# Lanv1/gsplat.js

Measured on AMD Instinct MI355X. Metric: frames_per_sec, higher is better.
Workload: dtype f32

## Files before the change

### gsplat.js_amd/csrc/gsr_api.cpp

```cpp
#include "gsr_ctx.h"

#include <cstdarg>
#include <cstdio>
#include <cstdlib>
#include <cstring>
#include <mutex>

using namespace gsr;

namespace {

thread_local std::string g_create_error;

Knobs read_knobs(std::string& bad)
{
    Knobs k;
    if (const char* e = getenv("GSR_NO_GRAPH")) k.graphs = atoi(e) == 0;
    if (const char* e = getenv("GSR_FUSE_COMBINE")) k.fuse_combine = atoi(e) != 0;
    if (const char* e = getenv("GSR_SATURATE")) k.saturate = atoi(e) != 0;
    if (const char* e = getenv("GSR_ITEMS_BY_SIZE")) k.items_by_size = atoi(e) != 0 ? 1 : 0;
    if (const char* e = getenv("GSR_LONG_ITEMS")) k.long_items = atoi(e) != 0 ? 1 : 0;
    if (const char* e = getenv("GSR_LONG_TAU")) k.long_tau = (uint32_t)std::max(0L, atol(e));
    if (const char* e = getenv("GSR_BIN_ROUNDS")) k.bin_rounds = std::min(64L, std::max(0L, atol(e)));
    if (const char* e = getenv("GSR_BIN_BIG")) k.bin_big = (uint32_t)std::min(2, std::max(0, atoi(e)));
    if (const char* e = getenv("GSR_BIN_TWO_LEVEL")) k.bin_two_level = atoi(e) ? 1 : 0;
    if (const char* e = getenv("GSR_RECT_CARRY")) { k.rect_carry = atoi(e) != 0; k.rect_carry_bucket = atoi(e) == 2; }
    if (const char* e = getenv("GSR_BLEND_SUB")) k.blend_sub = atoi(e) == 2 ? 2 : atoi(e) == 1 ? 1 : 0;
    if (const char* e = getenv("GSR_SORT_ORDER")) k.sort_order = !strcmp(e, "lsd") ? 0 : !strcmp(e, "bucket") ? 1 : -1;
    if (const char* e = getenv("GSR_TIMING_EVERY")) k.timing_every = (uint32_t)std::max(1L, atol(e));
    if (const char* e = getenv("GSR_CELL_GRID")) { const long v = atol(e); if (v >= 1) k.cell_grid = (uint32_t)std::min(v, 65535L); }
    if (const char* e = getenv("GSR_SEG_TARGET")) { const long v = atol(e); if (v >= 1) k.seg_target = (uint32_t)v; }
    if (const char* e = getenv("GSR_BLEND_GRID")) { const long v = atol(e); if (v >= 1) k.blend_grid = (uint32_t)v; }
    if (const char* e = getenv("GSR_SEG_LEN")) { const long v = atol(e); if (v >= 256) k.seg_len = (uint32_t)(v / 256 * 256); }
    if (const char* e = getenv("GSR_SORT_KPB")) { const long v = atol(e); if (v == 2048 || v == 4096 || v == 8192) k.sort_kpb = (uint32_t)v; }
    if (const char* e = getenv("GSR_FRONT_WAVES")) {
        char* end = nullptr;
        const long v = strtol(e, &end, 10);
        if (end != e && *end == 0 && (v == (long)FRONT_WAVES_NARROW || v == (long)FRONT_WAVES_WIDE)) k.front_waves = (uint32_t)v;
        else bad = std::string("GSR_FRONT_WAVES must be ") + std::to_string(FRONT_WAVES_NARROW) + " or " + std::to_string(FRONT_WAVES_WIDE) + ", not \"" + e + "\"";
    }
    if (const char* e = getenv("GSR_DEPTH_SKIP")) k.depth_skip = atoi(e) != 0;
    return k;
}

int alloc_fb(gsr_ctx* c)
{
    const size_t np = (size_t)c->W * c->H;
    if (np > c->out.pixels) {
        if (int r = c->out.fb.alloc(c, np)) return r;
        if (int r = c->out.fb8.alloc(c, np)) return r;
        c->out.pixels = np;
    }
    launch_clear_fb(c->out.fb, c->W, c->H, c->stream);
    return GSR_OK;
}

}

int gsr::fail(gsr_ctx* c, int code, const char* fmt, ...)
{
    char buf[512];
    va_list ap;
    va_start(ap, fmt);
    vsnprintf(buf, sizeof buf, fmt, ap);
    va_end(ap);
    if (c) {
        c->error = buf;
        if (code == GSR_ERR_HIP) c->words.slots_need_init = true;
    }
    else g_create_error = buf;
    return code;
}

extern "C" {

const char* gsr_last_error(gsr_ctx* ctx) { return ctx ? ctx->error.c_str() : g_create_error.c_str(); }

int gsr_create(gsr_ctx** out, const gsr_options* opt)
{
    if (!out) return fail(nullptr, GSR_ERR_ARG, "out is NULL");
    *out = nullptr;
    std::string bad_knob;
    const Knobs knobs = read_knobs(bad_knob);
    if (!bad_knob.empty()) return fail(nullptr, GSR_ERR_ARG, "%s", bad_knob.c_str());
    int count = 0;
    if (hipGetDeviceCount(&count) != hipSuccess || count <= 0)
        return fail(nullptr, GSR_ERR_NO_DEVICE, "no HIP device is visible (this library has no CPU path)");
    gsr_options o{};
    if (opt) o = *opt;
    if (o.device < 0 || o.device >= count) return fail(nullptr, GSR_ERR_ARG, "device %d out of range (%d visible)", o.device, count);
    if (o.width < 0 || o.height < 0 || o.width > 8192 || o.height > 8192) return fail(nullptr, GSR_ERR_ARG, "bad framebuffer size %dx%d (up to 8192)", o.width, o.height);
    if (!(o.early_out_eps >= 0.0f && o.early_out_eps < 1.0f)) return fail(nullptr, GSR_ERR_ARG, "early_out_eps must be in [0,1)");
    gsr_ctx* c = new gsr_ctx();
    c->device = o.device;
    c->scene = new SharedScene();
    c->scene->members.push_back(c);
    c->scene_gen = c->scene->generation;
    c->opt = o;
    c->knobs = knobs;
    c->graph.enabled = c->knobs.graphs;
    c->timing.every = c->knobs.timing_every;
    auto bail = [&](int code) {
        g_create_error = c->error;
        gsr_destroy(c);
        return code;
    };
    gsr_ctx::Words& w = c->words;
    const int r = [&]() -> int {
        HIP_TRY(c, hipSetDevice(c->device));
        HIP_TRY(c, hipStreamCreateWithFlags(&c->stream, hipStreamNonBlocking));
        int cus = 0;
        if (hipDeviceGetAttribute(&cus, hipDeviceAttributeMultiprocessorCount, c->device) == hipSuccess && cus > 0) c->cu_count = cus;
        const size_t slot_words = (size_t)3 * FRAME_SLOTS * FRAME_SLOT_WORDS;
        if (int r = w.fstate.alloc(c, 1)) return r;
        if (int r = w.cam_dev.alloc(c, 1)) return r;
        if (int r = w.slots.alloc(c, slot_words)) return r;
        HIP_TRY(c, hipMemset(w.slots, 0, sizeof(int32_t) * slot_words));
        w.slots_need_init = true;
        if (int r = w.accum.alloc(c, 8)) return r;
        HIP_TRY(c, hipMemset(w.accum, 0, 8 * sizeof(uint64_t)));
        HIP_TRY(c, hipHostMalloc((void**)&w.mailbox, 64, hipHostMallocMapped));
        memset(w.mailbox, 0, 64);
        reinterpret_cast<uint32_t*>(w.mailbox)[2] = 0xffffffffu;
        HIP_TRY(c, hipHostGetDevicePointer((void**)&w.mailbox_dev, w.mailbox, 0));
        HIP_TRY(c, hipHostMalloc((void**)&w.fstate_host, sizeof(FrameState), hipHostMallocDefault));
        memset(w.fstate_host, 0, sizeof(FrameState));
        w.fstate_host->minmax[0] = 0x7fffffff;
        w.fstate_host->minmax[1] = (int32_t)0x80000000;
        HIP_TRY(c, hipMemcpy(w.fstate, w.fstate_host, sizeof(FrameState), hipMemcpyHostToDevice));
        if (o.flags & GSR_FLAG_TIMING) {
            for (auto& set : c->timing.evring)
                for (auto& e : set) HIP_TRY(c, hipEventCreate(&e));
            c->timing.valid = true;
        }
        if (o.width && o.height) {
            if (int r = gsr_resize(c, o.width, o.height)) return r;
            if (o.band_x1 > o.band_x0) {
                if (int r = gsr_set_band(c, o.band_x0, o.band_x1)) return r;
            }
        }
        return GSR_OK;
    }();
    if (r) return bail(r);
    *out = c;
    return GSR_OK;
}

int gsr_destroy(gsr_ctx* c)
{
    if (!c) return GSR_OK;
    (void)hipSetDevice(c->device);
    if (c->stream) (void)hipStreamSynchronize(c->stream);
    comm_release(c);
    delivery_free(c);
    drop_graph(c);
    scene_release(c);
    if (c->share_ev) (void)hipEventDestroy(c->share_ev);
    for (auto& set : c->timing.evring)
        for (auto& e : set) if (e) (void)hipEventDestroy(e);
    for (auto& e : c->link_ev) if (e) (void)hipEventDestroy(e);
    if (c->words.fstate_host) (void)hipHostFree(c->words.fstate_host);
    if (c->words.mailbox) (void)hipHostFree(c->words.mailbox);
    if (c->stream) (void)hipStreamDestroy(c->stream);
    delete c;
    return GSR_OK;
}

int gsr_resize(gsr_ctx* c, int32_t w, int32_t h)
{
    if (!c) return GSR_ERR_ARG;
    if (w <= 0 || h <= 0 || w > 8192 || h > 8192) return fail(c, GSR_ERR_ARG, "bad framebuffer size %dx%d (1..8192)", w, h);
    const gsr_ctx::Delivery& dl = c->delivery;
    const bool new_ring = !dl.ring.empty() && (w != dl.W || h != dl.H);
    if (new_ring && delivery_frame_held(c))
        return fail(c, GSR_ERR_ARG, "gsr_resize: a delivered frame is held (gsr_release_frame first): its pixels would be freed");
    HIP_TRY(c, hipSetDevice(c->device));
    HIP_TRY(c, hipStreamSynchronize(c->stream));
    if (c->comm.nccl && (w != c->W || h != c->H)) comm_release(c);
    c->W = w; c->H = h;
    c->band_x0 = c->band_x1 = 0;
    c->have_frame = false;
    if (int r = alloc_fb(c)) return r;
    if (new_ring) { if (int r = delivery_alloc(c, (int)dl.ring.size())) return r; }
    return alloc_bins(c);
}

int gsr_set_band(gsr_ctx* c, int32_t x0, int32_t x1)
{
    if (!c) return GSR_ERR_ARG;
    if (x0 == 0 && x1 == 0) { c->band_x0 = c->band_x1 = 0; return alloc_bins(c); }
    if (x0 < 0 || x1 <= x0 || x0 % BIN_PX) return fail(c, GSR_ERR_ARG, "band [%d,%d) must start on a multiple of %d", x0, x1, BIN_PX);
    if (x1 > c->W) x1 = c->W;
    if (x0 >= c->W) return fail(c, GSR_ERR_ARG, "band starts outside the image");
    HIP_TRY(c, hipSetDevice(c->device));
    HIP_TRY(c, hipStreamSynchronize(c->stream));
    c->band_x0 = x0; c->band_x1 = x1;
    launch_clear_fb(c->out.fb, c->W, c->H, c->stream);
    return alloc_bins(c);
}

int gsr_set_list_capacity(gsr_ctx* c, uint32_t entries)
{
    if (!c) return GSR_ERR_ARG;
    HIP_TRY(c, hipSetDevice(c->device));
    HIP_TRY(c, hipStreamSynchronize(c->stream));
    c->bin.capacity = std::max<uint32_t>(entries, 1024u);
    if (int r = c->bin.list.alloc(c, c->bin.capacity)) return r;
    return alloc_bins(c, true);
}

int gsr_set_camera(gsr_ctx* c, const float* view, const float* proj, const float* vp, float fx, float fy)
{
    if (!c) return GSR_ERR_ARG;
    if (!view || !proj || !vp) return fail(c, GSR_ERR_ARG, "matrix pointer is NULL");
    memcpy(c->cam.view, view, 64);
    memcpy(c->cam.proj, proj, 64);
    c->cam.vp2 = vp[2]; c->cam.vp6 = vp[6]; c->cam.vp10 = vp[10];
    c->cam.fx = fx; c->cam.fy = fy;
    c->have_cam = true;
    return GSR_OK;
}

int gsr_set_depth_fade(gsr_ctx* c, int32_t use_depth_fade, float depth_fade)
{
    if (!c) return GSR_ERR_ARG;
    c->cam.use_fade = use_depth_fade ? 1 : 0;
    c->cam.fade = depth_fade;
    return GSR_OK;
}

int gsr_render_async(gsr_ctx* c)
{
    if (!c) return GSR_ERR_ARG;
    HIP_TRY(c, hipSetDevice(c->device));
    return enqueue_frame(c, true);
}

int gsr_sync(gsr_ctx* c)
{
    if (!c) return GSR_ERR_ARG;
    HIP_TRY(c, hipSetDevice(c->device));
    if (int r = sync_and_repair(c)) return r;
    if (c->comm.stream) HIP_TRY(c, hipStreamSynchronize(c->comm.stream));
    if (c->delivery.copy_stream) HIP_TRY(c, hipStreamSynchronize(c->delivery.copy_stream));
    if (c->words.dropped_unreported) {
        const unsigned long long k = c->words.dropped_unreported;
        c->words.dropped_unreported = 0;
        return fail(c, GSR_ERR_OVERFLOW,
                    "%llu asynchronous frame(s) were not composited: their bin lists did not fit and later frames had already been "
                    "enqueued (the framebuffer kept the preceding image for them); the lists have been regrown, the context stays usable",
                    k);
    }
    return GSR_OK;
}

int gsr_overflow_pending(gsr_ctx* c) { return c && overflow_pending(c) ? 1 : 0; }

int gsr_render(gsr_ctx* c)
{
    if (int r = gsr_render_async(c)) return r;
    c->timing.render = true;
    return gsr_sync(c);
}

int gsr_sort(gsr_ctx* c)
{
    if (!c) return GSR_ERR_ARG;
    HIP_TRY(c, hipSetDevice(c->device));
    if (int r = enqueue_frame(c, false)) return r;
    return finish_frame(c);
}

int gsr_get_timings(gsr_ctx* c, gsr_timings* out)
{
    if (!c || !out) return GSR_ERR_ARG;
    if (c->timing.recorded) { if (int r = finish_frame(c)) return r; }
    *out = c->timing.tm;
    out->overflow_frames = c->words.overflow_frames;
    out->dropped_frames = c->words.dropped_frames;
    return GSR_OK;
}

int gsr_set_timing_interval(gsr_ctx* c, uint32_t every)
{
    if (!c || !every) return c ? fail(c, GSR_ERR_ARG, "timing interval must be >= 1") : GSR_ERR_ARG;
    c->timing.every = every;
    c->timing.frame_no = 0;
    return GSR_OK;
}

int gsr_reset_timings(gsr_ctx* c)
{
    if (!c) return GSR_ERR_ARG;
    if (c->timing.recorded) { if (int r = finish_frame(c)) return r; }
    gsr_timings& tm = c->timing.tm;
    const uint64_t v = tm.visible, b = tm.bin_entries, d = tm.tile_entries;
    tm = gsr_timings{};
    HIP_TRY(c, hipMemsetAsync(c->words.accum, 0, 4 * sizeof(uint64_t), c->stream));
    tm.visible = v; tm.bin_entries = b; tm.tile_entries = d; tm.n = c->scene->n;
    c->timing.frame_no = 0;
    return GSR_OK;
}

int gsr_device_info(gsr_ctx* c, char* name, int32_t name_len, int32_t* cus, int32_t* clock_khz)
{
    if (!c) return GSR_ERR_ARG;
    hipDeviceProp_t p;
    HIP_TRY(c, hipGetDeviceProperties(&p, c->device));
    if (name && name_len > 0) snprintf(name, (size_t)name_len, "%s (%s)", p.name[0] ? p.name : "AMD GPU", p.gcnArchName);
    if (cus) *cus = p.multiProcessorCount;
    if (clock_khz) *clock_khz = p.clockRate;
    return GSR_OK;
}

void gsplat_sort_host(const float* viewProj, uint32_t vertexCount, const float* fBuffer, uint32_t* depthBuffer,
                      uint32_t* depthIndex, uint32_t* starts, uint32_t* counts)
{
    (void)starts; (void)counts;
    static std::mutex mu;
    static gsr_ctx* ctx = nullptr;
    std::lock_guard<std::mutex> lock(mu);
    auto failed = [&](const char* what) {
        fprintf(stderr, "gsplat_sort_host: %s\n", what);
        if (depthIndex && vertexCount) memset(depthIndex, 0, (size_t)vertexCount * sizeof(uint32_t));
    };
    if (!viewProj || !depthIndex || (vertexCount && !fBuffer)) return failed("NULL argument");
    if (!ctx) {
        gsr_options o{};
        if (gsr_create(&ctx, &o) != GSR_OK) { ctx = nullptr; return failed(gsr_last_error(nullptr)); }
    }
    gsr_ctx* c = ctx;
    if (hipSetDevice(c->device) != hipSuccess || hipStreamSynchronize(c->stream) != hipSuccess) return failed("device unavailable");
    if (vertexCount != c->scene->n || !c->scene->arr.px) {
        if (vertexCount > 0x7fffffffu / 8) return failed("too many splats");
        if (alloc_scene(c, vertexCount, false) != GSR_OK) return failed(gsr_last_error(c));
        c->scene->n = vertexCount;
    }
    c->have_sort = false; c->have_frame = false;
    static DevBuf<float>& stage_pos = *new DevBuf<float>();
    static size_t stage_cap = 0;
    if (vertexCount) {
        if ((size_t)vertexCount * 3 > stage_cap) {
            if (stage_pos.alloc(c, (size_t)vertexCount * 3) != GSR_OK) { stage_cap = 0; return failed(gsr_last_error(c)); }
            stage_cap = (size_t)vertexCount * 3;
        }
        const gsr::SceneArrays& sa = c->scene->arr;
        hipError_t e1 = hipMemcpyAsync(stage_pos, fBuffer, (size_t)vertexCount * 12, hipMemcpyHostToDevice, c->stream);
        launch_repack_positions(stage_pos, vertexCount, sa.px, sa.py, sa.pz, c->stream);
        for (hipError_t e : {e1, hipGetLastError()})
            if (e != hipSuccess) return failed(hipGetErrorString(e));
    }
    float ident[16] = {1, 0, 0, 0, 0, 1, 0, 0, 0, 0, 1, 0, 0, 0, 0, 1};
    if (gsr_set_camera(c, ident, ident, viewProj, 1.f, 1.f) != GSR_OK) return failed(gsr_last_error(c));
    if (hipSetDevice(c->device) != hipSuccess || enqueue_frame(c, false) != GSR_OK) return failed(gsr_last_error(c));
    if (vertexCount) {
        hipError_t e1 = hipMemcpyAsync(depthIndex, c->sort.depth_index, (size_t)vertexCount * 4, hipMemcpyDeviceToHost, c->stream);
        hipError_t e2 = depthBuffer ? hipMemcpyAsync(depthBuffer, c->sort.keys, (size_t)vertexCount * 4, hipMemcpyDeviceToHost, c->stream) : hipSuccess;
        for (hipError_t e : {e1, e2})
            if (e != hipSuccess) return failed(hipGetErrorString(e));
    }
    if (finish_frame(c) != GSR_OK) return failed(gsr_last_error(c));
}

const char* gsr_build_id(void)
{
#ifdef GSR_BUILD_ID
    return GSR_BUILD_ID;
#else
    return "unknown";
#endif
}

}
```

### gsplat.js_amd/csrc/gsr_ctx.h

```cpp
#pragma once
#include "../../include/gsplat_hip.h"
#include "gsr_internal.h"

#include <algorithm>
#include <cstddef>
#include <string>
#include <type_traits>
#include <utility>
#include <vector>

struct ncclComm;

#pragma GCC visibility push(hidden)

namespace gsr {

int fail(gsr_ctx* c, int code, const char* fmt, ...);

#define HIP_TRY(c, expr)                                                                         \
    do {                                                                                         \
        hipError_t e_ = (expr);                                                                  \
        if (e_ != hipSuccess) return gsr::fail((c), GSR_ERR_HIP, "%s failed: %s", #expr, hipGetErrorString(e_)); \
    } while (0)

template <class T>
struct DevBuf {
    T* p = nullptr;
    DevBuf() = default;
    DevBuf(const DevBuf&) = delete;
    DevBuf& operator=(const DevBuf&) = delete;
    DevBuf(DevBuf&& o) noexcept : p(o.p) { o.p = nullptr; }
    DevBuf& operator=(DevBuf&& o) noexcept { std::swap(p, o.p); return *this; }
    ~DevBuf() { reset(); }
    void reset() { if (p) { (void)hipFree(p); p = nullptr; } }
    int alloc(gsr_ctx* c, size_t count)
    {
        reset();
        if (!count) count = 1;
        HIP_TRY(c, hipMalloc((void**)&p, count * sizeof(T)));
        return GSR_OK;
    }
    operator T*() const { return p; }
    T* operator->() const { return p; }
};

enum Stage { EV_BEGIN = 0, EV_PROJECT, EV_SORT, EV_BIN, EV_BLEND , EV_COMBINE , EV_COUNT };

struct FrameState {
    int32_t minmax[2];
    uint32_t overflow;
    uint32_t queue;
    uint64_t visible;
    uint64_t tile_entries;
    uint64_t report[6];
    uint32_t digit_total[RADIX_LO_BINS + RADIX_HI_BINS];
    uint32_t sorted_count;
    uint32_t seg_len;
    uint32_t n_items;
    uint32_t spec;
};

struct Knobs {
    bool graphs = true;
    bool fuse_combine = true;
    bool saturate = true;
    int items_by_size = -1;
    int long_items = -1;
    uint32_t long_tau = 0;
    long bin_rounds = 0;
    uint32_t bin_big = 2;
    int bin_two_level = -1;
    bool rect_carry = true;
    bool rect_carry_bucket = false;
    int blend_sub = 0;
    int sort_order = -1;
    uint32_t timing_every = 1;
    uint32_t cell_grid = 0;
    uint32_t seg_target = 0;
    uint32_t blend_grid = 0;
    uint32_t seg_len = 0;
    uint32_t sort_kpb = 0;
    uint32_t front_waves = 0;
    bool depth_skip = true;
};

struct SceneArrays {
    DevBuf<float> px, py, pz;
    DevBuf<uint32_t> cov0, cov1, cov2, rgba;
    DevBuf<float4> rot, scl;
    int alloc(gsr_ctx* c, size_t n, bool with_rows)
    {
        int r;
        if ((r = px.alloc(c, n)) || (r = py.alloc(c, n)) || (r = pz.alloc(c, n)) || (r = cov0.alloc(c, n)) || (r = cov1.alloc(c, n)) ||
            (r = cov2.alloc(c, n)) || (r = rgba.alloc(c, n)))
            return r;
        rot.reset(); scl.reset();
        if (with_rows && ((r = rot.alloc(c, n)) || (r = scl.alloc(c, n)))) return r;
        return GSR_OK;
    }
    SceneDev view() const { return SceneDev{px, py, pz, cov0, cov1, cov2, rgba, rot, scl}; }
};

struct SharedScene {
    SceneArrays arr;
    uint32_t n = 0;
    uint32_t arr_rows = 0;
    bool have_rows = false;
    bool given = false;
    std::vector<gsr_ctx*> members;
    uint64_t generation = 1;
    DevBuf<uint32_t> sh_r, sh_g, sh_b;
    uint32_t sh_count = 0;
    int32_t band[3] = {-1, -1, -1};
    SceneSoA soa(float4* shcol) const { return SceneSoA{arr.px, arr.py, arr.pz, arr.cov0, arr.cov1, arr.cov2, arr.rgba, sh_r, sh_g, sh_b, shcol}; }
    bool sh_follow = false;
    DevBuf<uint32_t> sh_spare[3];
    uint32_t sh_rows = 0, sh_spare_rows = 0;
    double sh_frame[9] = {1, 0, 0, 0, 1, 0, 0, 0, 1};
    void reset_sh_frame() { for (int k = 0; k < 9; k++) sh_frame[k] = (k % 4 == 0) ? 1.0 : 0.0; }
    bool sh_frame_is_identity() const
    {
        for (int k = 0; k < 9; k++) if (sh_frame[k] != ((k % 4 == 0) ? 1.0 : 0.0)) return false;
        return true;
    }
    void drop_sh() { sh_count = 0; band[0] = band[1] = band[2] = -1; sh_r.reset(); sh_g.reset(); sh_b.reset(); reset_sh_frame();
                     for (auto& b : sh_spare) b.reset();
                     sh_rows = sh_spare_rows = 0; }
    struct Selection {
        DevBuf<uint32_t> mask, scratch;
        DevBuf<uint32_t> counters;
        DevBuf<uint8_t> region;
        uint32_t words = 0;
        uint32_t counter_words = 0;
        size_t region_bytes = 0;
        uint32_t count = 0;
        void reset() { mask.reset(); scratch.reset(); counters.reset(); region.reset(); words = counter_words = 0; region_bytes = 0; count = 0; }
        uint64_t bytes() const { return (uint64_t)words * 8 + (uint64_t)counter_words * 4 + region_bytes; }
    } sel;
    struct Contrib {
        DevBuf<unsigned long long> weight;
        DevBuf<uint32_t> peak, pixels;
        DevBuf<uint32_t> counters;
        uint32_t rows = 0;
        static constexpr uint32_t COUNTER_WORDS = 2;
        bool live() const { return (bool)counters.p; }
        void reset() { weight.reset(); peak.reset(); pixels.reset(); counters.reset(); rows = 0; }
        uint64_t bytes() const { return live() ? (uint64_t)rows * 16 + COUNTER_WORDS * 4 : 0; }
    } contrib;
    uint64_t bytes() const
    {
        return (uint64_t)arr_rows * (7 * 4 + (arr.rot ? 32 : 0)) + ((uint64_t)sh_rows + sh_spare_rows) * 3 * 32 + sel.bytes() + contrib.bytes();
    }
};

struct ProjectArgs {
    SceneSoA sc;
    int32_t* depth; int32_t* slots; Record* rec; uint32_t* rect; uint32_t* overflow; uint32_t* kept; uint8_t* kept_lane;
};

struct FrameArgs {
    ProjectArgs proj;
    int32_t* slots_next;
    SortBuffers sort;
    BinBuffers bin;
    BinGrid grid;
    BlendBuffers blend;
    float early_out_eps;
    uint32_t n;
    bool render;
};
static_assert(std::is_trivially_copyable<FrameArgs>::value, "FrameArgs is compared and copied as bytes");

struct DepthSpec {
    int format = GSR_DEPTH_NONE;
    int step = 1;
    float near = 0.0f;
    static DepthSpec from(const gsr_depth_delivery_options* o)
    {
        if (!o || o->format == GSR_DEPTH_NONE) return {};
        return {o->format, o->step, o->format == GSR_DEPTH_U16 ? o->near : 0.0f};
    }
    bool on() const { return format != GSR_DEPTH_NONE; }
    size_t sample_bytes() const { return format == GSR_DEPTH_U16 ? 2 : 4; }
    bool operator==(const DepthSpec& o) const { return format == o.format && step == o.step && near == o.near; }
    size_t plane_bytes(int Wd, int Hd) const { return (size_t)Wd * Hd * sample_bytes(); }
    gsr_depth_layout layout(int Wd, int Hd, uint64_t offset) const
    {
        gsr_depth_layout l{};
        l.format = format; l.step = step; l.width = Wd; l.height = Hd;
        l.stride = (int32_t)plane_bytes(Wd, 1);
        l.offset = offset;
        l.bytes = plane_bytes(Wd, Hd);
        l.near = near;
        return l;
    }
};

struct DepthPlanes {
    DevBuf<float> hit;
    DevBuf<float> mean;
    DevBuf<uint32_t> index;
    DevBuf<uint32_t> invalid;
    int Wd = 0, Hd = 0;
    int fill_key[4] = {0, 0, 0, 0};
    int alloc(gsr_ctx* c, int W, int H, int step)
    {
        reset();
        Wd = (W + step - 1) / step; Hd = (H + step - 1) / step;
        const size_t np = (size_t)Wd * Hd;
        int r = hit.alloc(c, np);
        if (!r && step == 1) { r = mean.alloc(c, np); if (!r) r = index.alloc(c, np); }
        if (!r) r = invalid.alloc(c, 1);
        if (r) reset();
        return r;
    }
    void reset() { hit.reset(); mean.reset(); index.reset(); invalid.reset(); Wd = Hd = 0; std::fill(fill_key, fill_key + 4, 0); }
};
enum DepthFill { DEPTH_FILL_NOTHING, DEPTH_FILL_HIT , DEPTH_FILL_PLANES  };

}

struct gsr_ctx {
    int device = 0;
    int cu_count = 256;
    hipStream_t stream = nullptr;
    std::string error;
    gsr_options opt{};
    gsr::Knobs knobs;
    int W = 0, H = 0;
    int band_x0 = 0, band_x1 = 0;
    gsr::CamParams cam{};
    gsr::CamParams cam_frame{};
    bool have_cam = false, have_frame = false, have_sort = false;
    uint64_t frame_serial = 0;
    bool frame_lists = false;
    hipEvent_t link_ev[2] = {nullptr, nullptr};

    gsr::SharedScene* scene = nullptr;
    uint64_t scene_gen = 0;
    gsr::DevBuf<float4> shcol;
    hipEvent_t share_ev = nullptr;
    gsr::SceneSoA scene_soa() const { return scene->soa(shcol); }

    struct Sort {
        gsr::DevBuf<int32_t> depth;
        gsr::DevBuf<uint32_t> kept;
        gsr::DevBuf<uint8_t> kept_lane;
        gsr::DevBuf<uint32_t> koff;
        gsr::DevBuf<uint32_t> keys, keys_tmp, idx_tmp, depth_index, block_hist;
        gsr::DevBuf<gsr::Record> rec;
        gsr::DevBuf<uint32_t> rect_idx;
        gsr::DevBuf<uint32_t> rects;
        gsr::DevBuf<uint32_t> rect_tmp;
        gsr::DevBuf<uint32_t> chunk_tab;
        uint32_t rows = 0;
        int parity = 0;
        gsr::SortPlan plan{};
    } sort;

    struct Bin {
        gsr::DevBuf<uint32_t> table, total, start, start_pre, list;
        gsr::DevBuf<uint32_t> cell_list, cell_total, cell_start, chunk_start, chunk_info, cell_table2, cell_wcnt;
        gsr::DevBuf<uint32_t> seg_start, items;
        gsr::DevBuf<unsigned long long> mask;
        gsr::DevBuf<float4> partial;
        gsr::BinPlan plan{};
        gsr::BlendPlan blend{};
        uint32_t cell_capacity_alloc = 0, cell_ncells_alloc = 0;
        uint32_t capacity = 0, table_elems = 0, nbins_alloc = 0;
    } bin;

    struct Words {
        gsr::DevBuf<gsr::FrameState> fstate;
        gsr::FrameState* fstate_host = nullptr;
        gsr::DevBuf<int32_t> slots;
        bool slots_need_init = true;
        gsr::DevBuf<gsr::CamParams> cam_dev;
        gsr::DevBuf<uint64_t> accum;
        uint64_t* mailbox = nullptr;
        uint64_t* mailbox_dev = nullptr;
        uint64_t overflow_seen = 0;
        uint64_t overflow_frames = 0;
        uint64_t dropped_frames = 0;
        uint64_t dropped_unreported = 0;
    } words;

    struct Out {
        gsr::DevBuf<float4> fb;
        gsr::DevBuf<uint32_t> fb8;
        size_t pixels = 0;
    } out;

    struct Graph {
        bool enabled = true;
        hipGraph_t graph = nullptr;
        hipGraphExec_t exec = nullptr;
        hipGraphNode_t project = nullptr;
        gsr::FrameArgs key;
    } graph;
    gsr::ProjectLaunch proj{};

    struct Timing {
        static constexpr int EV_RING = 128;
        hipEvent_t evring[EV_RING][gsr::EV_COUNT]{};
        bool is_render[EV_RING]{};
        int head = 0, pending = 0;
        hipEvent_t* ev = nullptr;
        bool valid = false, recorded = false, render = false;
        uint32_t every = 1, frame_no = 0;
        gsr_timings tm{};
    } timing;

    struct Comm {
        ncclComm* nccl = nullptr;
        gsr_allgather_fn fn = nullptr;
        void* fn_user = nullptr;
        bool owned = true;
        gsr_ctx* leader = nullptr;
        std::vector<gsr_ctx*> followers;
        int rank = 0, world = 0, slab_w = 0;
        hipStream_t stream = nullptr;
        hipEvent_t ev_packed = nullptr, ev_slab_free = nullptr;
        gsr::DevBuf<uint32_t> slab, gathered, frame8;
        gsr::SlabEdges edges{};
        bool frame8_valid = false;
        bool joined() const { return nccl || fn; }
        struct DepthExchange {
            gsr::DepthSpec spec;
            gsr::DepthPlanes planes;
            int W = 0, H = 0;
            int stride = 0;
            size_t offset = 0;
            size_t slab_bytes = 0;
            gsr::SlabEdges edges{};
            gsr::DevBuf<uint32_t> plane;
            bool on() const { return spec.on(); }
            size_t plane_bytes() const { return spec.plane_bytes(planes.Wd, planes.Hd); }
            void reset() { spec = {}; planes.reset(); plane.reset(); W = H = stride = 0; offset = slab_bytes = 0; }
        } depth;
        size_t slab_bytes(int H) const { return depth.on() ? depth.slab_bytes : ((size_t)slab_w * H + gsr::SLAB_FLAG_WORDS) * 4; }
    } comm;

    struct Depth {
        gsr::DepthPlanes planes;
        size_t pixels = 0;
        gsr::DevBuf<int32_t> query;
        gsr::DevBuf<gsr::PickResult> result;
        gsr::DevBuf<uint32_t> pick_invalid;
        float hit_alpha = 0.5f;
        uint64_t planes_serial = 0;
    } depth;

    struct Delivery {
        struct Slot {
            uint8_t* host = nullptr;
            gsr::DevBuf<uint32_t> staging;
            hipEvent_t done = nullptr;
            uint64_t serial = 0;
            enum State { FREE, IN_FLIGHT, HELD } state = FREE;
        };
        std::vector<Slot> ring;
        hipStream_t copy_stream = nullptr;
        hipEvent_t ev_staged = nullptr;
        int W = 0, H = 0;
        int format = GSR_FORMAT_RGBA8;
        gsr::YuvParams yuv{};
        int next = 0;
        uint64_t serial = 0;
        struct DepthPlane {
            gsr::DepthSpec spec;
            gsr::DepthPlanes planes;
        } depth;
        size_t pixel_bytes() const { return format == GSR_FORMAT_RGBA8 ? (size_t)W * H * 4 : gsr::yuv420_bytes(W, H); }
        size_t depth_offset() const { return (pixel_bytes() + 15) & ~(size_t)15; }
        size_t depth_bytes() const { return depth.spec.plane_bytes(depth.planes.Wd, depth.planes.Hd); }
        size_t trailer_offset() const { return depth.spec.on() ? (depth_offset() + depth_bytes() + 15) & ~(size_t)15 : (pixel_bytes() + 3) & ~(size_t)3; }
        size_t slot_bytes() const { return trailer_offset() + gsr::DELIVER_TRAILER_WORDS * 4; }
    } delivery;
};

namespace gsr {

inline BinGrid make_grid(const gsr_ctx* c)
{
    BinGrid g;
    g.W = c->W; g.H = c->H;
    g.nbx = (c->W + BIN_PX - 1) / BIN_PX;
    g.nby = (c->H + BIN_PX - 1) / BIN_PX;
    if (c->band_x1 > c->band_x0) {
        g.bx_lo = c->band_x0 / BIN_PX;
        g.bx_hi = std::min((c->band_x1 + BIN_PX - 1) / BIN_PX, g.nbx);
    } else {
        g.bx_lo = 0; g.bx_hi = g.nbx;
    }
    return g;
}

inline uint32_t front_waves_of(const gsr_ctx* c)
{
    return c->knobs.front_waves ? c->knobs.front_waves : (c->opt.flags & GSR_FLAG_THROUGHPUT) ? FRONT_WAVES_NARROW : FRONT_WAVES_WIDE;
}

inline SortKnobs sort_knobs_of(const gsr_ctx* c)
{
    return SortKnobs{c->knobs.sort_order, c->knobs.sort_kpb, c->knobs.rect_carry ? 1u : 0u, c->knobs.rect_carry_bucket ? 1u : 0u};
}

int alloc_bins(gsr_ctx* c, bool fresh_items = false);
int enqueue_frame(gsr_ctx* c, bool render);
int finish_frame(gsr_ctx* c);
int sync_and_repair(gsr_ctx* c);
void drop_graph(gsr_ctx* c);
int alloc_scene(gsr_ctx* c, uint32_t n, bool with_rows);
int adopt_scene(gsr_ctx* c);
void scene_release(gsr_ctx* c);
int scene_compact(gsr_ctx* c, const ScenePred& p, const char* what, uint32_t* kept_out);
int select_ensure(gsr_ctx* c);
int select_fold_and_count(gsr_ctx* c, int op, uint32_t* selected);
void comm_release(gsr_ctx* c);
int depth_frame_check(gsr_ctx* c, const char* who);
int depth_enqueue(gsr_ctx* c, DepthPlanes& p, int step, DepthFill fill);
int depth_settle_frame(gsr_ctx* c, const char* who);
int depth_planes_current(gsr_ctx* c, const char* who);
int delivery_alloc(gsr_ctx* c, int slots);
int depth_options_check(gsr_ctx* c, const char* who, const gsr_depth_delivery_options* depth);
void delivery_free(gsr_ctx* c);
bool delivery_frame_held(const gsr_ctx* c);

inline bool overflow_pending(const gsr_ctx* c)
{
    return c->words.mailbox && *reinterpret_cast<volatile const uint64_t*>(c->words.mailbox) != c->words.overflow_seen;
}

}

#pragma GCC visibility pop
```

### gsplat.js_amd/csrc/gsr_frame.cpp

```cpp
#include "gsr_ctx.h"

#include <algorithm>
#include <cstring>

using namespace gsr;

namespace {

inline uint32_t largest_bucket_reported(const gsr_ctx* c) { return reinterpret_cast<volatile const uint32_t*>(c->words.mailbox)[2]; }

bool band_is_partial(const BinGrid& g) { return g.bx_lo > 0 || g.bx_hi < g.nbx; }

void build_frame_args(const gsr_ctx* c, bool render, FrameArgs& a)
{
    memset(&a, 0, sizeof a);
    const BinGrid g = make_grid(c);
    const SortPlan sp = plan_sort(c->scene->n, c->sort.rows, front_waves_of(c), render, band_is_partial(g), largest_bucket_reported(c), sort_knobs_of(c));
    FrameState* fs = c->words.fstate;
    a.render = render;
    a.n = c->scene->n;
    a.grid = g;
    a.early_out_eps = c->opt.early_out_eps;

    const size_t slot_set = (size_t)FRAME_SLOTS * FRAME_SLOT_WORDS;
    int32_t* slots_now = render ? c->words.slots.p : c->words.slots + (size_t)(1 + c->sort.parity) * slot_set;
    a.slots_next = render ? nullptr : c->words.slots + (size_t)(2 - c->sort.parity) * slot_set;

    a.proj.sc = c->scene_soa();
    a.proj.depth = c->sort.depth;
    a.proj.slots = slots_now;
    if (render) {
        a.proj.rec = c->sort.rec;
        a.proj.rect = c->sort.rect_idx;
        a.proj.overflow = &fs->overflow;
        a.proj.kept = sp.band ? c->sort.kept.p : nullptr;
        a.proj.kept_lane = sp.band ? c->sort.kept_lane.p : nullptr;
    }

    SortBuffers& sb = a.sort;
    sb.depth = c->sort.depth;
    sb.slots = slots_now;
    sb.minmax = fs->minmax;
    sb.keys = c->sort.keys;
    sb.keys_tmp = c->sort.keys_tmp;
    sb.idx_tmp = c->sort.idx_tmp;
    sb.depth_index = c->sort.depth_index;
    sb.block_hist = c->sort.block_hist;
    sb.digit_total = fs->digit_total;
    sb.rect = c->sort.rect_idx;
    sb.kept = c->sort.kept;
    sb.kept_lane = c->sort.kept_lane;
    sb.koff = sp.band ? c->sort.koff.p : nullptr;
    sb.count = &fs->sorted_count;
    sb.plan = sp;
    sb.max_bucket = reinterpret_cast<uint32_t*>(c->words.mailbox_dev + 1);
    sb.chunk_tab = c->sort.chunk_tab;
    sb.rect_tmp = c->sort.rect_tmp;
    sb.rects_out = sp.carry ? c->sort.rects.p : nullptr;
    if (!render) return;

    BinBuffers& bb = a.bin;
    bb.depth_index = c->sort.depth_index;
    bb.count = &fs->sorted_count;
    bb.table = c->bin.table;
    bb.slots = c->words.slots;
    bb.rect_idx = c->sort.rect_idx;
    bb.rects = c->sort.rects;
    bb.rects_sorted = sp.carry;
    bb.bin_total = c->bin.total;
    bb.bin_start = c->bin.start;
    bb.bin_start_pre = c->bin.start_pre;
    bb.plan = c->bin.plan;
    bb.seg_start = c->bin.seg_start;
    bb.items = c->bin.items;
    bb.list = c->bin.list;
    bb.overflow = &fs->overflow;
    bb.visible = &fs->visible;
    bb.tile_entries = &fs->tile_entries;
    bb.accum = c->words.accum;
    bb.mailbox = c->words.mailbox_dev;
    bb.report = fs->report;
    bb.capacity = c->bin.capacity;
    bb.seg_len_dev = &fs->seg_len;
    bb.queue = &fs->queue;
    bb.bin_mask = c->bin.mask;
    bb.cell_list = c->bin.cell_list;
    bb.cell_total = c->bin.cell_total;
    bb.cell_start = c->bin.cell_start;
    bb.chunk_start = c->bin.chunk_start;
    bb.chunk_info = c->bin.chunk_info;
    bb.cell_wcnt = c->bin.cell_wcnt;
    bb.cell_table2 = c->bin.cell_table2;
    bb.band = band_is_partial(g) ? 1u : 0u;
    bb.n_max = c->scene->n;

    BlendBuffers& bl = a.blend;
    bl.items = bb.items;
    bl.seg_start = bb.seg_start;
    bl.bin_start = bb.bin_start;
    bl.list = bb.list;
    bl.rec = c->sort.rec;
    bl.shcol = c->shcol;
    bl.fb = c->out.fb;
    bl.partial = c->bin.partial;
    bl.queue = bb.queue;
    bl.seg_len_dev = bb.seg_len_dev;
    bl.capacity = bb.capacity;
    bl.nsplats = std::max(c->scene->n, 1u);
    bl.bin_mask = bb.bin_mask;
    bl.plan = c->bin.blend;
}

void set_projection(gsr_ctx* c, const FrameArgs& a)
{
    ProjectLaunch& p = c->proj;
    p.sc = a.proj.sc;
    p.n = a.n;
    p.cam = c->cam;
    p.do_project = 1;
    p.depth = a.proj.depth;
    p.slots = a.proj.slots;
    p.rec = a.proj.rec;
    p.bbox = nullptr;
    p.rect = a.proj.rect;
    p.overflow = a.proj.overflow;
    p.kept = a.proj.kept;
    p.kept_lane = a.proj.kept_lane;
    p.bind();
}

int enqueue_chain(gsr_ctx* c, const FrameArgs& a, bool timing)
{
    hipStream_t s = c->stream;
    hipEvent_t* ev = c->timing.ev;
    if (timing) HIP_TRY(c, hipEventRecord(ev[EV_BEGIN], s));
    if (a.n) {
        if (a.render) launch_project_key(c->proj, s);
        else launch_depth_key(a.proj.sc, a.n, c->cam, a.proj.depth, a.proj.slots, a.slots_next, s);
    } else {
        HIP_TRY(c, hipMemsetD32Async((hipDeviceptr_t)&a.sort.minmax[0], 0x7fffffff, 1, s));
        HIP_TRY(c, hipMemsetD32Async((hipDeviceptr_t)&a.sort.minmax[1], (int)0x80000000u, 1, s));
    }
    if (timing) HIP_TRY(c, hipEventRecord(ev[EV_PROJECT], s));
    launch_sort(a.sort, a.n, s);
    if (timing) HIP_TRY(c, hipEventRecord(ev[EV_SORT], s));
    if (a.render) {
        if (!a.n) {
            HIP_TRY(c, hipMemsetAsync(a.bin.bin_total, 0, sizeof(uint32_t) * a.bin.plan.nbins, s));
            HIP_TRY(c, hipMemsetAsync(a.bin.overflow, 0, sizeof(uint32_t), s));
        }
        launch_bin(a.bin, a.blend.plan, a.grid, s);
        if (timing) HIP_TRY(c, hipEventRecord(ev[EV_BIN], s));
        launch_blend(a.blend, a.grid, a.early_out_eps, s, (timing && !a.blend.plan.fused) ? ev[EV_BLEND] : nullptr);
        if (timing) HIP_TRY(c, hipEventRecord(ev[EV_COMBINE], s));
    }
    HIP_TRY(c, hipGetLastError());
    return GSR_OK;
}

bool capture_graph(gsr_ctx* c, const FrameArgs& a)
{
    hipStream_t s = c->stream;
    if (hipStreamBeginCapture(s, hipStreamCaptureModeRelaxed) != hipSuccess) return false;
    const int r = enqueue_chain(c, a, false);
    hipGraph_t gph = nullptr;
    bool ok = (hipStreamEndCapture(s, &gph) == hipSuccess) && r == GSR_OK && gph;
    hipGraphNode_t project = nullptr;
    if (ok && a.n) {
        size_t nn = 0;
        ok = hipGraphGetNodes(gph, nullptr, &nn) == hipSuccess && nn > 0;
        std::vector<hipGraphNode_t> nodes(nn);
        if (ok) ok = hipGraphGetNodes(gph, nodes.data(), &nn) == hipSuccess;
        for (size_t k = 0; ok && k < nn && !project; k++) {
            hipGraphNodeType ty;
            hipKernelNodeParams kp{};
            if (hipGraphNodeGetType(nodes[k], &ty) == hipSuccess && ty == hipGraphNodeTypeKernel &&
                hipGraphKernelNodeGetParams(nodes[k], &kp) == hipSuccess && kp.func == project_key_kernel())
                project = nodes[k];
        }
        ok = ok && project != nullptr;
    }
    if (ok) ok = hipGraphInstantiate(&c->graph.exec, gph, nullptr, nullptr, 0) == hipSuccess;
    if (ok) { c->graph.graph = gph; c->graph.project = project; memcpy(&c->graph.key, &a, sizeof a); }
    else if (gph) (void)hipGraphDestroy(gph);
    return ok;
}

bool set_graph_camera(gsr_ctx* c)
{
    hipKernelNodeParams kp{};
    kp.func = const_cast<void*>(project_key_kernel());
    kp.gridDim = project_key_grid(c->proj.n);
    kp.blockDim = dim3(PROJ_THREADS);
    kp.sharedMemBytes = 0;
    kp.kernelParams = c->proj.ptrs;
    kp.extra = nullptr;
    return hipGraphExecKernelNodeSetParams(c->graph.exec, c->graph.project, &kp) == hipSuccess;
}

int check_frame_words(gsr_ctx* c, bool* overflowed)
{
    FrameState* host = c->words.fstate_host;
    HIP_TRY(c, hipMemcpyAsync(host, c->words.fstate, offsetof(FrameState, digit_total), hipMemcpyDeviceToHost, c->stream));
    HIP_TRY(c, hipStreamSynchronize(c->stream));
    const uint64_t* acc = host->report;
    gsr_timings& tm = c->timing.tm;
    tm.sum_visible = acc[0]; tm.sum_bin_entries = acc[1]; tm.sum_tile_entries = acc[2]; tm.sum_frames = acc[3];
    tm.visible = host->visible;
    tm.tile_entries = host->tile_entries;
    tm.bin_entries = (uint32_t)host->report[5];
    tm.n = c->scene->n;
    *overflowed = host->overflow != 0;
    return GSR_OK;
}

int handle_overflow(gsr_ctx* c, uint64_t* newly)
{
    *newly = 0;
    HIP_TRY(c, hipStreamSynchronize(c->stream));
    uint64_t acc[8];
    HIP_TRY(c, hipMemcpyAsync(acc, c->words.accum, sizeof acc, hipMemcpyDeviceToHost, c->stream));
    HIP_TRY(c, hipStreamSynchronize(c->stream));
    if (acc[5] == c->words.overflow_seen) return GSR_OK;
    *newly = acc[5] - c->words.overflow_seen;
    c->words.overflow_seen = acc[5];
    c->words.overflow_frames += *newly;
    const uint64_t need = acc[6];
    const uint64_t want = need + (need >> 2) + (1u << 20);
    if (want > 0xfffffff0ull) return fail(c, GSR_ERR_OVERFLOW, "bin list would need %llu entries", (unsigned long long)want);
    if (want > c->bin.capacity) {
        c->bin.capacity = (uint32_t)want;
        if (int r = c->bin.list.alloc(c, c->bin.capacity)) return r;
    }
    return alloc_bins(c, true);
}

}

namespace gsr {

int alloc_bins(gsr_ctx* c, bool fresh_items)
{
    if (!c->W) return GSR_OK;
    c->frame_lists = false;
    gsr_ctx::Bin& b = c->bin;
    const Knobs& k = c->knobs;
    const BinGrid g = make_grid(c);
    const uint64_t capacity = b.capacity ? b.capacity : std::max<uint64_t>(6ull * c->scene->n + (1u << 20), 1u << 22);
    b.plan = plan_bins(g, c->scene->n, capacity, c->cu_count, front_waves_of(c), BinKnobs{k.bin_two_level, k.bin_big, k.bin_rounds, k.cell_grid});
    const BinPlan& p = b.plan;
    const uint32_t nbins = (uint32_t)p.nbins;
    const bool items_afresh = fresh_items || nbins > b.nbins_alloc || !b.capacity;
    const uint32_t items_alloc = items_afresh ? 0u : b.blend.max_items;
    b.blend = plan_blend(nbins, (uint32_t)((g.bx_hi - g.bx_lo) * BIN_PX) * (uint32_t)c->H, (uint32_t)capacity, c->cu_count,
                         (c->opt.flags & GSR_FLAG_THROUGHPUT) != 0, c->opt.early_out_eps > 0.0f, items_alloc,
                         BlendKnobs{k.fuse_combine ? 1u : 0u, k.saturate ? 1u : 0u, k.items_by_size, k.long_items, k.long_tau, k.blend_sub, k.seg_target,
                                    k.blend_grid, k.seg_len});
    const size_t table = (size_t)p.table_rows * p.table_cols;
    if (table > b.table_elems) {
        if (int r = b.table.alloc(c, table)) return r;
        b.table_elems = (uint32_t)table;
    }
    if (nbins > b.nbins_alloc) {
        if (int r = b.total.alloc(c, nbins)) return r;
        if (int r = b.start.alloc(c, nbins + 1)) return r;
        if (int r = b.start_pre.alloc(c, nbins + 1)) return r;
        if (int r = b.seg_start.alloc(c, nbins + 1)) return r;
        if (b.blend.fused) {
            if (int r = b.mask.alloc(c, nbins)) return r;
        }
        b.nbins_alloc = nbins;
    }
    if (!b.capacity) {
        b.capacity = (uint32_t)capacity;
        if (int r = b.list.alloc(c, b.capacity)) return r;
    }
    if (p.form == BIN_TWO_LEVEL) {
        const uint32_t ncells = (uint32_t)p.ncells;
        if (ncells > b.cell_ncells_alloc) {
            if (int r = b.cell_total.alloc(c, ncells + 1)) return r;
            if (int r = b.cell_start.alloc(c, ncells + 1)) return r;
            if (int r = b.chunk_start.alloc(c, ncells + 2)) return r;
            b.cell_ncells_alloc = ncells;
            b.cell_capacity_alloc = 0;
        }
        if (b.capacity > b.cell_capacity_alloc) {
            if (int r = b.cell_list.alloc(c, (size_t)b.capacity * 2)) return r;
            if (int r = b.cell_table2.alloc(c, (size_t)p.chunks * 16u)) return r;
            if (int r = b.chunk_info.alloc(c, (size_t)p.chunks * 4u)) return r;
            if (int r = b.cell_wcnt.alloc(c, (size_t)p.chunks * 64u)) return r;
            b.cell_capacity_alloc = b.capacity;
        }
    }
    if (b.blend.max_items > items_alloc) {
        if (int r = b.items.alloc(c, (size_t)b.blend.max_items * 4)) return r;
        if (b.blend.partial_slots) {
            if (int r = b.partial.alloc(c, (size_t)b.blend.partial_slots * BIN_PX * BIN_PX)) return r;
        }
    }
    return GSR_OK;
}

void drop_graph(gsr_ctx* c)
{
    if (c->graph.exec) (void)hipGraphExecDestroy(c->graph.exec);
    if (c->graph.graph) (void)hipGraphDestroy(c->graph.graph);
    c->graph.exec = nullptr; c->graph.graph = nullptr; c->graph.project = nullptr;
}

int enqueue_frame(gsr_ctx* c, bool render)
{
    if (!c->have_cam) return fail(c, GSR_ERR_ARG, "gsr_set_camera has not been called");
    if (render && (!c->W || !c->H)) return fail(c, GSR_ERR_ARG, "framebuffer size is 0");
    hipStream_t s = c->stream;
    if (int r = adopt_scene(c)) return r;
    if (render && overflow_pending(c)) {
        uint64_t newly = 0;
        if (int r = handle_overflow(c, &newly)) return r;
        c->words.dropped_frames += newly;
        c->words.dropped_unreported += newly;
    }
    gsr_ctx::Timing& t = c->timing;
    const bool timing = t.valid && t.every != 0xffffffffu && (t.frame_no++ % t.every) == 0;
    if (timing) {
        if (t.pending == gsr_ctx::Timing::EV_RING) { if (int r = finish_frame(c)) return r; }
        const int slot = (t.head + t.pending) % gsr_ctx::Timing::EV_RING;
        t.ev = t.evring[slot];
        t.is_render[slot] = render;
    }
    FrameArgs a;
    build_frame_args(c, render, a);
    c->cam.W = c->W; c->cam.H = c->H;
    c->cam.band_px0 = a.grid.bx_lo * BIN_PX;
    c->cam.band_px1 = a.grid.bx_hi * BIN_PX;
    c->cam.sh_on = c->scene->sh_count ? 1 : 0;
    c->cam.band[0] = c->scene->band[0]; c->cam.band[1] = c->scene->band[1]; c->cam.band[2] = c->scene->band[2];
    c->cam.sh_frame = (c->scene->sh_count && !c->scene->sh_frame_is_identity()) ? 1 : 0;
    for (int k = 0; k < 9; k++) c->cam.shm[k] = c->cam.sh_frame ? (float)c->scene->sh_frame[k] : 0.0f;
    if (render) c->cam_frame = c->cam;
    static_assert(offsetof(FrameState, minmax) == 0 && sizeof(FrameState) % 4 == 0, "k_begin_frame initialises the frame words");
    if (c->words.slots_need_init) {
        for (int k = 0; k < 3; k++)
            launch_begin_frame(c->cam, c->words.cam_dev, reinterpret_cast<uint32_t*>(c->words.fstate.p), (uint32_t)(sizeof(FrameState) / 4),
                               c->words.slots + (size_t)k * FRAME_SLOTS * FRAME_SLOT_WORDS, s);
        c->words.slots_need_init = false;
    }
    if (render) set_projection(c, a);

    bool replayed = false;
    if (c->graph.enabled && render && !timing) {
        bool ok = true;
        if (!c->graph.exec || memcmp(&a, &c->graph.key, sizeof a) != 0) {
            drop_graph(c);
            ok = capture_graph(c, a);
        }
        else if (c->graph.project) ok = set_graph_camera(c);
        if (!ok) {
            (void)hipGetLastError();
            drop_graph(c);
            c->graph.enabled = false;
        }
        if (c->graph.exec) {
            HIP_TRY(c, hipGraphLaunch(c->graph.exec, s));
            replayed = true;
        }
    }
    if (!replayed) { if (int r = enqueue_chain(c, a, timing)) return r; }
    if (!render && a.n) c->sort.parity ^= 1;
    c->sort.plan = a.sort.plan;
    if (timing) t.pending++;
    t.recorded = timing;
    t.render = render;
    c->have_sort = true;
    c->have_frame = c->have_frame || render;
    if (render) { c->frame_serial++; c->frame_lists = true; }
    return GSR_OK;
}

int finish_frame(gsr_ctx* c)
{
    HIP_TRY(c, hipStreamSynchronize(c->stream));
    gsr_ctx::Timing& t = c->timing;
    while (t.pending > 0) {
        hipEvent_t* ev = t.evring[t.head];
        const bool render = t.is_render[t.head];
        float a = 0, b = 0, d = 0, e = 0, f = 0, tot = 0;
        HIP_TRY(c, hipEventElapsedTime(&a, ev[EV_BEGIN], ev[EV_PROJECT]));
        HIP_TRY(c, hipEventElapsedTime(&b, ev[EV_PROJECT], ev[EV_SORT]));
        tot = a + b;
        if (render) {
            HIP_TRY(c, hipEventElapsedTime(&d, ev[EV_SORT], ev[EV_BIN]));
            if (c->bin.blend.fused) {
                HIP_TRY(c, hipEventElapsedTime(&e, ev[EV_BIN], ev[EV_COMBINE]));
            } else {
                HIP_TRY(c, hipEventElapsedTime(&e, ev[EV_BIN], ev[EV_BLEND]));
                HIP_TRY(c, hipEventElapsedTime(&f, ev[EV_BLEND], ev[EV_COMBINE]));
            }
            HIP_TRY(c, hipEventElapsedTime(&tot, ev[EV_BEGIN], ev[EV_COMBINE]));
        }
        t.tm.ms_project_key = a; t.tm.ms_sort = b; t.tm.ms_bin = d; t.tm.ms_blend = e; t.tm.ms_combine = f; t.tm.ms_total = tot;
        t.tm.sum_ms_project_key += a; t.tm.sum_ms_sort += b; t.tm.sum_ms_bin += d; t.tm.sum_ms_blend += e; t.tm.sum_ms_combine += f;
        t.tm.sum_ms_total += tot;
        t.tm.frames++;
        t.head = (t.head + 1) % gsr_ctx::Timing::EV_RING;
        t.pending--;
    }
    t.recorded = false;
    return GSR_OK;
}

int sync_and_repair(gsr_ctx* c)
{
    if (int r = finish_frame(c)) return r;
    bool last_ov = false;
    if (c->have_frame && c->timing.render) {
        if (int r = check_frame_words(c, &last_ov)) return r;
    }
    if (overflow_pending(c)) {
        uint64_t newly = 0;
        if (int r = handle_overflow(c, &newly)) return r;
        if (last_ov && newly) {
            if (int r = enqueue_frame(c, true)) return r;
            if (int r = finish_frame(c)) return r;
            bool again = false;
            if (int r = check_frame_words(c, &again)) return r;
            if (again) return fail(c, GSR_ERR_OVERFLOW, "bin list overflow after regrowth");
            newly -= 1;
        }
        c->words.dropped_frames += newly;
        c->words.dropped_unreported += newly;
    }
    return GSR_OK;
}

}

extern "C" int gsr_debug_last_sort_plan(gsr_ctx* c, SortPlan* out)
{
    if (!c || !out) return GSR_ERR_ARG;
    if (!c->have_sort) return fail(c, GSR_ERR_ARG, "no sort has run yet");
    *out = c->sort.plan;
    return GSR_OK;
}

extern "C" int gsr_debug_last_blend_plan(gsr_ctx* c, BlendPlan* out)
{
    if (!c || !out) return GSR_ERR_ARG;
    *out = c->bin.blend;
    return GSR_OK;
}
```

### gsplat.js_amd/csrc/gsr_internal.h

```cpp
#pragma once
#include <hip/hip_runtime.h>
#include <stdint.h>

namespace gsr {

constexpr int WAVE = 64;
constexpr uint32_t DEPTH_RANGE = 65536u;
constexpr int KEY_BITS = 17;
constexpr int RADIX_LO_BITS = 8;
constexpr int RADIX_HI_BITS = 9;
constexpr int RADIX_LO_BINS = 1 << RADIX_LO_BITS;
constexpr int RADIX_HI_BINS = 1 << RADIX_HI_BITS;

constexpr int TILE = 16;
constexpr int BIN_TILES = 2;
constexpr int BIN_PX = TILE * BIN_TILES;

struct CamParams {
    float view[16];
    float proj[16];
    float vp2, vp6, vp10;
    float fx, fy;
    int32_t W, H;
    int32_t sh_on;
    int32_t band[3];
    int32_t band_px0, band_px1;
    int32_t use_fade;
    float fade;
    int32_t sh_frame;
    float shm[9];
};

struct __attribute__((aligned(16))) Record {
    float cx, cy, ux, uy;
    float wx, wy, la;
    uint32_t rgb8;
};
constexpr uint32_t RGB8_IN_SHCOL = 0x01000000u;
static_assert(sizeof(Record) == 32, "record must be 32 bytes");

constexpr uint32_t BBOX_INVISIBLE_X = 1u;
constexpr uint32_t BBOX_INVISIBLE_Y = 1u;

constexpr uint32_t RECT_NONE = 1u;
__host__ __device__ inline uint32_t pack_bin_rect(uint32_t bbx, uint32_t bby, int bx_lo, int bx_hi)
{
    const int px0 = (int)(bbx & 0xffffu), px1 = (int)(bbx >> 16), py0 = (int)(bby & 0xffffu), py1 = (int)(bby >> 16);
    if (px0 > px1) return RECT_NONE;
    const int x0 = (px0 / BIN_PX > bx_lo ? px0 / BIN_PX : bx_lo) - bx_lo;
    const int x1 = (px1 / BIN_PX < bx_hi - 1 ? px1 / BIN_PX : bx_hi - 1) - bx_lo;
    if (x0 > x1) return RECT_NONE;
    return (uint32_t)x0 | ((uint32_t)x1 << 8) | ((uint32_t)(py0 / BIN_PX) << 16) | ((uint32_t)(py1 / BIN_PX) << 24);
}

struct SceneSoA {
    const float *px, *py, *pz;
    const uint32_t *cov0, *cov1, *cov2, *rgba;
    const uint32_t *sh_r, *sh_g, *sh_b;
    float4* shcol;
};

struct SceneDev {
    float *px, *py, *pz;
    uint32_t *cov0, *cov1, *cov2, *rgba;
    float4* rot;
    float4* scl;
};
void launch_build_scene(const uint8_t* rows, uint32_t n, const SceneDev& sc, hipStream_t s);
void launch_scene_translate(uint32_t n, const SceneDev& sc, const double* t, hipStream_t s);
void launch_scene_rotate(uint32_t n, const SceneDev& sc, const double* q_xyzw, hipStream_t s);
void launch_scene_scale(uint32_t n, const SceneDev& sc, const double* sv, hipStream_t s);
struct ScenePred { const double* box; const uint32_t* mask; uint32_t keep; };
void launch_scene_compact(uint32_t n, const SceneDev& src, const SceneDev& dst, const ScenePred& p, uint32_t* block_count,
                          uint32_t* total, hipStream_t s);
void launch_scene_compact_sh(uint32_t n, const SceneDev& src, const ScenePred& p, const uint32_t* block_off, uint32_t* count,
                             const int32_t* band, uint32_t sh_count, const uint32_t* const* sh_in, uint32_t* const* sh_out, hipStream_t s);
void launch_scene_import(const float* scales, uint32_t n, float4* scl, hipStream_t s);
void launch_scene_export(uint32_t n, const SceneDev& sc, uint32_t* data, float* positions, float* scales, hipStream_t s);

void launch_repack_scene(const uint32_t* data, const float* positions, uint32_t n, float* px, float* py, float* pz,
                         uint32_t* cov0, uint32_t* cov1, uint32_t* cov2, uint32_t* rgba, uint32_t* mismatch, hipStream_t s);

void launch_repack_positions(const float* positions, uint32_t n, float* px, float* py, float* pz, hipStream_t s);

void launch_begin_frame(const CamParams& cam, CamParams* dst, uint32_t* frame_words, uint32_t nwords, int32_t* slots, hipStream_t s);
#ifdef __HIPCC__
__device__ __forceinline__ uint32_t xcd_group_remap(uint32_t bid, uint32_t nwg)
{
    constexpr uint32_t RUN = 8u, G = 8u * RUN;
    const uint32_t full = nwg - nwg % G;
    if (bid >= full) return bid;
    const uint32_t in = bid % G;
    return (bid - in) + (in % 8u) * RUN + in / 8u;
}
#endif
#ifdef GSR_BOUNDS
#define GSR_BOUNDS_DECL(name) __device__ unsigned int g_bounds_##name[8];                                             \
    extern "C" int gsr_debug_bounds_##name(unsigned int* out) { return hipMemcpyFromSymbol(out, HIP_SYMBOL(g_bounds_##name), sizeof g_bounds_##name) == hipSuccess ? 0 : -1; }
#define GSR_BOUND(name, site, idx, limit) do { if (!((unsigned long long)(idx) < (unsigned long long)(limit))) atomicAdd(&g_bounds_##name[site], 1u); } while (0)
#else
#define GSR_BOUNDS_DECL(name)
#define GSR_BOUND(name, site, idx, limit) do { } while (0)
#endif

constexpr uint32_t PROJ_THREADS = 256;
constexpr int FRAME_SLOTS = 64;
constexpr int FRAME_SLOT_WORDS = 32;
void launch_depth_key(const SceneSoA& sc, uint32_t n, const CamParams& cam, int32_t* depth, int32_t* slots, int32_t* slots_next, hipStream_t s);
struct ProjectLaunch {
    SceneSoA sc; uint32_t n; CamParams cam; int do_project;
    int32_t* depth;
    int32_t* slots;
    Record* rec; uint2* bbox;
    uint32_t* rect;
    uint32_t* overflow;
    uint32_t* kept;
    uint8_t* kept_lane;
    void* ptrs[12];
    void bind();
};
const void* project_key_kernel();
dim3 project_key_grid(uint32_t n);
void launch_project_key(ProjectLaunch& a, hipStream_t s);

constexpr uint32_t FRONT_WAVES_WIDE = 16, FRONT_WAVES_NARROW = 8;

enum SortForm : uint32_t {
    SORT_NONE = 0,
    SORT_LSD,
    SORT_BUCKET_WIDE,
    SORT_BUCKET_NARROW,
};
struct SortPlan {
    uint32_t form;
    uint32_t carry;
    uint32_t band;
    uint32_t keys_per_block;
    uint32_t blocks;
    uint32_t waves;
    uint32_t lds_first, lds_last;
    uint32_t local_grid;
    uint32_t proj_blocks;
};
struct SortSizes {
    uint32_t keys_per_block;
    size_t block_hist, chunk_tab, kept, koff;
};
struct SortKnobs { int32_t sort_order; uint32_t sort_kpb, rect_carry, rect_carry_bucket; };
SortPlan plan_sort(uint32_t n, uint32_t rows, uint32_t front_waves, bool render, bool cull, uint32_t largest_bucket, const SortKnobs& k);
SortSizes sort_sizes(uint32_t rows, const SortKnobs& k);

struct SortBuffers {
    const int32_t* depth;
    const int32_t* slots;
    int32_t* minmax;
    uint32_t* keys;
    uint32_t* keys_tmp;
    uint32_t* idx_tmp;
    uint32_t* depth_index;
    uint32_t* block_hist;
    uint32_t* digit_total;
    const uint32_t* rect;
    const uint32_t* kept;
    const uint8_t* kept_lane;
    uint32_t* koff;
    uint32_t* count;
    SortPlan plan;
    uint32_t* max_bucket;
    uint32_t* chunk_tab;
    uint32_t* rect_tmp;
    uint32_t* rects_out;
};
void launch_sort(const SortBuffers& b, uint32_t n, hipStream_t s);
void launch_column_scan(uint32_t* table, uint32_t* total, int ncols, uint32_t nrows, hipStream_t s, const uint32_t* live = nullptr, uint32_t live_unit = 1);

struct BinGrid {
    int32_t nbx, nby;
    int32_t bx_lo, bx_hi;
    int32_t W, H;
};
enum BinForm : uint32_t {
    BIN_FINALIZE_ONLY = 0,
    BIN_FUSED_WIDE,
    BIN_FUSED_NARROW,
    BIN_SEPARATE_FINALIZE,
    BIN_LARGE_GRID,
    BIN_TWO_LEVEL,
};
struct BinSlices { int32_t sx, sy, w, h; };
struct BinPlan {
    uint32_t form;
    int32_t nbins;
    uint32_t groups;
    uint32_t steps_per_wave;
    uint32_t rounds;
    uint32_t blocks;
    BinSlices slices;
    uint32_t count_slices, count_rows;
    uint32_t count_lds, scatter_lds;
    uint32_t extra_wg;
    uint32_t table_rows, table_cols;
    int32_t ncx, ncy, ncells;
    uint32_t cell_grid;
    uint32_t chunks;
};
struct BinKnobs { int32_t two_level; uint32_t big; int64_t rounds; uint32_t cell_grid; };
BinPlan plan_bins(const BinGrid& g, uint32_t n, uint64_t capacity, int cu_count, uint32_t front_waves, const BinKnobs& k);

constexpr uint32_t SEG_LEN_WHOLE_BIN = 0x7fffff00u;
__host__ __device__ inline bool is_whole_bin(uint32_t seg_len) { return seg_len >= 0x40000000u; }

struct BlendPlan {
    uint32_t waves_per_tile;
    uint32_t fused;
    uint32_t separate_fold;
    uint32_t whole_bin;
    uint32_t threads;
    uint32_t grid;
    uint32_t queue_start;
    uint32_t seg_len;
    uint32_t seg_target_items;
    uint32_t max_items;
    uint32_t partial_slots;
    int32_t items_by_size;
    int32_t long_policy;
    uint32_t seg_len_long, long_tau;
    uint32_t long_tiles_x2;
    uint32_t long_tau_bin;
    uint32_t long_mass_min;
    uint32_t npix;
    uint32_t saturate;
};
struct BlendKnobs { uint32_t fuse_combine, saturate; int32_t items_by_size, long_items; uint32_t long_tau; int32_t blend_sub; uint32_t seg_target, blend_grid, seg_len; };
BlendPlan plan_blend(uint32_t nbins, uint32_t npix, uint32_t capacity, int cu_count, bool throughput, bool early_out, uint32_t allocated_items,
                     const BlendKnobs& k);

struct BinBuffers {
    const uint32_t* depth_index;
    const uint32_t* count;
    uint32_t* table;
    int32_t* slots;
    const uint32_t* rect_idx;
    uint32_t* rects;
    uint32_t rects_sorted;
    uint32_t* bin_total;
    uint32_t* bin_start;
    uint32_t* bin_start_pre;
    BinPlan plan;
    uint32_t* seg_start;
    uint32_t* items;
    uint32_t* list;
    uint32_t* overflow;
    uint64_t* visible;
    uint64_t* tile_entries;
    uint64_t* accum;
    uint64_t* mailbox;
    uint64_t* report;
    uint32_t capacity;
    uint32_t* seg_len_dev;
    uint32_t* queue;
    unsigned long long* bin_mask;
    uint32_t* cell_list;
    uint32_t* cell_total;
    uint32_t* cell_start;
    uint32_t* chunk_start;
    uint32_t* chunk_info;
    uint32_t* cell_wcnt;
    uint32_t* cell_table2;
    uint32_t band;
    uint32_t n_max;
};
void launch_bin(const BinBuffers& b, const BlendPlan& bp, const BinGrid& g, hipStream_t s);

struct BlendBuffers {
    const uint32_t* items;
    const uint32_t* seg_start;
    const uint32_t* bin_start;
    const uint32_t* list;
    const Record* rec;
    const float4* shcol;
    float4* fb;
    float4* partial;
    uint32_t* queue;
    const uint32_t* seg_len_dev;
    uint32_t capacity;
    uint32_t nsplats;
    unsigned long long* bin_mask;
    BlendPlan plan;
};
void launch_blend(const BlendBuffers& b, const BinGrid& g, float early_out_eps, hipStream_t s, hipEvent_t between);
void launch_clear_fb(float4* fb, int32_t W, int32_t H, hipStream_t s);
void launch_to_rgba8(const float4* fb, uint32_t* out, uint32_t npix, hipStream_t s);
#ifdef __HIPCC__
__device__ __forceinline__ uint32_t to_rgba8(float4 v)
{
    auto q = [](float x) -> uint32_t {
        x = fminf(fmaxf(x, 0.0f), 1.0f);
        return (uint32_t)(x * 255.0f + 0.5f);
    };
    return q(v.x) | (q(v.y) << 8) | (q(v.z) << 16) | (q(v.w) << 24);
}
#endif
constexpr int DELIVER_TRAILER_WORDS = 4;
void launch_deliver_rgba8(const float4* fb, uint32_t* staging, int32_t W, int32_t H, uint64_t serial, const uint32_t* overflow, hipStream_t s);
struct YuvParams {
    int32_t y0, y[3], cb[3], cr[3], c_lo, c_hi;
    uint32_t bg;
};
constexpr int DELIVER_NV12 = 1, DELIVER_I420 = 2;
inline size_t yuv420_bytes(int32_t W, int32_t H) { return (size_t)W * H + 2 * (size_t)((W + 1) / 2) * ((H + 1) / 2); }
void launch_deliver_yuv(int format, const float4* fb, const uint32_t* frame8, uint8_t* staging, size_t staging_bytes, int32_t W, int32_t H,
                        const YuvParams& k, uint64_t serial, const uint32_t* overflow, hipStream_t s);
constexpr int DELIVER_DEPTH_F32 = 1, DELIVER_DEPTH_U16 = 2;
void launch_deliver_depth(int format, const float* plane, uint8_t* staging, size_t depth_offset, size_t trailer_offset, int32_t Wd, int32_t Hd, float near,
                          int32_t W, int32_t H, uint64_t serial, const uint32_t* overflow, hipStream_t s);

struct DepthBuffers {
    const uint32_t* bin_start;
    const uint32_t* list;
    const Record* rec;
    const float *px, *py, *pz;
    const uint32_t* overflow;
    uint32_t* invalid;
    float* mean; float* hit; uint32_t* index;
    uint32_t capacity;
    uint32_t nsplats;
    float hit_alpha;
};
struct PickResult { uint32_t index; float depth, mean, alpha; };
void launch_depth_planes(const DepthBuffers& b, const BinGrid& g, const CamParams& cam, bool skip, int step, hipStream_t s);
void launch_pick(const DepthBuffers& b, const BinGrid& g, const CamParams& cam, const int32_t* xy, uint32_t count, PickResult* out, hipStream_t s);
void launch_depth_fill(float* mean, float* hit, uint32_t* index, uint32_t npix, hipStream_t s);

constexpr int SELECT_CENTRE = 0, SELECT_HIT = 1;
constexpr int SELOP_REPLACE = 0, SELOP_ADD = 1, SELOP_SUBTRACT = 2, SELOP_INTERSECT = 3,
              SELOP_INVERT = 4;
constexpr uint32_t SELECT_APPLY_THREADS = 256;
struct SelectRegion {
    int32_t x0, y0, x1, y1;
    const uint8_t* bytes;
    int32_t stride;
    uint32_t nbytes;
};
struct SelectBuffers {
    const uint32_t* bin_start;
    const uint32_t* list;
    const Record* rec;
    const uint32_t* overflow;
    const uint32_t* index;
    uint32_t* invalid;
    uint32_t* scratch;
    uint32_t capacity;
    uint32_t nsplats, nwords;
};
void launch_select_region(int mode, const SelectBuffers& b, const BinGrid& g, const SelectRegion& r, hipStream_t s);
void launch_select_box(uint32_t n, const float* px, const float* py, const float* pz, const double* box, uint32_t* scratch, uint32_t nwords, hipStream_t s);
void launch_select_apply(int op, uint32_t* sel, const uint32_t* scratch, uint32_t n, uint32_t nwords, uint32_t* block_sums, uint32_t* count, hipStream_t s);

struct ContribBuffers {
    const uint32_t* bin_start;
    const uint32_t* list;
    const Record* rec;
    const float *px, *py, *pz;
    const uint32_t* overflow;
    unsigned long long* weight;
    uint32_t* peak;
    uint32_t* pixels;
    uint32_t* frames;
    uint32_t capacity;
    uint32_t nsplats;
    uint32_t rows;
};
constexpr int CONTRIB_WEIGHT = 0, CONTRIB_PEAK = 1, CONTRIB_PIXELS = 2;
void launch_contrib(const ContribBuffers& b, const BinGrid& g, const CamParams& cam, bool skip, hipStream_t s);
void launch_contrib_select(int stat, double below, uint32_t n, const unsigned long long* weight, const uint32_t* peak, const uint32_t* pixels,
                           uint32_t* scratch, uint32_t nwords, hipStream_t s);

constexpr int MAX_SLABS = 16;
struct SlabEdges { int32_t x0[MAX_SLABS], x1[MAX_SLABS]; };
constexpr int SLAB_FLAG_WORDS = 4;
void launch_pack_band_rgba8(const float4* fb, uint32_t* slab, int W, int H, int x0, int x1, int slab_w, hipStream_t s, const uint32_t* overflow = nullptr);
void launch_unpack_slabs_rgba8(const uint32_t* gathered, uint32_t* image, int W, int H, int slab_w, int world,
                               const SlabEdges& e, hipStream_t s, uint32_t* stale = nullptr, size_t slab_stride = 0);
void launch_pack_band_depth(int format, const float* plane, uint8_t* section, int Wd, int Hd, int xd0, int xd1, int stride, float near, hipStream_t s);
void launch_unpack_slabs_depth(int format, const uint8_t* gathered, uint32_t* plane, int Wd, int Hd, size_t slab_bytes, size_t offset, int stride,
                               int world, const SlabEdges& e, hipStream_t s);
void launch_deliver_gathered_depth(const uint32_t* plane, uint32_t words, uint8_t* staging, size_t depth_offset, size_t trailer_offset, int32_t W, int32_t H,
                                   uint64_t serial, const uint32_t* stale, hipStream_t s);

}
```

### gsplat.js_amd/csrc/k_project.hip

```cpp
#include "gsr_internal.h"

namespace gsr {

__global__ __launch_bounds__(256) void k_repack_scene(const uint4* __restrict__ data, const float* __restrict__ positions,
                                                      uint32_t n, float* __restrict__ px, float* __restrict__ py,
                                                      float* __restrict__ pz, uint32_t* __restrict__ cov0,
                                                      uint32_t* __restrict__ cov1, uint32_t* __restrict__ cov2,
                                                      uint32_t* __restrict__ rgba, uint32_t* __restrict__ mismatch)
{
    uint32_t i = blockIdx.x * blockDim.x + threadIdx.x;
    if (i >= n) return;
    uint4 a = data[2 * (size_t)i], b = data[2 * (size_t)i + 1];
    float x = positions[3 * (size_t)i], y = positions[3 * (size_t)i + 1], z = positions[3 * (size_t)i + 2];
    if (__float_as_uint(x) != a.x || __float_as_uint(y) != a.y || __float_as_uint(z) != a.z) atomicOr(mismatch, 1u);
    px[i] = x; py[i] = y; pz[i] = z;
    cov0[i] = b.x; cov1[i] = b.y; cov2[i] = b.z; rgba[i] = b.w;
}

void launch_repack_scene(const uint32_t* data, const float* positions, uint32_t n, float* px, float* py, float* pz,
                         uint32_t* cov0, uint32_t* cov1, uint32_t* cov2, uint32_t* rgba, uint32_t* mismatch, hipStream_t s)
{
    if (!n) return;
    hipLaunchKernelGGL(k_repack_scene, dim3((n + 255) / 256), dim3(256), 0, s, (const uint4*)data, positions, n, px, py,
                       pz, cov0, cov1, cov2, rgba, mismatch);
}

__global__ __launch_bounds__(256) void k_repack_positions(const float* __restrict__ positions, uint32_t n, float* __restrict__ px,
                                                          float* __restrict__ py, float* __restrict__ pz)
{
    const uint32_t i = blockIdx.x * blockDim.x + threadIdx.x;
    if (i >= n) return;
    px[i] = positions[3 * (size_t)i]; py[i] = positions[3 * (size_t)i + 1]; pz[i] = positions[3 * (size_t)i + 2];
}

void launch_repack_positions(const float* positions, uint32_t n, float* px, float* py, float* pz, hipStream_t s)
{
    if (!n) return;
    hipLaunchKernelGGL(k_repack_positions, dim3((n + 255) / 256), dim3(256), 0, s, positions, n, px, py, pz);
}

__device__ __forceinline__ void mat3_mul(const float* a, const float* b, float* r)
{
#pragma unroll
    for (int c = 0; c < 3; c++)
#pragma unroll
        for (int ro = 0; ro < 3; ro++) {
            float s = a[0 * 3 + ro] * b[c * 3 + 0];
            s = s + a[1 * 3 + ro] * b[c * 3 + 1];
            s = s + a[2 * 3 + ro] * b[c * 3 + 2];
            r[c * 3 + ro] = s;
        }
}

__device__ __forceinline__ float half_bits_to_float(uint32_t h)
{
    return (float)__builtin_bit_cast(_Float16, (unsigned short)(h & 0xffffu));
}

__device__ __forceinline__ bool finite4(float a, float b, float c, float d)
{
    return isfinite(a) && isfinite(b) && isfinite(c) && isfinite(d);
}

__device__ __forceinline__ float eval_sh_channel(const float* k, uint32_t deg, float x, float y, float z)
{
    constexpr float C0 = 0.28209479177387814f, C1 = 0.4886025119029199f;
    constexpr float C2_0 = 1.0925484305920792f, C2_1 = -1.0925484305920792f, C2_2 = 0.31539156525252005f,
                    C2_3 = -1.0925484305920792f, C2_4 = 0.5462742152960396f;
    constexpr float C3_0 = -0.5900435899266435f, C3_1 = 2.890611442640554f, C3_2 = -0.4570457994644658f,
                    C3_3 = 0.3731763325901154f, C3_4 = -0.4570457994644658f, C3_5 = 1.445305721320277f,
                    C3_6 = -0.5900435899266435f;
    float r = C0 * k[0];
    if (deg > 0) {
        r = r - ((((C1 * y) * k[1]) + ((C1 * z) * k[2])) - ((C1 * x) * k[3]));
        if (deg > 1) {
            const float xx = x * x, yy = y * y, zz = z * z, xy = x * y, yz = y * z, xz = x * z;
            float s2 = (C2_0 * xy) * k[4];
            s2 = s2 + (C2_1 * yz) * k[5];
            s2 = s2 + (C2_2 * ((2.0f * zz - xx) - yy)) * k[6];
            s2 = s2 + (C2_3 * xz) * k[7];
            s2 = s2 + (C2_4 * (xx - yy)) * k[8];
            r = r + s2;
            if (deg > 2) {
                float s3 = ((C3_0 * y) * (3.0f * xx - yy)) * k[9];
                s3 = s3 + ((C3_1 * xy) * z) * k[10];
                s3 = s3 + ((C3_2 * y) * ((4.0f * zz - xx) - yy)) * k[11];
                s3 = s3 + ((C3_3 * z) * ((2.0f * zz - 3.0f * xx) - 3.0f * yy)) * k[12];
                s3 = s3 + ((C3_4 * x) * ((4.0f * zz - xx) - yy)) * k[13];
                s3 = s3 + ((C3_5 * z) * (xx - yy)) * k[14];
                s3 = s3 + ((C3_6 * x) * (xx - 3.0f * yy)) * k[15];
                r = r + s3;
            }
        }
    }
    r = r + 0.5f;
    r = (r > 0.0f) ? r : 0.0f;
    return (r < 1.0f) ? r : 1.0f;
}

__device__ __forceinline__ float eval_sh_texture(const uint32_t* __restrict__ tex, uint32_t t, uint32_t deg, float x, float y, float z)
{
    const uint4 a = reinterpret_cast<const uint4*>(tex)[2 * (size_t)t], b = reinterpret_cast<const uint4*>(tex)[2 * (size_t)t + 1];
    const uint32_t w[8] = {a.x, a.y, a.z, a.w, b.x, b.y, b.z, b.w};
    float k[16];
#pragma unroll
    for (int j = 0; j < 8; j++) { k[2 * j] = half_bits_to_float(w[j]); k[2 * j + 1] = half_bits_to_float(w[j] >> 16); }
    return eval_sh_channel(k, deg, x, y, z);
}

__global__ __launch_bounds__(PROJ_THREADS) void k_project_key(SceneSoA sc, uint32_t n, CamParams cam,
                                                              int do_project, int32_t* __restrict__ depth,
                                                              int32_t* __restrict__ slots,
                                                              Record* __restrict__ rec, uint2* __restrict__ bbox,
                                                              uint32_t* __restrict__ rect, uint32_t* __restrict__ overflow,
                                                              uint32_t* __restrict__ kept, uint8_t* __restrict__ kept_lane)
{
    const bool frame = do_project != 2;
    const bool pack = frame && kept != nullptr;
    if (frame && blockIdx.x == 0 && threadIdx.x == 0) *overflow = 0u;
    __shared__ int32_t s_min[4], s_max[4];
    __shared__ uint32_t s_vis[4], s_til[4], s_oti[4], s_oma[4], s_keep[4];
    int32_t mydepth = 0;
    bool keep = false;
    int32_t dmin = 0x7fffffff, dmax = (int32_t)0x80000000;
    uint32_t vis = 0, tiles = 0;
    uint32_t otiles = 0;
    uint32_t omass = 0;
    const int bx_lo = cam.band_px0 / BIN_PX, bx_hi = (cam.band_px1 + BIN_PX - 1) / BIN_PX;

    const uint32_t i = blockIdx.x * PROJ_THREADS + threadIdx.x;
    if (i < n) {
        const float x = sc.px[i], y = sc.py[i], z = sc.pz[i];
        const float f0 = cam.vp2 * x;
        const float f1 = cam.vp6 * y;
        const float f2 = cam.vp10 * z;
        const int32_t d = (int32_t)(((f0 + f1) + f2) * 4096.0f);
        if (frame && !pack) depth[i] = d;
        mydepth = d;
        dmin = d; dmax = d;

        if (do_project) {
            uint2 bb = make_uint2(BBOX_INVISIBLE_X, BBOX_INVISIBLE_Y);
            uint32_t op8 = 0;
            float area = 0.0f;
            do {
                float camv[4], pos2d[4];
#pragma unroll
                for (int r = 0; r < 4; r++) {
                    float s = cam.view[0 * 4 + r] * x;
                    s = s + cam.view[1 * 4 + r] * y;
                    s = s + cam.view[2 * 4 + r] * z;
                    s = s + cam.view[3 * 4 + r];
                    camv[r] = s;
                }
#pragma unroll
                for (int r = 0; r < 4; r++) {
                    float s = cam.proj[0 * 4 + r] * camv[0];
                    s = s + cam.proj[1 * 4 + r] * camv[1];
                    s = s + cam.proj[2 * 4 + r] * camv[2];
                    s = s + cam.proj[3 * 4 + r] * camv[3];
                    pos2d[r] = s;
                }
                const float clip = 1.2f * pos2d[3];
                if (pos2d[2] < -pos2d[3] || pos2d[0] < -clip || pos2d[0] > clip || pos2d[1] < -clip || pos2d[1] > clip) break;

                const uint32_t c0 = sc.cov0[i], c1 = sc.cov1[i], c2 = sc.cov2[i], cw = sc.rgba[i];
                const float u1x = half_bits_to_float(c0), u1y = half_bits_to_float(c0 >> 16);
                const float u2x = half_bits_to_float(c1), u2y = half_bits_to_float(c1 >> 16);
                const float u3x = half_bits_to_float(c2), u3y = half_bits_to_float(c2 >> 16);
                const float Vrk[9] = {u1x, u1y, u2x, u1y, u2y, u3x, u2x, u3x, u3y};
                const float zz = camv[2] * camv[2];
                const float J[9] = {cam.fx / camv[2], 0.f, -(cam.fx * camv[0]) / zz,
                                    0.f, -cam.fy / camv[2], (cam.fy * camv[1]) / zz,
                                    0.f, 0.f, 0.f};
                const float V3t[9] = {cam.view[0], cam.view[4], cam.view[8], cam.view[1], cam.view[5],
                                      cam.view[9], cam.view[2], cam.view[6], cam.view[10]};
                float T[9], Tt[9], TtV[9], cov2d[9];
                mat3_mul(V3t, J, T);
#pragma unroll
                for (int c = 0; c < 3; c++)
#pragma unroll
                    for (int r = 0; r < 3; r++) Tt[c * 3 + r] = T[r * 3 + c];
                mat3_mul(Tt, Vrk, TtV);
                mat3_mul(TtV, T, cov2d);
                const float a = cov2d[0] + 0.3f;
                const float b = cov2d[1];
                const float c = cov2d[4] + 0.3f;
                const float det = a * c - b * b;
                if (det == 0.0f) break;
                const float mid = (a + c) / 2.0f;
                const float rad = mid * mid - det;
                const float sq = sqrtf((0.1f < rad) ? rad : 0.1f);
                const float lambda1 = mid + sq;
                const float lambda2 = mid - sq;
                if (lambda2 < 0.0f) break;
                const float dvx = b, dvy = lambda1 - a;
                const float len = sqrtf(dvx * dvx + dvy * dvy);
                const float dgx = dvx / len, dgy = dvy / len;
                float smaj = sqrtf(2.0f * lambda1), smin = sqrtf(2.0f * lambda2);
                smaj = (1024.0f < smaj) ? 1024.0f : smaj;
                smin = (1024.0f < smin) ? 1024.0f : smin;
                float majx = smaj * dgx, majy = smaj * dgy;
                float minx = smin * dgy, miny = smin * -dgx;
                if (cam.use_fade) {
                    const float depthNorm = (pos2d[2] / pos2d[3] + 1.0f) / 2.0f;
                    const float nearv = 0.1f, farv = 100.0f;
                    const float normalizedDepth = (2.0f * nearv) / (farv + nearv - depthNorm * (farv - nearv));
                    float st = normalizedDepth - 0.1f; st = (st > 0.0f) ? st : 0.0f;
                    float en = normalizedDepth + 0.1f; en = (en < 1.0f) ? en : 1.0f;
                    float sf = (cam.fade - st) / (en - st);
                    sf = (sf < 0.0f) ? 0.0f : ((sf > 1.0f) ? 1.0f : sf);
                    if (!(sf > 0.0f)) break;
                    majx = majx * sf; majy = majy * sf; minx = minx * sf; miny = miny * sf;
                }
                if (!finite4(majx, majy, minx, miny)) break;
                const float opacity = (float)((cw >> 24) & 0xffu) / 255.0f;
                op8 = (cw >> 24) & 0xffu;
                const float vcx = pos2d[0] / pos2d[3], vcy = pos2d[1] / pos2d[3];
                const float cx = ((vcx + 1.0f) * 0.5f) * (float)cam.W;
                const float cy = ((1.0f - vcy) * 0.5f) * (float)cam.H;
                const float m2 = majx * majx + majy * majy;
                const float n2 = minx * minx + miny * miny;
                const float im = 2.0f / m2, in = 2.0f / n2;
                area = fminf(0.77f * __builtin_amdgcn_sqrtf(m2 * n2), 65535.0f);
                Record r;
                r.cx = cx; r.cy = cy;
                r.ux = majx * im; r.uy = -majy * im;
                r.wx = minx * in; r.wy = -miny * in;
                if (!(finite4(r.ux, r.uy, r.wx, r.wy) && isfinite(cx) && isfinite(cy))) break;
                r.la = __log2f(opacity);
                r.rgb8 = cw & 0x00ffffffu;
                if (cam.sh_on && (int32_t)i > cam.band[0]) {
                    const uint32_t deg = (int32_t)i > cam.band[1] ? ((int32_t)i > cam.band[2] ? 3u : 2u) : 1u;
                    float cp[3];
#pragma unroll
                    for (int q = 0; q < 3; q++) {
                        float t = cam.view[q * 4 + 0] * cam.view[12];
                        t = t + cam.view[q * 4 + 1] * cam.view[13];
                        t = t + cam.view[q * 4 + 2] * cam.view[14];
                        cp[q] = -t;
                    }
                    float dvx = x - cp[0], dvy = y - cp[1], dvz = z - cp[2];
                    if (cam.sh_frame) {
                        const float e0 = (cam.shm[0] * dvx + cam.shm[1] * dvy) + cam.shm[2] * dvz;
                        const float e1 = (cam.shm[3] * dvx + cam.shm[4] * dvy) + cam.shm[5] * dvz;
                        const float e2 = (cam.shm[6] * dvx + cam.shm[7] * dvy) + cam.shm[8] * dvz;
                        dvx = e0; dvy = e1; dvz = e2;
                    }
                    const float dl = sqrtf((dvx * dvx + dvy * dvy) + dvz * dvz);
                    const float dxn = dvx / dl, dyn = dvy / dl, dzn = dvz / dl;
                    const uint32_t t = i - (uint32_t)(cam.band[0] + 1);
                    sc.shcol[i] = make_float4(eval_sh_texture(sc.sh_r, t, deg, dxn, dyn, dzn), eval_sh_texture(sc.sh_g, t, deg, dxn, dyn, dzn),
                                              eval_sh_texture(sc.sh_b, t, deg, dxn, dyn, dzn), 0.0f);
                    r.rgb8 = RGB8_IN_SHCOL;
                }
                const float ex = sqrtf(majx * majx + minx * minx);
                const float ey = sqrtf(majy * majy + miny * miny);
                float fx0 = floorf(cx - ex - 0.5f), fx1 = ceilf(cx + ex - 0.5f);
                float fy0 = floorf(cy - ey - 0.5f), fy1 = ceilf(cy + ey - 0.5f);
                fx0 = fmaxf(fx0, 0.0f); fy0 = fmaxf(fy0, 0.0f);
                fx1 = fminf(fx1, (float)(cam.W - 1)); fy1 = fminf(fy1, (float)(cam.H - 1));
                if (fx0 <= fx1 && (fx1 < (float)cam.band_px0 || fx0 >= (float)cam.band_px1)) break;
                float4* rp = reinterpret_cast<float4*>(rec + i);
                rp[0] = make_float4(r.cx, r.cy, r.ux, r.uy);
                rp[1] = make_float4(r.wx, r.wy, r.la, __uint_as_float(r.rgb8));
                if (fx0 > fx1 || fy0 > fy1) break;
                bb.x = (uint32_t)(int32_t)fx0 | ((uint32_t)(int32_t)fx1 << 16);
                bb.y = (uint32_t)(int32_t)fy0 | ((uint32_t)(int32_t)fy1 << 16);
            } while (0);
            if (bbox) bbox[i] = bb;
            if (frame) {
                const uint32_t rv = pack_bin_rect(bb.x, bb.y, bx_lo, bx_hi);
                keep = rv != RECT_NONE;
                if (!pack || keep) rect[i] = rv;
            }
            if ((bb.x & 0xffffu) <= (bb.x >> 16)) {
                vis++;
                const int tx0 = max((int)(bb.x & 0xffffu) / TILE, bx_lo * BIN_TILES), tx1 = min((int)(bb.x >> 16) / TILE, bx_hi * BIN_TILES - 1);
                const uint32_t nt = (uint32_t)((tx1 - tx0 + 1) * ((int)(bb.y >> 16) / TILE - (int)(bb.y & 0xffffu) / TILE + 1));
                tiles += nt;
                otiles += (op8 * min(nt, 4096u)) >> 4;
                omass += (op8 * (uint32_t)area) >> 8;
            }
        }
    }

#pragma unroll
    for (int off = 32; off > 0; off >>= 1) {
        dmin = min(dmin, __shfl_xor(dmin, off));
        dmax = max(dmax, __shfl_xor(dmax, off));
        vis += __shfl_xor(vis, off);
        tiles += __shfl_xor(tiles, off);
        otiles += __shfl_xor(otiles, off);
        omass += __shfl_xor(omass, off);
    }
    const int wave = threadIdx.x >> 6;
    uint32_t keep_rank = 0;
    if (pack) {
        const unsigned long long kb = __ballot(keep);
        keep_rank = __builtin_amdgcn_mbcnt_hi((uint32_t)(kb >> 32), __builtin_amdgcn_mbcnt_lo((uint32_t)kb, 0u));
        if ((threadIdx.x & 63) == 0) s_keep[wave] = (uint32_t)__popcll(kb);
    }
    if ((threadIdx.x & 63) == 0) { s_min[wave] = dmin; s_max[wave] = dmax; s_vis[wave] = vis; s_til[wave] = tiles; s_oti[wave] = otiles; s_oma[wave] = omass; }
    __syncthreads();
    if (pack) {
        uint32_t before = 0;
        for (int w = 0; w < wave; w++) before += s_keep[w];
        if (keep) {
            const uint32_t slot = blockIdx.x * PROJ_THREADS + before + keep_rank;
            depth[slot] = mydepth;
            kept_lane[slot] = (uint8_t)threadIdx.x;
        }
        if (threadIdx.x == 0) kept[blockIdx.x] = s_keep[0] + s_keep[1] + s_keep[2] + s_keep[3];
    }
    if (threadIdx.x == 0 && frame) {
        int32_t* slot = slots + (size_t)(blockIdx.x & (FRAME_SLOTS - 1)) * FRAME_SLOT_WORDS;
        atomicMin(&slot[0], min(min(s_min[0], s_min[1]), min(s_min[2], s_min[3])));
        atomicMax(&slot[1], max(max(s_max[0], s_max[1]), max(s_max[2], s_max[3])));
        if (do_project) {
            atomicAdd(reinterpret_cast<uint32_t*>(&slot[2]), s_vis[0] + s_vis[1] + s_vis[2] + s_vis[3]);
            atomicAdd(reinterpret_cast<uint32_t*>(&slot[3]), s_til[0] + s_til[1] + s_til[2] + s_til[3]);
            atomicAdd(reinterpret_cast<uint32_t*>(&slot[4]), s_oti[0] + s_oti[1] + s_oti[2] + s_oti[3]);
            atomicAdd(reinterpret_cast<uint32_t*>(&slot[5]), s_oma[0] + s_oma[1] + s_oma[2] + s_oma[3]);
        }
    }
}

constexpr int KEY_PER_THREAD = 4;
__global__ __launch_bounds__(PROJ_THREADS) void k_depth_key(SceneSoA sc, uint32_t n, float vp2, float vp6, float vp10,
                                                            int32_t* __restrict__ depth, int32_t* __restrict__ slots,
                                                            int32_t* __restrict__ slots_next)
{
    struct { float vp2, vp6, vp10; } cam = {vp2, vp6, vp10};
    if (blockIdx.x == 0 && threadIdx.x < FRAME_SLOTS) {
        slots_next[(size_t)threadIdx.x * FRAME_SLOT_WORDS + 0] = 0x7fffffff;
        slots_next[(size_t)threadIdx.x * FRAME_SLOT_WORDS + 1] = (int32_t)0x80000000;
    }
    __shared__ int32_t s_min[PROJ_THREADS / WAVE], s_max[PROJ_THREADS / WAVE];
    int32_t dmin = 0x7fffffff, dmax = (int32_t)0x80000000;
    float x[KEY_PER_THREAD], y[KEY_PER_THREAD], z[KEY_PER_THREAD];
#pragma unroll
    for (int k = 0; k < KEY_PER_THREAD; k++) {
        const uint32_t i = (blockIdx.x * KEY_PER_THREAD + k) * PROJ_THREADS + threadIdx.x;
        const bool in = i < n;
        x[k] = in ? sc.px[i] : 0.0f; y[k] = in ? sc.py[i] : 0.0f; z[k] = in ? sc.pz[i] : 0.0f;
    }
#pragma unroll
    for (int k = 0; k < KEY_PER_THREAD; k++) {
        const uint32_t i = (blockIdx.x * KEY_PER_THREAD + k) * PROJ_THREADS + threadIdx.x;
        if (i < n) {
            const float f0 = cam.vp2 * x[k];
            const float f1 = cam.vp6 * y[k];
            const float f2 = cam.vp10 * z[k];
            const int32_t d = (int32_t)(((f0 + f1) + f2) * 4096.0f);
            depth[i] = d;
            dmin = min(dmin, d); dmax = max(dmax, d);
        }
    }
#pragma unroll
    for (int off = 32; off > 0; off >>= 1) {
        dmin = min(dmin, __shfl_xor(dmin, off));
        dmax = max(dmax, __shfl_xor(dmax, off));
    }
    const int wave = threadIdx.x >> 6;
    if ((threadIdx.x & 63) == 0) { s_min[wave] = dmin; s_max[wave] = dmax; }
    __syncthreads();
    if (threadIdx.x == 0) {
        int32_t* slot = slots + (size_t)(blockIdx.x & (FRAME_SLOTS - 1)) * FRAME_SLOT_WORDS;
        int32_t mn = s_min[0], mx = s_max[0];
        for (int w = 1; w < PROJ_THREADS / WAVE; w++) { mn = min(mn, s_min[w]); mx = max(mx, s_max[w]); }
        atomicMin(&slot[0], mn);
        atomicMax(&slot[1], mx);
    }
}

void launch_depth_key(const SceneSoA& sc, uint32_t n, const CamParams& cam, int32_t* depth, int32_t* slots, int32_t* slots_next, hipStream_t s)
{
    if (!n) return;
    const uint32_t per = PROJ_THREADS * KEY_PER_THREAD;
    hipLaunchKernelGGL(k_depth_key, dim3((n + per - 1) / per), dim3(PROJ_THREADS), 0, s, sc, n, cam.vp2, cam.vp6, cam.vp10, depth, slots, slots_next);
}

void ProjectLaunch::bind()
{
    void* p[] = {&sc, &n, &cam, &do_project, &depth, &slots, &rec, &bbox, &rect, &overflow, &kept, &kept_lane};
    static_assert(sizeof p == sizeof ptrs, "one pointer per kernel argument");
    for (size_t k = 0; k < sizeof p / sizeof p[0]; k++) ptrs[k] = p[k];
}
const void* project_key_kernel() { return (const void*)k_project_key; }
dim3 project_key_grid(uint32_t n) { return dim3((n + PROJ_THREADS - 1) / PROJ_THREADS); }

void launch_project_key(ProjectLaunch& a, hipStream_t s)
{
    if (!a.n) return;
    a.bind();
    (void)hipLaunchKernel(project_key_kernel(), project_key_grid(a.n), dim3(PROJ_THREADS), a.ptrs, 0, s);
}

__global__ void k_begin_frame(CamParams cam, CamParams* __restrict__ dst, uint32_t* __restrict__ frame_words, uint32_t nwords,
                              int32_t* __restrict__ slots)
{
    for (uint32_t t = threadIdx.x; t < (uint32_t)FRAME_SLOTS * 8; t += blockDim.x) {
        const uint32_t k = t & 7u;
        slots[(size_t)(t >> 3) * FRAME_SLOT_WORDS + k] = k == 0 ? 0x7fffffff : k == 1 ? (int32_t)0x80000000 : 0;
    }
    constexpr uint32_t WORDS = sizeof(CamParams) / 4;
    const uint32_t* src = reinterpret_cast<const uint32_t*>(&cam);
    for (uint32_t w = threadIdx.x; w < WORDS; w += blockDim.x) reinterpret_cast<uint32_t*>(dst)[w] = src[w];
    for (uint32_t w = threadIdx.x; w < nwords; w += blockDim.x) frame_words[w] = w == 0 ? 0x7fffffffu : w == 1 ? 0x80000000u : 0u;
}

void launch_begin_frame(const CamParams& cam, CamParams* dst, uint32_t* frame_words, uint32_t nwords, int32_t* slots, hipStream_t s)
{
    static_assert(sizeof(CamParams) % 4 == 0, "camera is copied word by word");
    hipLaunchKernelGGL(k_begin_frame, dim3(1), dim3(256), 0, s, cam, dst, frame_words, nwords, slots);
}

}
```

### gsplat.js_amd/csrc/k_sort.hip

```cpp
#include "gsr_internal.h"

#include <algorithm>
#include <cstring>
#include <mutex>

namespace gsr {

GSR_BOUNDS_DECL(sort)
constexpr int SORT_THREADS = 256;

#ifdef GSR_KSTAMPS
__device__ unsigned int g_sort_stamps[2 * 4096 * 8];
#define KSTAMP(slot) do { if (threadIdx.x == 0 && blockIdx.x < 4096) g_sort_stamps[((FIRST ? 0 : 1) * 4096 + blockIdx.x) * 8 + (slot)] = (unsigned int)__builtin_amdgcn_s_memrealtime(); } while (0)
extern "C" int gsr_debug_sort_stamps(unsigned int* out) { return hipMemcpyFromSymbol(out, HIP_SYMBOL(g_sort_stamps), sizeof g_sort_stamps) == hipSuccess ? 0 : -1; }
#else
#define KSTAMP(slot)
#endif

__device__ __forceinline__ uint32_t lanes_below(uint64_t mask)
{
    return __builtin_amdgcn_mbcnt_hi((uint32_t)(mask >> 32), __builtin_amdgcn_mbcnt_lo((uint32_t)mask, 0u));
}

template <int BITS>
__device__ __forceinline__ uint64_t match_digit(uint32_t digit, bool valid)
{
    uint64_t m = __ballot(valid);
#pragma unroll
    for (int b = 0; b < BITS; b++) {
        const bool bit = (digit >> b) & 1u;
        const uint64_t bal = __ballot(bit);
        m &= bit ? bal : ~bal;
    }
    return valid ? m : 0ull;
}

constexpr int KS_THREADS = 1024;
constexpr int KS_WAVES = KS_THREADS / WAVE;
constexpr int KS_BATCH = 4;
__global__ __launch_bounds__(KS_THREADS) void k_kept_scan(const uint32_t* __restrict__ kept, uint32_t nb, uint32_t* __restrict__ koff,
                                                          uint32_t* __restrict__ count)
{
    extern __shared__ uint32_t s_sup[];
    const uint32_t nsup = (nb + WAVE - 1u) / WAVE;
    const uint32_t wave = threadIdx.x >> 6, lane = threadIdx.x & 63u;
    for (uint32_t sb = wave; sb < nsup; sb += KS_WAVES * KS_BATCH) {
        uint32_t v[KS_BATCH];
#pragma unroll
        for (int k = 0; k < KS_BATCH; k++) {
            const uint32_t b = (sb + k * KS_WAVES) * WAVE + lane;
            v[k] = b < nb ? kept[b] : 0u;
        }
#pragma unroll
        for (int k = 0; k < KS_BATCH; k++) {
            uint32_t t = v[k];
#pragma unroll
            for (int off = 32; off > 0; off >>= 1) t += __shfl_xor(t, off);
            if (lane == 0 && sb + k * KS_WAVES < nsup) s_sup[sb + k * KS_WAVES] = t;
        }
    }
    __syncthreads();
    if (wave == 0) {
        uint32_t carry = 0;
        for (uint32_t base = 0; base < nsup; base += WAVE) {
            const uint32_t v = base + lane < nsup ? s_sup[base + lane] : 0u;
            uint32_t inc = v;
#pragma unroll
            for (int off = 1; off < WAVE; off <<= 1) {
                const uint32_t u = __shfl_up(inc, off);
                if ((int)lane >= off) inc += u;
            }
            if (base + lane < nsup) s_sup[base + lane] = carry + inc - v;
            carry += __shfl(inc, WAVE - 1);
        }
        if (lane == 0) { koff[nb] = carry; *count = carry; }
    }
    __syncthreads();
    for (uint32_t sb = wave; sb < nsup; sb += KS_WAVES * KS_BATCH) {
        uint32_t v[KS_BATCH];
#pragma unroll
        for (int k = 0; k < KS_BATCH; k++) {
            const uint32_t b = (sb + k * KS_WAVES) * WAVE + lane;
            v[k] = b < nb ? kept[b] : 0u;
        }
#pragma unroll
        for (int k = 0; k < KS_BATCH; k++) {
            const uint32_t b = (sb + k * KS_WAVES) * WAVE + lane;
            uint32_t inc = v[k];
#pragma unroll
            for (int off = 1; off < WAVE; off <<= 1) {
                const uint32_t u = __shfl_up(inc, off);
                if ((int)lane >= off) inc += u;
            }
            if (b < nb) koff[b] = s_sup[sb + k * KS_WAVES] + inc - v[k];
        }
    }
}

constexpr int BG_BLOCKS = 4;
__global__ __launch_bounds__(BG_BLOCKS * WAVE) void k_band_gather(const int32_t* __restrict__ depth, const uint8_t* __restrict__ kept_lane,
                                                                 const uint32_t* __restrict__ kept, const uint32_t* __restrict__ koff,
                                                                 uint32_t n, uint32_t nb, int32_t* __restrict__ depth_out,
                                                                 uint32_t* __restrict__ idx_out)
{
    const uint32_t b = blockIdx.x * BG_BLOCKS + (threadIdx.x >> 6);
    if (b >= nb) return;
    const uint32_t c = kept[b], o = koff[b];
    const uint32_t lane = threadIdx.x & 63u;
#pragma unroll
    for (uint32_t k = 0; k < PROJ_THREADS / WAVE; k++) {
        const uint32_t t = k * WAVE + lane;
        if (t < c) {
            const uint32_t slot = b * PROJ_THREADS + t;
            GSR_BOUND(sort, 4, slot, n);
            depth_out[o + t] = depth[slot];
            idx_out[o + t] = b * PROJ_THREADS + kept_lane[slot];
        }
    }
}

__global__ __launch_bounds__(SORT_THREADS) void k_quantise_hist(const int32_t* __restrict__ depth,
                                                                const int32_t* __restrict__ slots,
                                                                int32_t* __restrict__ minmax_out, uint32_t n,
                                                                uint32_t keys_per_block, const uint32_t* __restrict__ live,
                                                                uint32_t* __restrict__ keys,
                                                                uint32_t* __restrict__ block_hist, int hist_shift, int hist_bins)
{
    __shared__ uint32_t h_lo[RADIX_HI_BINS];
    __shared__ int32_t s_mm[2][SORT_THREADS / WAVE];
    for (int d = threadIdx.x; d < hist_bins; d += SORT_THREADS) h_lo[d] = 0;
    const uint32_t begin = blockIdx.x * keys_per_block;
    if (live) n = *live;
    const uint32_t end = min(begin + keys_per_block, n);
    constexpr int QH_PRE = 8;
    int32_t pre[QH_PRE];
#pragma unroll
    for (int k = 0; k < QH_PRE; k++) {
        const uint32_t i = begin + threadIdx.x + (uint32_t)k * SORT_THREADS;
        pre[k] = i < end ? depth[i] : 0;
    }
    int32_t mn = 0x7fffffff, mx = (int32_t)0x80000000;
    if (threadIdx.x < FRAME_SLOTS) {
        mn = slots[(size_t)threadIdx.x * FRAME_SLOT_WORDS];
        mx = slots[(size_t)threadIdx.x * FRAME_SLOT_WORDS + 1];
    }
#pragma unroll
    for (int off = 32; off > 0; off >>= 1) {
        mn = min(mn, __shfl_xor(mn, off));
        mx = max(mx, __shfl_xor(mx, off));
    }
    if ((threadIdx.x & 63) == 0) { s_mm[0][threadIdx.x >> 6] = mn; s_mm[1][threadIdx.x >> 6] = mx; }
    __syncthreads();
    int32_t minDepth = s_mm[0][0], maxDepth = s_mm[1][0];
#pragma unroll
    for (int w = 1; w < SORT_THREADS / WAVE; w++) { minDepth = min(minDepth, s_mm[0][w]); maxDepth = max(maxDepth, s_mm[1][w]); }
    if (blockIdx.x == 0 && threadIdx.x == 0) { minmax_out[0] = minDepth; minmax_out[1] = maxDepth; }

    const bool degenerate = (maxDepth == minDepth);
    const float depthInv = degenerate ? 0.0f : (float)DEPTH_RANGE / (float)(maxDepth - minDepth);

    auto quantise = [&](uint32_t i, int32_t d) {
        const uint32_t rel = (uint32_t)d - (uint32_t)minDepth;
        uint32_t q = degenerate ? 0u : (uint32_t)((float)rel * depthInv);
        q = min(q, DEPTH_RANGE);
        keys[i] = q;
        atomicAdd(&h_lo[(q >> hist_shift) & (uint32_t)(hist_bins - 1)], 1u);
    };
#pragma unroll
    for (int k = 0; k < QH_PRE; k++) {
        const uint32_t i = begin + threadIdx.x + (uint32_t)k * SORT_THREADS;
        if (i < end) quantise(i, pre[k]);
    }
    for (uint32_t i = begin + threadIdx.x + QH_PRE * SORT_THREADS; i < end; i += SORT_THREADS) quantise(i, depth[i]);
    __syncthreads();
    for (int d = threadIdx.x; d < hist_bins; d += SORT_THREADS) block_hist[(size_t)blockIdx.x * hist_bins + d] = h_lo[d];
}

__global__ __launch_bounds__(SORT_THREADS) void k_hist_hi(const uint32_t* __restrict__ keys, const uint32_t* __restrict__ count,
                                                          uint32_t keys_per_block, uint32_t* __restrict__ block_hist)
{
    const uint32_t n = *count;
    __shared__ uint32_t h[RADIX_HI_BINS];
    for (int d = threadIdx.x; d < RADIX_HI_BINS; d += SORT_THREADS) h[d] = 0;
    __syncthreads();
    const uint32_t begin = blockIdx.x * keys_per_block;
    const uint32_t end = min(begin + keys_per_block, n);
    for (uint32_t i = begin + threadIdx.x; i < end; i += SORT_THREADS) atomicAdd(&h[keys[i] >> RADIX_LO_BITS], 1u);
    __syncthreads();
    for (int d = threadIdx.x; d < RADIX_HI_BINS; d += SORT_THREADS) block_hist[(size_t)blockIdx.x * RADIX_HI_BINS + d] = h[d];
}

constexpr int CS_THREADS = 512;
constexpr int CS_COLS = 16;
constexpr int CS_SLOTS = CS_THREADS / CS_COLS;
constexpr int CS_BATCH = 8;

constexpr int CS_KEEP = 16;
constexpr int CS_KEEP_LONG = 40;

template <int KEEP>
__global__ __launch_bounds__(CS_THREADS) void k_column_scan(uint32_t* __restrict__ table, uint32_t* __restrict__ total,
                                                            int ncols, uint32_t nrows, const uint32_t* __restrict__ live, uint32_t live_unit)
{
    if (live) nrows = min(nrows, (*live + live_unit - 1u) / live_unit);
    __shared__ uint32_t s_sum[CS_SLOTS][CS_COLS];
    const int c = threadIdx.x & (CS_COLS - 1);
    const int slot = threadIdx.x / CS_COLS;
    const int col = blockIdx.x * CS_COLS + c;
    const bool ok = col < ncols;
    const uint32_t per = (nrows + CS_SLOTS - 1) / CS_SLOTS;
    const uint32_t r0 = min((uint32_t)slot * per, nrows), r1 = min(r0 + per, nrows);
    uint32_t* p = table + (size_t)r0 * ncols + (ok ? col : 0);

    uint32_t sum = 0;
    uint32_t kept[KEEP ? KEEP : 1];
    if (KEEP) {
#pragma unroll
        for (int k = 0; k < KEEP; k++) kept[k] = (ok && r0 + k < r1) ? p[(size_t)k * ncols] : 0u;
#pragma unroll
        for (int k = 0; k < KEEP; k++) sum += kept[k];
    } else if (ok) {
        for (uint32_t r = r0; r < r1; r += CS_BATCH) {
            uint32_t v[CS_BATCH];
#pragma unroll
            for (int k = 0; k < CS_BATCH; k++) v[k] = (r + k < r1) ? p[(size_t)(r - r0 + k) * ncols] : 0u;
#pragma unroll
            for (int k = 0; k < CS_BATCH; k++) sum += v[k];
        }
    }
    s_sum[slot][c] = sum;
    __syncthreads();
    uint32_t base = 0, tot = 0;
#pragma unroll 8
    for (int k = 0; k < CS_SLOTS; k++) {
        const uint32_t v = s_sum[k][c];
        base += (k < slot) ? v : 0u;
        tot += v;
    }
    if (ok) {
        uint32_t run = base;
        if (KEEP) {
#pragma unroll
            for (int k = 0; k < KEEP; k++) {
                if (r0 + k < r1) p[(size_t)k * ncols] = run;
                run += kept[k];
            }
        } else {
            for (uint32_t r = r0; r < r1; r += CS_BATCH) {
                uint32_t v[CS_BATCH];
#pragma unroll
                for (int k = 0; k < CS_BATCH; k++) v[k] = (r + k < r1) ? p[(size_t)(r - r0 + k) * ncols] : 0u;
#pragma unroll
                for (int k = 0; k < CS_BATCH; k++) {
                    if (r + k < r1) p[(size_t)(r - r0 + k) * ncols] = run;
                    run += v[k];
                }
            }
        }
        if (slot == 0) total[col] = tot;
    }
}

void launch_column_scan(uint32_t* table, uint32_t* total, int ncols, uint32_t nrows, hipStream_t s, const uint32_t* live, uint32_t live_unit)
{
    const dim3 grid((ncols + CS_COLS - 1) / CS_COLS), block(CS_THREADS);
    if (nrows <= (uint32_t)CS_SLOTS * CS_KEEP) hipLaunchKernelGGL(k_column_scan<CS_KEEP>, grid, block, 0, s, table, total, ncols, nrows, live, live_unit);
    else if (nrows <= (uint32_t)CS_SLOTS * CS_KEEP_LONG) hipLaunchKernelGGL(k_column_scan<CS_KEEP_LONG>, grid, block, 0, s, table, total, ncols, nrows, live, live_unit);
    else hipLaunchKernelGGL(k_column_scan<0>, grid, block, 0, s, table, total, ncols, nrows, live, live_unit);
}

constexpr int SCAT_THREADS = 1024;
constexpr int SCAT_WAVES = SCAT_THREADS / WAVE;
constexpr int SCAT_MAX_STEPS = 8;
constexpr uint32_t NARROW_KEYS_PER_BLOCK = 2048;
constexpr int scat_max_steps(int waves) { return waves == SCAT_WAVES ? SCAT_MAX_STEPS : (int)NARROW_KEYS_PER_BLOCK / (waves * WAVE); }
constexpr uint32_t LOCAL_CHUNK = 4096;

constexpr size_t scatter_lds_bytes(int bits, uint32_t keys_per_block, int waves = SCAT_WAVES)
{
    return (size_t)(waves * (1 << bits) + 2 * (1 << bits) + 3 * ((1 << bits) / WAVE) + 2 * keys_per_block) * sizeof(uint32_t);
}

template <int BITS, int SHIFT, bool FIRST, bool PAY = false, int WAVES = SCAT_WAVES>
__global__ __launch_bounds__(WAVES * WAVE) void k_scatter(const uint32_t* __restrict__ keys_in,
                                                          const uint32_t* __restrict__ idx_in, uint32_t n_in,
                                                          uint32_t* __restrict__ count,
                                                          uint32_t keys_per_block, const uint32_t* __restrict__ base,
                                                          const uint32_t* __restrict__ total,
                                                          uint32_t* __restrict__ keys_out, uint32_t* __restrict__ idx_out,
                                                          uint32_t* __restrict__ max_bucket,
                                                          const uint32_t* __restrict__ pay_in = nullptr, uint32_t* __restrict__ pay_out = nullptr,
                                                          uint4* __restrict__ chunk_tab = nullptr)
{
    constexpr int BINS = 1 << BITS;
    constexpr int THREADS = WAVES * WAVE, MAX_STEPS = scat_max_steps(WAVES);
    static_assert(BINS <= THREADS, "one digit per thread");
    const bool band = FIRST && idx_in != nullptr;
    const uint32_t n = (FIRST && !band) ? n_in : *count;
    extern __shared__ uint32_t s_scat[];
    uint32_t (*cnt)[BINS] = reinterpret_cast<uint32_t (*)[BINS]>(s_scat);
    uint32_t* gdelta = s_scat + WAVES * BINS;
    uint32_t* lstart = gdelta + BINS;
    uint32_t* wsum = lstart + BINS;
    uint32_t* lkey = wsum + 3 * (BINS / WAVE);
    uint32_t* lidx = lkey + keys_per_block;
    const int lane = threadIdx.x & 63, wave = threadIdx.x >> 6;
    const uint32_t blk = xcd_group_remap(blockIdx.x, gridDim.x);
    if ((unsigned long long)blk * keys_per_block >= n && blockIdx.x != 0) return;
    KSTAMP(0);
    uint32_t tot = 0, wg_base = 0;
    if (threadIdx.x < BINS) {
        tot = total[threadIdx.x];
        wg_base = base[(size_t)blk * BINS + threadIdx.x];
    }
    for (int d = threadIdx.x; d < WAVES * BINS; d += THREADS) (&cnt[0][0])[d] = 0;
    __syncthreads();
    KSTAMP(1);

    const uint32_t per_wave = keys_per_block / WAVES;
    const uint32_t steps = per_wave / WAVE;
    const uint32_t wbegin = blk * keys_per_block + wave * per_wave;
    const uint32_t wend = min(wbegin + per_wave, n);

    uint32_t key[MAX_STEPS], src[MAX_STEPS];
    uint32_t pay[PAY ? MAX_STEPS : 1], pos[PAY ? MAX_STEPS : 1];
#pragma unroll
    for (int k = 0; k < MAX_STEPS; k++) {
        const uint32_t i = wbegin + k * WAVE + lane;
        const bool in = (uint32_t)k < steps && i < wend;
        key[k] = in ? keys_in[i] : 0xffffffffu;
        src[k] = (FIRST && !band) ? i : (in ? idx_in[i] : 0u);
        if (band) GSR_BOUND(sort, 4, src[k], n_in);
        if (PAY) pay[k] = in ? pay_in[band ? src[k] : i] : 0u;
    }
#pragma unroll
    for (int k = 0; k < MAX_STEPS; k++)
        if (key[k] != 0xffffffffu) atomicAdd(&cnt[wave][(key[k] >> SHIFT) & (BINS - 1)], 1u);
    __syncthreads();
    KSTAMP(2);
    uint32_t H = 0, incl_t = 0, incl_h = 0;
    if (threadIdx.x < BINS) {
        const int d = threadIdx.x;
#pragma unroll
        for (int w = 0; w < WAVES; w++) {
            const uint32_t c = cnt[w][d];
            cnt[w][d] = H;
            H += c;
        }
        incl_t = tot; incl_h = H;
#pragma unroll
        for (int off = 1; off < WAVE; off <<= 1) {
            const uint32_t u = __shfl_up(incl_t, off), v = __shfl_up(incl_h, off);
            if (lane >= off) { incl_t += u; incl_h += v; }
        }
        if (lane == WAVE - 1) { wsum[wave] = incl_t; wsum[BINS / WAVE + wave] = incl_h; }
        if (max_bucket && blockIdx.x == 0) {
            uint32_t mx = tot;
#pragma unroll
            for (int off = 32; off > 0; off >>= 1) mx = max(mx, __shfl_xor(mx, off));
            if (lane == 0) wsum[2 * (BINS / WAVE) + wave] = mx;
        }
    }
    __syncthreads();
    if (max_bucket && blockIdx.x == 0 && threadIdx.x == 0) {
        uint32_t mx = 0;
        for (int w = 0; w < BINS / WAVE; w++) mx = max(mx, wsum[2 * (BINS / WAVE) + w]);
        *max_bucket = mx;
    }
    KSTAMP(3);
    if (threadIdx.x < BINS) {
        const int d = threadIdx.x;
        uint32_t run_t = incl_t - tot, run_h = incl_h - H;
        for (int w = 0; w < wave; w++) { run_t += wsum[w]; run_h += wsum[BINS / WAVE + w]; }
        if (FIRST && blockIdx.x == 0 && d == BINS - 1) *count = run_t + tot;
        lstart[d] = run_h;
        gdelta[d] = run_t + wg_base - run_h;
    }
    if (chunk_tab && blockIdx.x == 0) {
        __shared__ uint32_t s_cw[BINS / WAVE];
        const uint32_t nch = threadIdx.x < BINS ? (tot + LOCAL_CHUNK - 1) / LOCAL_CHUNK : 0u;
        uint32_t inc = nch;
#pragma unroll
        for (int off = 1; off < WAVE; off <<= 1) {
            const uint32_t u = __shfl_up(inc, off);
            if (lane >= off) inc += u;
        }
        if (threadIdx.x < BINS && lane == WAVE - 1) s_cw[wave] = inc;
        __syncthreads();
        if (threadIdx.x < BINS) {
            uint32_t first = inc - nch, run_t = incl_t - tot, all = 0;
            for (int w = 0; w < BINS / WAVE; w++) {
                if (w < wave) { first += s_cw[w]; run_t += wsum[w]; }
                all += s_cw[w];
            }
            for (uint32_t ch = 0; ch < nch; ch++) chunk_tab[1 + first + ch] = make_uint4((uint32_t)threadIdx.x, ch, run_t, tot);
            if (threadIdx.x == 0) chunk_tab[0] = make_uint4(all, 0u, 0u, 0u);
        }
    }
    __syncthreads();
    KSTAMP(4);
    uint32_t* wc = cnt[wave];
#pragma unroll
    for (int k = 0; k < MAX_STEPS; k++) {
        if ((uint32_t)k >= steps) break;
        const bool valid = key[k] != 0xffffffffu;
        const uint32_t digit = (key[k] >> SHIFT) & (BINS - 1);
        const uint64_t m = match_digit<BITS>(digit, valid);
        const uint32_t rank = lanes_below(m);
        const uint32_t before = wc[valid ? digit : 0];
        __builtin_amdgcn_fence(__ATOMIC_SEQ_CST, "wavefront", "local");
        __builtin_amdgcn_wave_barrier();
        if (valid && rank == 0) wc[digit] = before + (uint32_t)__popcll(m);
        __builtin_amdgcn_fence(__ATOMIC_SEQ_CST, "wavefront", "local");
        __builtin_amdgcn_wave_barrier();
        if (valid) {
            const uint32_t p = lstart[digit] + before + rank;
            GSR_BOUND(sort, 1, p, keys_per_block);
            lkey[p] = key[k];
            lidx[p] = src[k];
            if (PAY) pos[k] = p;
        }
    }
    __syncthreads();
    const uint32_t nlocal = lstart[BINS - 1] + cnt[WAVES - 1][BINS - 1];
    for (uint32_t p = threadIdx.x; p < nlocal; p += THREADS) {
        const uint32_t kv = lkey[p];
        const uint32_t dst = gdelta[(kv >> SHIFT) & (BINS - 1)] + p;
        GSR_BOUND(sort, 0, dst, n);
        GSR_BOUND(sort, 3, kv, DEPTH_RANGE + 1u);
        if (keys_out) keys_out[dst] = kv;
        idx_out[dst] = lidx[p];
    }
    if (PAY) {
        __syncthreads();
#pragma unroll
        for (int k = 0; k < MAX_STEPS; k++) {
            if ((uint32_t)k >= steps) break;
            if (key[k] != 0xffffffffu) lidx[pos[k]] = pay[k];
        }
        __syncthreads();
        for (uint32_t p = threadIdx.x; p < nlocal; p += THREADS) pay_out[gdelta[(lkey[p] >> SHIFT) & (BINS - 1)] + p] = lidx[p];
    }
#ifdef GSR_KSTAMPS
    __syncthreads();
    KSTAMP(5);
#endif
}

inline uint32_t local_sort_grid(uint32_t n) { return (n + LOCAL_CHUNK - 1) / LOCAL_CHUNK + RADIX_HI_BINS / 2 + 1; }

template <int WAVES>
__global__ __launch_bounds__(WAVES * WAVE) void k_local_sort(const uint32_t* __restrict__ keys, const uint32_t* __restrict__ idx,
                                                              const uint4* __restrict__ chunk_tab,
                                                              uint32_t* __restrict__ depth_index,
                                                              const uint32_t* __restrict__ pay_in, uint32_t* __restrict__ pay_out)
{
    constexpr int BINS = RADIX_LO_BINS;
    constexpr int LOCAL_THREADS = WAVES * WAVE, LOCAL_WAVES = WAVES, LOCAL_STEPS = (int)LOCAL_CHUNK / LOCAL_THREADS;
    static_assert(BINS <= LOCAL_THREADS && LOCAL_STEPS * LOCAL_THREADS == (int)LOCAL_CHUNK, "one digit per thread, whole steps");
    __shared__ uint32_t cnt[LOCAL_WAVES][BINS];
    __shared__ uint32_t tot[BINS];
    __shared__ uint32_t bef[BINS];
    __shared__ uint32_t wsum[BINS / WAVE];
    const int lane = threadIdx.x & 63, wave = threadIdx.x >> 6;
    if (blockIdx.x >= chunk_tab[0].x) return;
    const uint4 me = chunk_tab[1 + blockIdx.x];
    for (int d = threadIdx.x; d < LOCAL_WAVES * BINS; d += LOCAL_THREADS) (&cnt[0][0])[d] = 0;
    if (threadIdx.x < BINS) { tot[threadIdx.x] = 0; bef[threadIdx.x] = 0; }
    __syncthreads();
    const uint32_t chunk = me.y, s0 = me.z, sz = me.w;
    const uint32_t cbeg = chunk * LOCAL_CHUNK, cend = min(cbeg + LOCAL_CHUNK, sz);

    const uint32_t wbegin = cbeg + wave * (LOCAL_STEPS * WAVE), wend = min(wbegin + LOCAL_STEPS * WAVE, cend);
    uint32_t key[LOCAL_STEPS], src[LOCAL_STEPS], pay[LOCAL_STEPS];
#pragma unroll
    for (int k = 0; k < LOCAL_STEPS; k++) {
        const uint32_t i = wbegin + k * WAVE + lane;
        const bool in = i < wend;
        key[k] = in ? (keys[s0 + i] & (BINS - 1)) : 0xffffffffu;
        src[k] = in ? idx[s0 + i] : 0u;
        pay[k] = (in && pay_out) ? pay_in[s0 + i] : 0u;
    }
#pragma unroll
    for (int k = 0; k < LOCAL_STEPS; k++)
        if (key[k] != 0xffffffffu) atomicAdd(&cnt[wave][key[k]], 1u);
    constexpr int CB = 8;
    for (uint32_t i0 = threadIdx.x; i0 < sz; i0 += CB * LOCAL_THREADS) {
        uint32_t v[CB];
#pragma unroll
        for (int j = 0; j < CB; j++) {
            const uint32_t i = i0 + j * LOCAL_THREADS;
            v[j] = (i < sz && (i < cbeg || i >= cend)) ? keys[s0 + i] : 0xffffffffu;
        }
#pragma unroll
        for (int j = 0; j < CB; j++) {
            const uint32_t i = i0 + j * LOCAL_THREADS;
            if (v[j] != 0xffffffffu) atomicAdd(i < cbeg ? &bef[v[j] & (BINS - 1)] : &tot[v[j] & (BINS - 1)], 1u);
        }
    }
    __syncthreads();
    uint32_t H = 0, incl = 0, td = 0;
    if (threadIdx.x < BINS) {
        const int d = threadIdx.x;
#pragma unroll
        for (int w = 0; w < LOCAL_WAVES; w++) {
            const uint32_t cv = cnt[w][d];
            cnt[w][d] = H;
            H += cv;
        }
        td = tot[d] + bef[d] + H;
        incl = td;
#pragma unroll
        for (int off = 1; off < WAVE; off <<= 1) {
            const uint32_t u = __shfl_up(incl, off);
            if (lane >= off) incl += u;
        }
        if (lane == WAVE - 1) wsum[wave] = incl;
    }
    __syncthreads();
    if (threadIdx.x < BINS) {
        uint32_t run = incl - td;
        for (int w = 0; w < wave; w++) run += wsum[w];
        tot[threadIdx.x] = run + bef[threadIdx.x];
    }
    __syncthreads();
    uint32_t* wc = cnt[wave];
#pragma unroll
    for (int k = 0; k < LOCAL_STEPS; k++) {
        const bool valid = key[k] != 0xffffffffu;
        const uint32_t digit = valid ? key[k] : 0u;
        const uint64_t m = match_digit<RADIX_LO_BITS>(digit, valid);
        const uint32_t rank = lanes_below(m);
        const uint32_t earlier = wc[digit];
        __builtin_amdgcn_fence(__ATOMIC_SEQ_CST, "wavefront", "local");
        __builtin_amdgcn_wave_barrier();
        if (valid && rank == 0) wc[digit] = earlier + (uint32_t)__popcll(m);
        __builtin_amdgcn_fence(__ATOMIC_SEQ_CST, "wavefront", "local");
        __builtin_amdgcn_wave_barrier();
        if (valid) {
            GSR_BOUND(sort, 2, tot[digit] + earlier + rank, sz);
            depth_index[s0 + tot[digit] + earlier + rank] = src[k];
            if (pay_out) pay_out[s0 + tot[digit] + earlier + rank] = pay[k];
        }
    }
}

constexpr uint32_t KPB_SMALL = 2048, KPB_LARGE = 4096, KPB_SMALL_MAX_ROWS = 3u << 20;
constexpr uint32_t BUCKET_ORDER_MAX_N = 3u << 20;
constexpr uint32_t LOCAL_BUCKET_LIMIT = 48u << 10;
constexpr uint32_t CHUNK_TAB_SPARE = 2;

inline uint32_t keys_per_block_of(uint32_t rows, const SortKnobs& k) { return k.sort_kpb ? k.sort_kpb : rows <= KPB_SMALL_MAX_ROWS ? KPB_SMALL : KPB_LARGE; }
inline uint32_t ceil_div(uint32_t a, uint32_t b) { return (uint32_t)(((uint64_t)a + b - 1u) / b); }

SortSizes sort_sizes(uint32_t rows, const SortKnobs& k)
{
    SortSizes z;
    z.keys_per_block = keys_per_block_of(rows, k);
    z.block_hist = (size_t)std::max(ceil_div(rows, z.keys_per_block), 1u) * RADIX_HI_BINS;
    z.chunk_tab = 4 * ((size_t)1 + local_sort_grid(rows) + CHUNK_TAB_SPARE);
    z.kept = (size_t)ceil_div(rows, PROJ_THREADS) + 1;
    z.koff = (size_t)ceil_div(rows, PROJ_THREADS) + 2;
    return z;
}

SortPlan plan_sort(uint32_t n, uint32_t rows, uint32_t front_waves, bool render, bool cull, uint32_t largest_bucket, const SortKnobs& k)
{
    SortPlan p;
    memset(&p, 0, sizeof p);
    p.keys_per_block = keys_per_block_of(rows, k);
    if (!n) return p;
    const bool bucket = k.sort_order >= 0 ? k.sort_order == 1 : (n <= BUCKET_ORDER_MAX_N && largest_bucket <= LOCAL_BUCKET_LIMIT);
    const bool narrow = bucket && front_waves == FRONT_WAVES_NARROW && p.keys_per_block == NARROW_KEYS_PER_BLOCK;
    p.form = !bucket ? SORT_LSD : narrow ? SORT_BUCKET_NARROW : SORT_BUCKET_WIDE;
    p.waves = narrow ? FRONT_WAVES_NARROW : FRONT_WAVES_WIDE;
    p.carry = (render && k.rect_carry && (k.rect_carry_bucket || !bucket)) ? 1u : 0u;
    p.band = (render && cull) ? 1u : 0u;
    p.blocks = ceil_div(n, p.keys_per_block);
    p.proj_blocks = ceil_div(n, PROJ_THREADS);
    if (bucket) {
        p.lds_first = (uint32_t)scatter_lds_bytes(RADIX_HI_BITS, p.keys_per_block, (int)p.waves);
        p.local_grid = local_sort_grid(n);
    } else {
        p.lds_first = (uint32_t)scatter_lds_bytes(RADIX_LO_BITS, p.keys_per_block, (int)p.waves);
        p.lds_last = (uint32_t)scatter_lds_bytes(RADIX_HI_BITS, p.keys_per_block, (int)p.waves);
    }
    return p;
}

extern "C" int gsr_debug_sort_plan(unsigned int n, unsigned int rows, unsigned int front_waves, int render, int cull, unsigned int largest_bucket,
                                    int sort_order, unsigned int sort_kpb, int rect_carry, int rect_carry_bucket, SortPlan* out)
{
    *out = plan_sort(n, rows, front_waves, render != 0, cull != 0, largest_bucket,
                     SortKnobs{sort_order, sort_kpb, rect_carry ? 1u : 0u, rect_carry_bucket ? 1u : 0u});
    return (int)sizeof(SortPlan);
}
extern "C" int gsr_debug_sort_sizes(unsigned int rows, unsigned int sort_kpb, unsigned long long* out)
{
    const SortSizes z = sort_sizes(rows, SortKnobs{-1, sort_kpb, 1u, 0u});
    out[0] = z.keys_per_block; out[1] = z.block_hist; out[2] = z.chunk_tab; out[3] = z.kept; out[4] = z.koff;
    return 5;
}

using ScatterFn = void (*)(const uint32_t*, const uint32_t*, uint32_t, uint32_t*, uint32_t, const uint32_t*, const uint32_t*, uint32_t*, uint32_t*,
                           uint32_t*, const uint32_t*, uint32_t*, uint4*);
using LocalSortFn = void (*)(const uint32_t*, const uint32_t*, const uint4*, uint32_t*, const uint32_t*, uint32_t*);
struct ScatterKernel { ScatterFn fn; uint32_t waves; int bits; bool first, pay; };
static const ScatterKernel SCATTER_KERNELS[] = {
    {k_scatter<RADIX_LO_BITS, 0, true>, FRONT_WAVES_WIDE, RADIX_LO_BITS, true, false},
    {k_scatter<RADIX_LO_BITS, 0, true, true>, FRONT_WAVES_WIDE, RADIX_LO_BITS, true, true},
    {k_scatter<RADIX_HI_BITS, RADIX_LO_BITS, false>, FRONT_WAVES_WIDE, RADIX_HI_BITS, false, false},
    {k_scatter<RADIX_HI_BITS, RADIX_LO_BITS, false, true>, FRONT_WAVES_WIDE, RADIX_HI_BITS, false, true},
    {k_scatter<RADIX_HI_BITS, RADIX_LO_BITS, true>, FRONT_WAVES_WIDE, RADIX_HI_BITS, true, false},
    {k_scatter<RADIX_HI_BITS, RADIX_LO_BITS, true, true>, FRONT_WAVES_WIDE, RADIX_HI_BITS, true, true},
    {k_scatter<RADIX_HI_BITS, RADIX_LO_BITS, true, false, FRONT_WAVES_NARROW>, FRONT_WAVES_NARROW, RADIX_HI_BITS, true, false},
    {k_scatter<RADIX_HI_BITS, RADIX_LO_BITS, true, true, FRONT_WAVES_NARROW>, FRONT_WAVES_NARROW, RADIX_HI_BITS, true, true},
};
struct LocalSortKernel { LocalSortFn fn; uint32_t waves; };
static const LocalSortKernel LOCAL_SORT_KERNELS[] = {{k_local_sort<SCAT_WAVES>, FRONT_WAVES_WIDE}, {k_local_sort<FRONT_WAVES_NARROW>, FRONT_WAVES_NARROW}};

static const ScatterKernel& scatter_kernel(int bits, bool first, bool pay, uint32_t waves)
{
    for (const ScatterKernel& k : SCATTER_KERNELS)
        if (k.bits == bits && k.first == first && k.pay == pay && k.waves == waves) return k;
    return SCATTER_KERNELS[0];
}
static LocalSortFn local_sort_kernel(uint32_t waves) { return LOCAL_SORT_KERNELS[waves == LOCAL_SORT_KERNELS[0].waves ? 0 : 1].fn; }

static void raise_scatter_lds()
{
    static std::once_flag once[64];
    int dev = 0;
    (void)hipGetDevice(&dev);
    std::call_once(once[dev >= 0 && dev < 64 ? dev : 0], [] {
        for (const ScatterKernel& k : SCATTER_KERNELS)
            (void)hipFuncSetAttribute((const void*)k.fn, hipFuncAttributeMaxDynamicSharedMemorySize,
                                      (int)scatter_lds_bytes(k.bits, k.waves * WAVE * scat_max_steps((int)k.waves), (int)k.waves));
        (void)hipGetLastError();
    });
}

void launch_sort(const SortBuffers& b, uint32_t n, hipStream_t s)
{
    const SortPlan& p = b.plan;
    if (p.form == SORT_NONE) return;
    raise_scatter_lds();
    const dim3 grid(p.blocks), block(SORT_THREADS);
    uint32_t* total_lo = b.digit_total;
    uint32_t* total_hi = b.digit_total + RADIX_LO_BINS;
    uint32_t* band_idx = p.band ? b.depth_index : nullptr;
    const uint32_t* live = p.band ? b.count : nullptr;
    const int32_t* depth_in = p.band ? reinterpret_cast<const int32_t*>(b.keys_tmp) : b.depth;
    if (p.band) {
        const uint32_t nb = p.proj_blocks;
        hipLaunchKernelGGL(k_kept_scan, dim3(1), dim3(KS_THREADS), (size_t)((nb + WAVE - 1u) / WAVE) * sizeof(uint32_t), s, b.kept, nb, b.koff, b.count);
        hipLaunchKernelGGL(k_band_gather, dim3((nb + BG_BLOCKS - 1) / BG_BLOCKS), dim3(BG_BLOCKS * WAVE), 0, s, b.depth, b.kept_lane, b.kept,
                           (const uint32_t*)b.koff, n, nb, reinterpret_cast<int32_t*>(b.keys_tmp), band_idx);
    }
    const bool bucket = p.form != SORT_LSD;
    const int bits = bucket ? RADIX_HI_BITS : RADIX_LO_BITS;
    uint32_t* total = bucket ? total_hi : total_lo;
    uint4* tab = bucket ? reinterpret_cast<uint4*>(b.chunk_tab) : nullptr;
    hipLaunchKernelGGL(k_quantise_hist, grid, block, 0, s, depth_in, b.slots, b.minmax, n, p.keys_per_block, live, b.keys, b.block_hist,
                       bucket ? RADIX_LO_BITS : 0, 1 << bits);
    launch_column_scan(b.block_hist, total, 1 << bits, p.blocks, s, live, p.keys_per_block);
    const ScatterFn first = scatter_kernel(bits, true, p.carry, p.waves).fn;
    hipLaunchKernelGGL(first, grid, dim3(p.waves * WAVE), p.lds_first, s, (const uint32_t*)b.keys,
                       (const uint32_t*)band_idx, n, b.count, p.keys_per_block, (const uint32_t*)b.block_hist, (const uint32_t*)total, b.keys_tmp,
                       b.idx_tmp, bucket ? b.max_bucket : nullptr, p.carry ? b.rect : nullptr, p.carry ? b.rect_tmp : nullptr, tab);
    if (bucket) {
        const LocalSortFn local = local_sort_kernel(p.waves);
        hipLaunchKernelGGL(local, dim3(p.local_grid), dim3(p.waves * WAVE), 0, s, (const uint32_t*)b.keys_tmp, (const uint32_t*)b.idx_tmp,
                           (const uint4*)tab, b.depth_index, (const uint32_t*)b.rect_tmp, b.rects_out);
        return;
    }
    hipLaunchKernelGGL(k_hist_hi, grid, block, 0, s, (const uint32_t*)b.keys_tmp, (const uint32_t*)b.count, p.keys_per_block, b.block_hist);
    launch_column_scan(b.block_hist, total_hi, RADIX_HI_BINS, p.blocks, s, live, p.keys_per_block);
    const ScatterFn last = scatter_kernel(RADIX_HI_BITS, false, p.carry, p.waves).fn;
    hipLaunchKernelGGL(last, grid, dim3(p.waves * WAVE), p.lds_last, s, (const uint32_t*)b.keys_tmp,
                       (const uint32_t*)b.idx_tmp, n, b.count, p.keys_per_block, (const uint32_t*)b.block_hist, (const uint32_t*)total_hi,
                       (uint32_t*)nullptr, b.depth_index, b.max_bucket, p.carry ? (const uint32_t*)b.rect_tmp : nullptr, b.rects_out, (uint4*)nullptr);
}

}
```

Before: 5814.

## Split projection across sort kernels so it rides along with sort passes

```diff
diff --git a/gsplat.js_amd/csrc/gsr_api.cpp b/gsplat.js_amd/csrc/gsr_api.cpp
--- a/gsplat.js_amd/csrc/gsr_api.cpp
+++ b/gsplat.js_amd/csrc/gsr_api.cpp
@@ -40,6 +40,15 @@
         else bad = std::string("GSR_FRONT_WAVES must be ") + std::to_string(FRONT_WAVES_NARROW) + " or " + std::to_string(FRONT_WAVES_WIDE) + ", not \"" + e + "\"";
     }
     if (const char* e = getenv("GSR_DEPTH_SKIP")) k.depth_skip = atoi(e) != 0;
+    if (const char* e = getenv("GSR_PROJECT_RIDE")) k.project_ride = atoi(e) != 0 ? 1 : 0;
+    if (const char* e = getenv("GSR_RIDE_SPLIT")) {
+        unsigned v[RIDE_HOSTS];
+        std::string t(e);
+        std::replace(t.begin(), t.end(), ':', ',');
+        if (sscanf(t.c_str(), "%u,%u,%u,%u", &v[0], &v[1], &v[2], &v[3]) == RIDE_HOSTS && (v[0] | v[1] | v[2] | v[3]) && std::max(std::max(v[0], v[1]), std::max(v[2], v[3])) <= 1000u)
+            for (int h = 0; h < RIDE_HOSTS; h++) k.ride_split[h] = v[h];
+        else bad = std::string("GSR_RIDE_SPLIT must be four shares a,b,c,d of at most 1000, not all 0, not \"") + e + "\"";
+    }
     return k;
 }
 
diff --git a/gsplat.js_amd/csrc/gsr_ctx.h b/gsplat.js_amd/csrc/gsr_ctx.h
--- a/gsplat.js_amd/csrc/gsr_ctx.h
+++ b/gsplat.js_amd/csrc/gsr_ctx.h
@@ -81,6 +81,8 @@
     uint32_t seg_len = 0;
     uint32_t sort_kpb = 0;
     uint32_t front_waves = 0;
+    int project_ride = -1;
+    uint32_t ride_split[gsr::RIDE_HOSTS] = {0, 0, 0, 0};
     bool depth_skip = true;
 };
 
@@ -256,6 +258,7 @@
         uint32_t rows = 0;
         int parity = 0;
         gsr::SortPlan plan{};
+        gsr::RidePlan ride{};
     } sort;
 
     struct Bin {
@@ -295,10 +298,13 @@
         bool enabled = true;
         hipGraph_t graph = nullptr;
         hipGraphExec_t exec = nullptr;
-        hipGraphNode_t project = nullptr;
+        hipGraphNode_t cam_node[1 + gsr::RIDE_HOSTS] = {};
+        int cam_launch[1 + gsr::RIDE_HOSTS] = {};
+        int cam_nodes = 0;
         gsr::FrameArgs key;
     } graph;
     gsr::ProjectLaunch proj{};
+    gsr::RideChain ride{};
 
     struct Timing {
         static constexpr int EV_RING = 128;
@@ -403,7 +409,10 @@
 
 inline SortKnobs sort_knobs_of(const gsr_ctx* c)
 {
-    return SortKnobs{c->knobs.sort_order, c->knobs.sort_kpb, c->knobs.rect_carry ? 1u : 0u, c->knobs.rect_carry_bucket ? 1u : 0u};
+    SortKnobs k{c->knobs.sort_order, c->knobs.sort_kpb, c->knobs.rect_carry ? 1u : 0u, c->knobs.rect_carry_bucket ? 1u : 0u};
+    k.project_ride = c->knobs.project_ride;
+    for (int h = 0; h < RIDE_HOSTS; h++) k.ride_split[h] = c->knobs.ride_split[h];
+    return k;
 }
 
 int alloc_bins(gsr_ctx* c, bool fresh_items = false);
diff --git a/gsplat.js_amd/csrc/gsr_frame.cpp b/gsplat.js_amd/csrc/gsr_frame.cpp
--- a/gsplat.js_amd/csrc/gsr_frame.cpp
+++ b/gsplat.js_amd/csrc/gsr_frame.cpp
@@ -15,7 +15,8 @@
 {
     memset(&a, 0, sizeof a);
     const BinGrid g = make_grid(c);
-    const SortPlan sp = plan_sort(c->scene->n, c->sort.rows, front_waves_of(c), render, band_is_partial(g), largest_bucket_reported(c), sort_knobs_of(c));
+    RidePlan rp;
+    const SortPlan sp = plan_sort(c->scene->n, c->sort.rows, front_waves_of(c), render, band_is_partial(g), largest_bucket_reported(c), sort_knobs_of(c), &rp);
     FrameState* fs = c->words.fstate;
     a.render = render;
     a.n = c->scene->n;
@@ -53,6 +54,7 @@
     sb.koff = sp.band ? c->sort.koff.p : nullptr;
     sb.count = &fs->sorted_count;
     sb.plan = sp;
+    sb.ride = rp;
     sb.max_bucket = reinterpret_cast<uint32_t*>(c->words.mailbox_dev + 1);
     sb.chunk_tab = c->sort.chunk_tab;
     sb.rect_tmp = c->sort.rect_tmp;
@@ -127,6 +129,10 @@
     p.kept = a.proj.kept;
     p.kept_lane = a.proj.kept_lane;
     p.bind();
+    if (a.sort.ride.on) {
+        bind_ride_chain(c->ride, a.sort, a.n, a.proj.sc, a.proj.depth, a.proj.rec, a.proj.rect, a.proj.slots, a.proj.overflow);
+        set_ride_camera(c->ride, c->cam);
+    }
 }
 
 int enqueue_chain(gsr_ctx* c, const FrameArgs& a, bool timing)
@@ -135,14 +141,16 @@
     hipEvent_t* ev = c->timing.ev;
     if (timing) HIP_TRY(c, hipEventRecord(ev[EV_BEGIN], s));
     if (a.n) {
-        if (a.render) launch_project_key(c->proj, s);
+        if (a.sort.ride.on) launch_ride_key(c->ride, s);
+        else if (a.render) launch_project_key(c->proj, s);
         else launch_depth_key(a.proj.sc, a.n, c->cam, a.proj.depth, a.proj.slots, a.slots_next, s);
     } else {
         HIP_TRY(c, hipMemsetD32Async((hipDeviceptr_t)&a.sort.minmax[0], 0x7fffffff, 1, s));
         HIP_TRY(c, hipMemsetD32Async((hipDeviceptr_t)&a.sort.minmax[1], (int)0x80000000u, 1, s));
     }
     if (timing) HIP_TRY(c, hipEventRecord(ev[EV_PROJECT], s));
-    launch_sort(a.sort, a.n, s);
+    if (a.sort.ride.on) launch_ride_sort(c->ride, s);
+    else launch_sort(a.sort, a.n, s);
     if (timing) HIP_TRY(c, hipEventRecord(ev[EV_SORT], s));
     if (a.render) {
         if (!a.n) {
@@ -158,6 +166,16 @@
     return GSR_OK;
 }
 
+int camera_launches(const gsr_ctx* c, const FrameArgs& a, const void** fn, int* launch)
+{
+    if (!a.n) return 0;
+    if (!a.sort.ride.on) { fn[0] = project_key_kernel(); launch[0] = -1; return 1; }
+    int count = 0;
+    for (int k = 0; k < 1 + RIDE_HOSTS; k++)
+        if (c->ride.launch[k].cam) { fn[count] = c->ride.launch[k].fn; launch[count] = k; count++; }
+    return count;
+}
+
 bool capture_graph(gsr_ctx* c, const FrameArgs& a)
 {
     hipStream_t s = c->stream;
@@ -165,37 +183,58 @@
     const int r = enqueue_chain(c, a, false);
     hipGraph_t gph = nullptr;
     bool ok = (hipStreamEndCapture(s, &gph) == hipSuccess) && r == GSR_OK && gph;
-    hipGraphNode_t project = nullptr;
-    if (ok && a.n) {
+    const void* fn[1 + RIDE_HOSTS];
+    int launch[1 + RIDE_HOSTS];
+    hipGraphNode_t found[1 + RIDE_HOSTS] = {};
+    const int want = camera_launches(c, a, fn, launch);
+    if (ok && want) {
         size_t nn = 0;
         ok = hipGraphGetNodes(gph, nullptr, &nn) == hipSuccess && nn > 0;
         std::vector<hipGraphNode_t> nodes(nn);
         if (ok) ok = hipGraphGetNodes(gph, nodes.data(), &nn) == hipSuccess;
-        for (size_t k = 0; ok && k < nn && !project; k++) {
+        for (size_t k = 0; ok && k < nn; k++) {
             hipGraphNodeType ty;
             hipKernelNodeParams kp{};
-            if (hipGraphNodeGetType(nodes[k], &ty) == hipSuccess && ty == hipGraphNodeTypeKernel &&
-                hipGraphKernelNodeGetParams(nodes[k], &kp) == hipSuccess && kp.func == project_key_kernel())
-                project = nodes[k];
-        }
-        ok = ok && project != nullptr;
+            if (hipGraphNodeGetType(nodes[k], &ty) != hipSuccess || ty != hipGraphNodeTypeKernel || hipGraphKernelNodeGetParams(nodes[k], &kp) != hipSuccess) continue;
+            for (int w = 0; w < want; w++)
+                if (kp.func == fn[w] && !found[w]) found[w] = nodes[k];
+        }
+        for (int w = 0; w < want; w++) ok = ok && found[w] != nullptr;
     }
     if (ok) ok = hipGraphInstantiate(&c->graph.exec, gph, nullptr, nullptr, 0) == hipSuccess;
-    if (ok) { c->graph.graph = gph; c->graph.project = project; memcpy(&c->graph.key, &a, sizeof a); }
+    if (ok) {
+        c->graph.graph = gph;
+        c->graph.cam_nodes = want;
+        for (int w = 0; w < want; w++) { c->graph.cam_node[w] = found[w]; c->graph.cam_launch[w] = launch[w]; }
+        memcpy(&c->graph.key, &a, sizeof a);
+    }
     else if (gph) (void)hipGraphDestroy(gph);
     return ok;
 }
 
 bool set_graph_camera(gsr_ctx* c)
 {
-    hipKernelNodeParams kp{};
-    kp.func = const_cast<void*>(project_key_kernel());
-    kp.gridDim = project_key_grid(c->proj.n);
-    kp.blockDim = dim3(PROJ_THREADS);
-    kp.sharedMemBytes = 0;
-    kp.kernelParams = c->proj.ptrs;
-    kp.extra = nullptr;
-    return hipGraphExecKernelNodeSetParams(c->graph.exec, c->graph.project, &kp) == hipSuccess;
+    for (int w = 0; w < c->graph.cam_nodes; w++) {
+        hipKernelNodeParams kp{};
+        const int l = c->graph.cam_launch[w];
+        if (l < 0) {
+            kp.func = const_cast<void*>(project_key_kernel());
+            kp.gridDim = project_key_grid(c->proj.n);
+            kp.blockDim = dim3(PROJ_THREADS);
+            kp.sharedMemBytes = 0;
+            kp.kernelParams = c->proj.ptrs;
+        } else {
+            RideLaunch& rl = c->ride.launch[l];
+            kp.func = const_cast<void*>(rl.fn);
+            kp.gridDim = rl.grid;
+            kp.blockDim = rl.block;
+            kp.sharedMemBytes = rl.lds;
+            kp.kernelParams = rl.ptrs;
+        }
+        kp.extra = nullptr;
+        if (hipGraphExecKernelNodeSetParams(c->graph.exec, c->graph.cam_node[w], &kp) != hipSuccess) return false;
+    }
+    return true;
 }
 
 int check_frame_words(gsr_ctx* c, bool* overflowed)
@@ -305,7 +344,7 @@
 {
     if (c->graph.exec) (void)hipGraphExecDestroy(c->graph.exec);
     if (c->graph.graph) (void)hipGraphDestroy(c->graph.graph);
-    c->graph.exec = nullptr; c->graph.graph = nullptr; c->graph.project = nullptr;
+    c->graph.exec = nullptr; c->graph.graph = nullptr; c->graph.cam_nodes = 0;
 }
 
 int enqueue_frame(gsr_ctx* c, bool render)
@@ -354,7 +393,7 @@
             drop_graph(c);
             ok = capture_graph(c, a);
         }
-        else if (c->graph.project) ok = set_graph_camera(c);
+        else ok = set_graph_camera(c);
         if (!ok) {
             (void)hipGetLastError();
             drop_graph(c);
@@ -368,6 +407,7 @@
     if (!replayed) { if (int r = enqueue_chain(c, a, timing)) return r; }
     if (!render && a.n) c->sort.parity ^= 1;
     c->sort.plan = a.sort.plan;
+    c->sort.ride = a.sort.ride;
     if (timing) t.pending++;
     t.recorded = timing;
     t.render = render;
@@ -442,6 +482,13 @@
     *out = c->sort.plan;
     return GSR_OK;
 }
+extern "C" int gsr_debug_last_ride_plan(gsr_ctx* c, RidePlan* out)
+{
+    if (!c || !out) return GSR_ERR_ARG;
+    if (!c->have_sort) return fail(c, GSR_ERR_ARG, "no sort has run yet");
+    *out = c->sort.ride;
+    return GSR_OK;
+}
 
 extern "C" int gsr_debug_last_blend_plan(gsr_ctx* c, BlendPlan* out)
 {
diff --git a/gsplat.js_amd/csrc/gsr_internal.h b/gsplat.js_amd/csrc/gsr_internal.h
--- a/gsplat.js_amd/csrc/gsr_internal.h
+++ b/gsplat.js_amd/csrc/gsr_internal.h
@@ -122,6 +122,24 @@
 const void* project_key_kernel();
 dim3 project_key_grid(uint32_t n);
 void launch_project_key(ProjectLaunch& a, hipStream_t s);
+const void* depth_key_frame_kernel();
+dim3 depth_key_grid(uint32_t n);
+
+
+constexpr int RIDE_HOSTS = 4;
+struct RideSlice { uint32_t first, count; };
+struct RidePlan {
+    uint32_t on;
+    RideSlice slice[RIDE_HOSTS];
+};
+struct RideArgs {
+    SceneSoA sc; uint32_t n;
+    uint32_t host_grid;
+    uint32_t first, count;
+    CamParams cam;
+    Record* rec; uint32_t* rect;
+    int32_t* slots;
+};
 
 constexpr uint32_t FRONT_WAVES_WIDE = 16, FRONT_WAVES_NARROW = 8;
 
@@ -146,8 +164,13 @@
     uint32_t keys_per_block;
     size_t block_hist, chunk_tab, kept, koff;
 };
-struct SortKnobs { int32_t sort_order; uint32_t sort_kpb, rect_carry, rect_carry_bucket; };
-SortPlan plan_sort(uint32_t n, uint32_t rows, uint32_t front_waves, bool render, bool cull, uint32_t largest_bucket, const SortKnobs& k);
+struct SortKnobs {
+    int32_t sort_order; uint32_t sort_kpb, rect_carry, rect_carry_bucket;
+    int32_t project_ride = -1;
+    uint32_t ride_split[RIDE_HOSTS] = {0, 0, 0, 0};
+};
+SortPlan plan_sort(uint32_t n, uint32_t rows, uint32_t front_waves, bool render, bool cull, uint32_t largest_bucket, const SortKnobs& k,
+                   RidePlan* ride = nullptr);
 SortSizes sort_sizes(uint32_t rows, const SortKnobs& k);
 
 struct SortBuffers {
@@ -166,12 +189,35 @@
     uint32_t* koff;
     uint32_t* count;
     SortPlan plan;
+    RidePlan ride;
     uint32_t* max_bucket;
     uint32_t* chunk_tab;
     uint32_t* rect_tmp;
     uint32_t* rects_out;
 };
 void launch_sort(const SortBuffers& b, uint32_t n, hipStream_t s);
+struct RideLaunch {
+    const void* fn; dim3 grid, block; uint32_t lds;
+    bool cam;
+    void* ptrs[16];
+};
+struct RideChain {
+    struct Key { SceneSoA sc; uint32_t n; float vp2, vp6, vp10; int32_t* depth; int32_t* slots; uint32_t* overflow; } key;
+    struct Quant { const int32_t* depth; const int32_t* slots; int32_t* minmax; uint32_t n, keys_per_block; const uint32_t* live; uint32_t* keys;
+                   uint32_t* block_hist; int hist_shift, hist_bins; } quant;
+    struct Scan { uint32_t* table; uint32_t* total; int ncols; uint32_t nrows; const uint32_t* live; uint32_t live_unit; } scan;
+    struct Scatter { const uint32_t* keys_in; const uint32_t* idx_in; uint32_t n_in; uint32_t* count; uint32_t keys_per_block; const uint32_t* base;
+                     const uint32_t* total; uint32_t* keys_out; uint32_t* idx_out; uint32_t* max_bucket; const uint32_t* pay_in; uint32_t* pay_out;
+                     uint4* chunk_tab; } scatter;
+    struct Local { const uint32_t* keys; const uint32_t* idx; const uint4* chunk_tab; uint32_t* depth_index; const uint32_t* pay_in; uint32_t* pay_out; } local;
+    RideArgs ra[RIDE_HOSTS];
+    RideLaunch launch[1 + RIDE_HOSTS];
+};
+void bind_ride_chain(RideChain& r, const SortBuffers& b, uint32_t n, const SceneSoA& sc, int32_t* depth, Record* rec, uint32_t* rect, int32_t* slots,
+                     uint32_t* overflow);
+void set_ride_camera(RideChain& r, const CamParams& cam);
+void launch_ride_key(const RideChain& r, hipStream_t s);
+void launch_ride_sort(const RideChain& r, hipStream_t s);
 void launch_column_scan(uint32_t* table, uint32_t* total, int ncols, uint32_t nrows, hipStream_t s, const uint32_t* live = nullptr, uint32_t live_unit = 1);
 
 struct BinGrid {
diff --git a/gsplat.js_amd/csrc/k_project.hip b/gsplat.js_amd/csrc/k_project.hip
--- a/gsplat.js_amd/csrc/k_project.hip
+++ b/gsplat.js_amd/csrc/k_project.hip
@@ -1,4 +1,5 @@
 #include "gsr_internal.h"
+#include "k_project_body.h"
 
 namespace gsr {
 
@@ -37,75 +38,6 @@
 {
     if (!n) return;
     hipLaunchKernelGGL(k_repack_positions, dim3((n + 255) / 256), dim3(256), 0, s, positions, n, px, py, pz);
-}
-
-__device__ __forceinline__ void mat3_mul(const float* a, const float* b, float* r)
-{
-#pragma unroll
-    for (int c = 0; c < 3; c++)
-#pragma unroll
-        for (int ro = 0; ro < 3; ro++) {
-            float s = a[0 * 3 + ro] * b[c * 3 + 0];
-            s = s + a[1 * 3 + ro] * b[c * 3 + 1];
-            s = s + a[2 * 3 + ro] * b[c * 3 + 2];
-            r[c * 3 + ro] = s;
-        }
-}
-
-__device__ __forceinline__ float half_bits_to_float(uint32_t h)
-{
-    return (float)__builtin_bit_cast(_Float16, (unsigned short)(h & 0xffffu));
-}
-
-__device__ __forceinline__ bool finite4(float a, float b, float c, float d)
-{
-    return isfinite(a) && isfinite(b) && isfinite(c) && isfinite(d);
-}
-
-__device__ __forceinline__ float eval_sh_channel(const float* k, uint32_t deg, float x, float y, float z)
-{
-    constexpr float C0 = 0.28209479177387814f, C1 = 0.4886025119029199f;
-    constexpr float C2_0 = 1.0925484305920792f, C2_1 = -1.0925484305920792f, C2_2 = 0.31539156525252005f,
-                    C2_3 = -1.0925484305920792f, C2_4 = 0.5462742152960396f;
-    constexpr float C3_0 = -0.5900435899266435f, C3_1 = 2.890611442640554f, C3_2 = -0.4570457994644658f,
-                    C3_3 = 0.3731763325901154f, C3_4 = -0.4570457994644658f, C3_5 = 1.445305721320277f,
-                    C3_6 = -0.5900435899266435f;
-    float r = C0 * k[0];
-    if (deg > 0) {
-        r = r - ((((C1 * y) * k[1]) + ((C1 * z) * k[2])) - ((C1 * x) * k[3]));
-        if (deg > 1) {
-            const float xx = x * x, yy = y * y, zz = z * z, xy = x * y, yz = y * z, xz = x * z;
-            float s2 = (C2_0 * xy) * k[4];
-            s2 = s2 + (C2_1 * yz) * k[5];
-            s2 = s2 + (C2_2 * ((2.0f * zz - xx) - yy)) * k[6];
-            s2 = s2 + (C2_3 * xz) * k[7];
-            s2 = s2 + (C2_4 * (xx - yy)) * k[8];
-            r = r + s2;
-            if (deg > 2) {
-                float s3 = ((C3_0 * y) * (3.0f * xx - yy)) * k[9];
-                s3 = s3 + ((C3_1 * xy) * z) * k[10];
-                s3 = s3 + ((C3_2 * y) * ((4.0f * zz - xx) - yy)) * k[11];
-                s3 = s3 + ((C3_3 * z) * ((2.0f * zz - 3.0f * xx) - 3.0f * yy)) * k[12];
-                s3 = s3 + ((C3_4 * x) * ((4.0f * zz - xx) - yy)) * k[13];
-                s3 = s3 + ((C3_5 * z) * (xx - yy)) * k[14];
-                s3 = s3 + ((C3_6 * x) * (xx - 3.0f * yy)) * k[15];
-                r = r + s3;
-            }
-        }
-    }
-    r = r + 0.5f;
-    r = (r > 0.0f) ? r : 0.0f;
-    return (r < 1.0f) ? r : 1.0f;
-}
-
-__device__ __forceinline__ float eval_sh_texture(const uint32_t* __restrict__ tex, uint32_t t, uint32_t deg, float x, float y, float z)
-{
-    const uint4 a = reinterpret_cast<const uint4*>(tex)[2 * (size_t)t], b = reinterpret_cast<const uint4*>(tex)[2 * (size_t)t + 1];
-    const uint32_t w[8] = {a.x, a.y, a.z, a.w, b.x, b.y, b.z, b.w};
-    float k[16];
-#pragma unroll
-    for (int j = 0; j < 8; j++) { k[2 * j] = half_bits_to_float(w[j]); k[2 * j + 1] = half_bits_to_float(w[j] >> 16); }
-    return eval_sh_channel(k, deg, x, y, z);
 }
 
 __global__ __launch_bounds__(PROJ_THREADS) void k_project_key(SceneSoA sc, uint32_t n, CamParams cam,
@@ -140,148 +72,16 @@
         dmin = d; dmax = d;
 
         if (do_project) {
-            uint2 bb = make_uint2(BBOX_INVISIBLE_X, BBOX_INVISIBLE_Y);
             uint32_t op8 = 0;
             float area = 0.0f;
-            do {
-                float camv[4], pos2d[4];
-#pragma unroll
-                for (int r = 0; r < 4; r++) {
-                    float s = cam.view[0 * 4 + r] * x;
-                    s = s + cam.view[1 * 4 + r] * y;
-                    s = s + cam.view[2 * 4 + r] * z;
-                    s = s + cam.view[3 * 4 + r];
-                    camv[r] = s;
-                }
-#pragma unroll
-                for (int r = 0; r < 4; r++) {
-                    float s = cam.proj[0 * 4 + r] * camv[0];
-                    s = s + cam.proj[1 * 4 + r] * camv[1];
-                    s = s + cam.proj[2 * 4 + r] * camv[2];
-                    s = s + cam.proj[3 * 4 + r] * camv[3];
-                    pos2d[r] = s;
-                }
-                const float clip = 1.2f * pos2d[3];
-                if (pos2d[2] < -pos2d[3] || pos2d[0] < -clip || pos2d[0] > clip || pos2d[1] < -clip || pos2d[1] > clip) break;
-
-                const uint32_t c0 = sc.cov0[i], c1 = sc.cov1[i], c2 = sc.cov2[i], cw = sc.rgba[i];
-                const float u1x = half_bits_to_float(c0), u1y = half_bits_to_float(c0 >> 16);
-                const float u2x = half_bits_to_float(c1), u2y = half_bits_to_float(c1 >> 16);
-                const float u3x = half_bits_to_float(c2), u3y = half_bits_to_float(c2 >> 16);
-                const float Vrk[9] = {u1x, u1y, u2x, u1y, u2y, u3x, u2x, u3x, u3y};
-                const float zz = camv[2] * camv[2];
-                const float J[9] = {cam.fx / camv[2], 0.f, -(cam.fx * camv[0]) / zz,
-                                    0.f, -cam.fy / camv[2], (cam.fy * camv[1]) / zz,
-                                    0.f, 0.f, 0.f};
-                const float V3t[9] = {cam.view[0], cam.view[4], cam.view[8], cam.view[1], cam.view[5],
-                                      cam.view[9], cam.view[2], cam.view[6], cam.view[10]};
-                float T[9], Tt[9], TtV[9], cov2d[9];
-                mat3_mul(V3t, J, T);
-#pragma unroll
-                for (int c = 0; c < 3; c++)
-#pragma unroll
-                    for (int r = 0; r < 3; r++) Tt[c * 3 + r] = T[r * 3 + c];
-                mat3_mul(Tt, Vrk, TtV);
-                mat3_mul(TtV, T, cov2d);
-                const float a = cov2d[0] + 0.3f;
-                const float b = cov2d[1];
-                const float c = cov2d[4] + 0.3f;
-                const float det = a * c - b * b;
-                if (det == 0.0f) break;
-                const float mid = (a + c) / 2.0f;
-                const float rad = mid * mid - det;
-                const float sq = sqrtf((0.1f < rad) ? rad : 0.1f);
-                const float lambda1 = mid + sq;
-                const float lambda2 = mid - sq;
-                if (lambda2 < 0.0f) break;
-                const float dvx = b, dvy = lambda1 - a;
-                const float len = sqrtf(dvx * dvx + dvy * dvy);
-                const float dgx = dvx / len, dgy = dvy / len;
-                float smaj = sqrtf(2.0f * lambda1), smin = sqrtf(2.0f * lambda2);
-                smaj = (1024.0f < smaj) ? 1024.0f : smaj;
-                smin = (1024.0f < smin) ? 1024.0f : smin;
-                float majx = smaj * dgx, majy = smaj * dgy;
-                float minx = smin * dgy, miny = smin * -dgx;
-                if (cam.use_fade) {
-                    const float depthNorm = (pos2d[2] / pos2d[3] + 1.0f) / 2.0f;
-                    const float nearv = 0.1f, farv = 100.0f;
-                    const float normalizedDepth = (2.0f * nearv) / (farv + nearv - depthNorm * (farv - nearv));
-                    float st = normalizedDepth - 0.1f; st = (st > 0.0f) ? st : 0.0f;
-                    float en = normalizedDepth + 0.1f; en = (en < 1.0f) ? en : 1.0f;
-                    float sf = (cam.fade - st) / (en - st);
-                    sf = (sf < 0.0f) ? 0.0f : ((sf > 1.0f) ? 1.0f : sf);
-                    if (!(sf > 0.0f)) break;
-                    majx = majx * sf; majy = majy * sf; minx = minx * sf; miny = miny * sf;
-                }
-                if (!finite4(majx, majy, minx, miny)) break;
-                const float opacity = (float)((cw >> 24) & 0xffu) / 255.0f;
-                op8 = (cw >> 24) & 0xffu;
-                const float vcx = pos2d[0] / pos2d[3], vcy = pos2d[1] / pos2d[3];
-                const float cx = ((vcx + 1.0f) * 0.5f) * (float)cam.W;
-                const float cy = ((1.0f - vcy) * 0.5f) * (float)cam.H;
-                const float m2 = majx * majx + majy * majy;
-                const float n2 = minx * minx + miny * miny;
-                const float im = 2.0f / m2, in = 2.0f / n2;
-                area = fminf(0.77f * __builtin_amdgcn_sqrtf(m2 * n2), 65535.0f);
-                Record r;
-                r.cx = cx; r.cy = cy;
-                r.ux = majx * im; r.uy = -majy * im;
-                r.wx = minx * in; r.wy = -miny * in;
-                if (!(finite4(r.ux, r.uy, r.wx, r.wy) && isfinite(cx) && isfinite(cy))) break;
-                r.la = __log2f(opacity);
-                r.rgb8 = cw & 0x00ffffffu;
-                if (cam.sh_on && (int32_t)i > cam.band[0]) {
-                    const uint32_t deg = (int32_t)i > cam.band[1] ? ((int32_t)i > cam.band[2] ? 3u : 2u) : 1u;
-                    float cp[3];
-#pragma unroll
-                    for (int q = 0; q < 3; q++) {
-                        float t = cam.view[q * 4 + 0] * cam.view[12];
-                        t = t + cam.view[q * 4 + 1] * cam.view[13];
-                        t = t + cam.view[q * 4 + 2] * cam.view[14];
-                        cp[q] = -t;
-                    }
-                    float dvx = x - cp[0], dvy = y - cp[1], dvz = z - cp[2];
-                    if (cam.sh_frame) {
-                        const float e0 = (cam.shm[0] * dvx + cam.shm[1] * dvy) + cam.shm[2] * dvz;
-                        const float e1 = (cam.shm[3] * dvx + cam.shm[4] * dvy) + cam.shm[5] * dvz;
-                        const float e2 = (cam.shm[6] * dvx + cam.shm[7] * dvy) + cam.shm[8] * dvz;
-                        dvx = e0; dvy = e1; dvz = e2;
-                    }
-                    const float dl = sqrtf((dvx * dvx + dvy * dvy) + dvz * dvz);
-                    const float dxn = dvx / dl, dyn = dvy / dl, dzn = dvz / dl;
-                    const uint32_t t = i - (uint32_t)(cam.band[0] + 1);
-                    sc.shcol[i] = make_float4(eval_sh_texture(sc.sh_r, t, deg, dxn, dyn, dzn), eval_sh_texture(sc.sh_g, t, deg, dxn, dyn, dzn),
-                                              eval_sh_texture(sc.sh_b, t, deg, dxn, dyn, dzn), 0.0f);
-                    r.rgb8 = RGB8_IN_SHCOL;
-                }
-                const float ex = sqrtf(majx * majx + minx * minx);
-                const float ey = sqrtf(majy * majy + miny * miny);
-                float fx0 = floorf(cx - ex - 0.5f), fx1 = ceilf(cx + ex - 0.5f);
-                float fy0 = floorf(cy - ey - 0.5f), fy1 = ceilf(cy + ey - 0.5f);
-                fx0 = fmaxf(fx0, 0.0f); fy0 = fmaxf(fy0, 0.0f);
-                fx1 = fminf(fx1, (float)(cam.W - 1)); fy1 = fminf(fy1, (float)(cam.H - 1));
-                if (fx0 <= fx1 && (fx1 < (float)cam.band_px0 || fx0 >= (float)cam.band_px1)) break;
-                float4* rp = reinterpret_cast<float4*>(rec + i);
-                rp[0] = make_float4(r.cx, r.cy, r.ux, r.uy);
-                rp[1] = make_float4(r.wx, r.wy, r.la, __uint_as_float(r.rgb8));
-                if (fx0 > fx1 || fy0 > fy1) break;
-                bb.x = (uint32_t)(int32_t)fx0 | ((uint32_t)(int32_t)fx1 << 16);
-                bb.y = (uint32_t)(int32_t)fy0 | ((uint32_t)(int32_t)fy1 << 16);
-            } while (0);
+            const uint2 bb = project_splat(sc, cam, i, x, y, z, rec, op8, area);
             if (bbox) bbox[i] = bb;
             if (frame) {
                 const uint32_t rv = pack_bin_rect(bb.x, bb.y, bx_lo, bx_hi);
                 keep = rv != RECT_NONE;
                 if (!pack || keep) rect[i] = rv;
             }
-            if ((bb.x & 0xffffu) <= (bb.x >> 16)) {
-                vis++;
-                const int tx0 = max((int)(bb.x & 0xffffu) / TILE, bx_lo * BIN_TILES), tx1 = min((int)(bb.x >> 16) / TILE, bx_hi * BIN_TILES - 1);
-                const uint32_t nt = (uint32_t)((tx1 - tx0 + 1) * ((int)(bb.y >> 16) / TILE - (int)(bb.y & 0xffffu) / TILE + 1));
-                tiles += nt;
-                otiles += (op8 * min(nt, 4096u)) >> 4;
-                omass += (op8 * (uint32_t)area) >> 8;
-            }
+            count_splat(bb, op8, area, bx_lo, bx_hi, vis, tiles, otiles, omass);
         }
     }
 
@@ -327,12 +127,15 @@
 }
 
 constexpr int KEY_PER_THREAD = 4;
+template <bool FRAME>
 __global__ __launch_bounds__(PROJ_THREADS) void k_depth_key(SceneSoA sc, uint32_t n, float vp2, float vp6, float vp10,
                                                             int32_t* __restrict__ depth, int32_t* __restrict__ slots,
                                                             int32_t* __restrict__ slots_next)
 {
     struct { float vp2, vp6, vp10; } cam = {vp2, vp6, vp10};
-    if (blockIdx.x == 0 && threadIdx.x < FRAME_SLOTS) {
+    if (FRAME) {
+        if (blockIdx.x == 0 && threadIdx.x == 0) *reinterpret_cast<uint32_t*>(slots_next) = 0u;
+    } else if (blockIdx.x == 0 && threadIdx.x < FRAME_SLOTS) {
         slots_next[(size_t)threadIdx.x * FRAME_SLOT_WORDS + 0] = 0x7fffffff;
         slots_next[(size_t)threadIdx.x * FRAME_SLOT_WORDS + 1] = (int32_t)0x80000000;
     }
@@ -374,11 +177,14 @@
     }
 }
 
+const void* depth_key_frame_kernel() { return (const void*)k_depth_key<true>; }
+dim3 depth_key_grid(uint32_t n) { const uint32_t per = PROJ_THREADS * KEY_PER_THREAD; return dim3((n + per - 1) / per); }
+
 void launch_depth_key(const SceneSoA& sc, uint32_t n, const CamParams& cam, int32_t* depth, int32_t* slots, int32_t* slots_next, hipStream_t s)
 {
     if (!n) return;
     const uint32_t per = PROJ_THREADS * KEY_PER_THREAD;
-    hipLaunchKernelGGL(k_depth_key, dim3((n + per - 1) / per), dim3(PROJ_THREADS), 0, s, sc, n, cam.vp2, cam.vp6, cam.vp10, depth, slots, slots_next);
+    hipLaunchKernelGGL(k_depth_key<false>, dim3((n + per - 1) / per), dim3(PROJ_THREADS), 0, s, sc, n, cam.vp2, cam.vp6, cam.vp10, depth, slots, slots_next);
 }
 
 void ProjectLaunch::bind()
diff --git a/gsplat.js_amd/csrc/k_project_body.h b/gsplat.js_amd/csrc/k_project_body.h
--- /dev/null
+++ b/gsplat.js_amd/csrc/k_project_body.h
@@ -0,0 +1,261 @@
+#pragma once
+#include "gsr_internal.h"
+
+namespace gsr {
+
+__device__ __forceinline__ void mat3_mul(const float* a, const float* b, float* r)
+{
+#pragma unroll
+    for (int c = 0; c < 3; c++)
+#pragma unroll
+        for (int ro = 0; ro < 3; ro++) {
+            float s = a[0 * 3 + ro] * b[c * 3 + 0];
+            s = s + a[1 * 3 + ro] * b[c * 3 + 1];
+            s = s + a[2 * 3 + ro] * b[c * 3 + 2];
+            r[c * 3 + ro] = s;
+        }
+}
+
+__device__ __forceinline__ float half_bits_to_float(uint32_t h)
+{
+    return (float)__builtin_bit_cast(_Float16, (unsigned short)(h & 0xffffu));
+}
+
+__device__ __forceinline__ bool finite4(float a, float b, float c, float d)
+{
+    return isfinite(a) && isfinite(b) && isfinite(c) && isfinite(d);
+}
+
+__device__ __forceinline__ float eval_sh_channel(const float* k, uint32_t deg, float x, float y, float z)
+{
+    constexpr float C0 = 0.28209479177387814f, C1 = 0.4886025119029199f;
+    constexpr float C2_0 = 1.0925484305920792f, C2_1 = -1.0925484305920792f, C2_2 = 0.31539156525252005f,
+                    C2_3 = -1.0925484305920792f, C2_4 = 0.5462742152960396f;
+    constexpr float C3_0 = -0.5900435899266435f, C3_1 = 2.890611442640554f, C3_2 = -0.4570457994644658f,
+                    C3_3 = 0.3731763325901154f, C3_4 = -0.4570457994644658f, C3_5 = 1.445305721320277f,
+                    C3_6 = -0.5900435899266435f;
+    float r = C0 * k[0];
+    if (deg > 0) {
+        r = r - ((((C1 * y) * k[1]) + ((C1 * z) * k[2])) - ((C1 * x) * k[3]));
+        if (deg > 1) {
+            const float xx = x * x, yy = y * y, zz = z * z, xy = x * y, yz = y * z, xz = x * z;
+            float s2 = (C2_0 * xy) * k[4];
+            s2 = s2 + (C2_1 * yz) * k[5];
+            s2 = s2 + (C2_2 * ((2.0f * zz - xx) - yy)) * k[6];
+            s2 = s2 + (C2_3 * xz) * k[7];
+            s2 = s2 + (C2_4 * (xx - yy)) * k[8];
+            r = r + s2;
+            if (deg > 2) {
+                float s3 = ((C3_0 * y) * (3.0f * xx - yy)) * k[9];
+                s3 = s3 + ((C3_1 * xy) * z) * k[10];
+                s3 = s3 + ((C3_2 * y) * ((4.0f * zz - xx) - yy)) * k[11];
+                s3 = s3 + ((C3_3 * z) * ((2.0f * zz - 3.0f * xx) - 3.0f * yy)) * k[12];
+                s3 = s3 + ((C3_4 * x) * ((4.0f * zz - xx) - yy)) * k[13];
+                s3 = s3 + ((C3_5 * z) * (xx - yy)) * k[14];
+                s3 = s3 + ((C3_6 * x) * (xx - 3.0f * yy)) * k[15];
+                r = r + s3;
+            }
+        }
+    }
+    r = r + 0.5f;
+    r = (r > 0.0f) ? r : 0.0f;
+    return (r < 1.0f) ? r : 1.0f;
+}
+
+__device__ __forceinline__ float eval_sh_texture(const uint32_t* __restrict__ tex, uint32_t t, uint32_t deg, float x, float y, float z)
+{
+    const uint4 a = reinterpret_cast<const uint4*>(tex)[2 * (size_t)t], b = reinterpret_cast<const uint4*>(tex)[2 * (size_t)t + 1];
+    const uint32_t w[8] = {a.x, a.y, a.z, a.w, b.x, b.y, b.z, b.w};
+    float k[16];
+#pragma unroll
+    for (int j = 0; j < 8; j++) { k[2 * j] = half_bits_to_float(w[j]); k[2 * j + 1] = half_bits_to_float(w[j] >> 16); }
+    return eval_sh_channel(k, deg, x, y, z);
+}
+
+
+__device__ __forceinline__ uint2 project_splat(const SceneSoA& sc, const CamParams& cam, uint32_t i, float x, float y, float z,
+                                               Record* __restrict__ rec, uint32_t& op8, float& area)
+{
+    uint2 bb = make_uint2(BBOX_INVISIBLE_X, BBOX_INVISIBLE_Y);
+    do {
+        float camv[4], pos2d[4];
+#pragma unroll
+        for (int r = 0; r < 4; r++) {
+            float s = cam.view[0 * 4 + r] * x;
+            s = s + cam.view[1 * 4 + r] * y;
+            s = s + cam.view[2 * 4 + r] * z;
+            s = s + cam.view[3 * 4 + r];
+            camv[r] = s;
+        }
+#pragma unroll
+        for (int r = 0; r < 4; r++) {
+            float s = cam.proj[0 * 4 + r] * camv[0];
+            s = s + cam.proj[1 * 4 + r] * camv[1];
+            s = s + cam.proj[2 * 4 + r] * camv[2];
+            s = s + cam.proj[3 * 4 + r] * camv[3];
+            pos2d[r] = s;
+        }
+        const float clip = 1.2f * pos2d[3];
+        if (pos2d[2] < -pos2d[3] || pos2d[0] < -clip || pos2d[0] > clip || pos2d[1] < -clip || pos2d[1] > clip) break;
+
+        const uint32_t c0 = sc.cov0[i], c1 = sc.cov1[i], c2 = sc.cov2[i], cw = sc.rgba[i];
+        const float u1x = half_bits_to_float(c0), u1y = half_bits_to_float(c0 >> 16);
+        const float u2x = half_bits_to_float(c1), u2y = half_bits_to_float(c1 >> 16);
+        const float u3x = half_bits_to_float(c2), u3y = half_bits_to_float(c2 >> 16);
+        const float Vrk[9] = {u1x, u1y, u2x, u1y, u2y, u3x, u2x, u3x, u3y};
+        const float zz = camv[2] * camv[2];
+        const float J[9] = {cam.fx / camv[2], 0.f, -(cam.fx * camv[0]) / zz,
+                            0.f, -cam.fy / camv[2], (cam.fy * camv[1]) / zz,
+                            0.f, 0.f, 0.f};
+        const float V3t[9] = {cam.view[0], cam.view[4], cam.view[8], cam.view[1], cam.view[5],
+                              cam.view[9], cam.view[2], cam.view[6], cam.view[10]};
+        float T[9], Tt[9], TtV[9], cov2d[9];
+        mat3_mul(V3t, J, T);
+#pragma unroll
+        for (int c = 0; c < 3; c++)
+#pragma unroll
+            for (int r = 0; r < 3; r++) Tt[c * 3 + r] = T[r * 3 + c];
+        mat3_mul(Tt, Vrk, TtV);
+        mat3_mul(TtV, T, cov2d);
+        const float a = cov2d[0] + 0.3f;
+        const float b = cov2d[1];
+        const float c = cov2d[4] + 0.3f;
+        const float det = a * c - b * b;
+        if (det == 0.0f) break;
+        const float mid = (a + c) / 2.0f;
+        const float rad = mid * mid - det;
+        const float sq = sqrtf((0.1f < rad) ? rad : 0.1f);
+        const float lambda1 = mid + sq;
+        const float lambda2 = mid - sq;
+        if (lambda2 < 0.0f) break;
+        const float dvx = b, dvy = lambda1 - a;
+        const float len = sqrtf(dvx * dvx + dvy * dvy);
+        const float dgx = dvx / len, dgy = dvy / len;
+        float smaj = sqrtf(2.0f * lambda1), smin = sqrtf(2.0f * lambda2);
+        smaj = (1024.0f < smaj) ? 1024.0f : smaj;
+        smin = (1024.0f < smin) ? 1024.0f : smin;
+        float majx = smaj * dgx, majy = smaj * dgy;
+        float minx = smin * dgy, miny = smin * -dgx;
+        if (cam.use_fade) {
+            const float depthNorm = (pos2d[2] / pos2d[3] + 1.0f) / 2.0f;
+            const float nearv = 0.1f, farv = 100.0f;
+            const float normalizedDepth = (2.0f * nearv) / (farv + nearv - depthNorm * (farv - nearv));
+            float st = normalizedDepth - 0.1f; st = (st > 0.0f) ? st : 0.0f;
+            float en = normalizedDepth + 0.1f; en = (en < 1.0f) ? en : 1.0f;
+            float sf = (cam.fade - st) / (en - st);
+            sf = (sf < 0.0f) ? 0.0f : ((sf > 1.0f) ? 1.0f : sf);
+            if (!(sf > 0.0f)) break;
+            majx = majx * sf; majy = majy * sf; minx = minx * sf; miny = miny * sf;
+        }
+        if (!finite4(majx, majy, minx, miny)) break;
+        const float opacity = (float)((cw >> 24) & 0xffu) / 255.0f;
+        op8 = (cw >> 24) & 0xffu;
+        const float vcx = pos2d[0] / pos2d[3], vcy = pos2d[1] / pos2d[3];
+        const float cx = ((vcx + 1.0f) * 0.5f) * (float)cam.W;
+        const float cy = ((1.0f - vcy) * 0.5f) * (float)cam.H;
+        const float m2 = majx * majx + majy * majy;
+        const float n2 = minx * minx + miny * miny;
+        const float im = 2.0f / m2, in = 2.0f / n2;
+        area = fminf(0.77f * __builtin_amdgcn_sqrtf(m2 * n2), 65535.0f);
+        Record r;
+        r.cx = cx; r.cy = cy;
+        r.ux = majx * im; r.uy = -majy * im;
+        r.wx = minx * in; r.wy = -miny * in;
+        if (!(finite4(r.ux, r.uy, r.wx, r.wy) && isfinite(cx) && isfinite(cy))) break;
+        r.la = __log2f(opacity);
+        r.rgb8 = cw & 0x00ffffffu;
+        if (cam.sh_on && (int32_t)i > cam.band[0]) {
+            const uint32_t deg = (int32_t)i > cam.band[1] ? ((int32_t)i > cam.band[2] ? 3u : 2u) : 1u;
+            float cp[3];
+#pragma unroll
+            for (int q = 0; q < 3; q++) {
+                float t = cam.view[q * 4 + 0] * cam.view[12];
+                t = t + cam.view[q * 4 + 1] * cam.view[13];
+                t = t + cam.view[q * 4 + 2] * cam.view[14];
+                cp[q] = -t;
+            }
+            float dvx = x - cp[0], dvy = y - cp[1], dvz = z - cp[2];
+            if (cam.sh_frame) {
+                const float e0 = (cam.shm[0] * dvx + cam.shm[1] * dvy) + cam.shm[2] * dvz;
+                const float e1 = (cam.shm[3] * dvx + cam.shm[4] * dvy) + cam.shm[5] * dvz;
+                const float e2 = (cam.shm[6] * dvx + cam.shm[7] * dvy) + cam.shm[8] * dvz;
+                dvx = e0; dvy = e1; dvz = e2;
+            }
+            const float dl = sqrtf((dvx * dvx + dvy * dvy) + dvz * dvz);
+            const float dxn = dvx / dl, dyn = dvy / dl, dzn = dvz / dl;
+            const uint32_t t = i - (uint32_t)(cam.band[0] + 1);
+            sc.shcol[i] = make_float4(eval_sh_texture(sc.sh_r, t, deg, dxn, dyn, dzn), eval_sh_texture(sc.sh_g, t, deg, dxn, dyn, dzn),
+                                      eval_sh_texture(sc.sh_b, t, deg, dxn, dyn, dzn), 0.0f);
+            r.rgb8 = RGB8_IN_SHCOL;
+        }
+        const float ex = sqrtf(majx * majx + minx * minx);
+        const float ey = sqrtf(majy * majy + miny * miny);
+        float fx0 = floorf(cx - ex - 0.5f), fx1 = ceilf(cx + ex - 0.5f);
+        float fy0 = floorf(cy - ey - 0.5f), fy1 = ceilf(cy + ey - 0.5f);
+        fx0 = fmaxf(fx0, 0.0f); fy0 = fmaxf(fy0, 0.0f);
+        fx1 = fminf(fx1, (float)(cam.W - 1)); fy1 = fminf(fy1, (float)(cam.H - 1));
+        if (fx0 <= fx1 && (fx1 < (float)cam.band_px0 || fx0 >= (float)cam.band_px1)) break;
+        float4* rp = reinterpret_cast<float4*>(rec + i);
+        rp[0] = make_float4(r.cx, r.cy, r.ux, r.uy);
+        rp[1] = make_float4(r.wx, r.wy, r.la, __uint_as_float(r.rgb8));
+        if (fx0 > fx1 || fy0 > fy1) break;
+        bb.x = (uint32_t)(int32_t)fx0 | ((uint32_t)(int32_t)fx1 << 16);
+        bb.y = (uint32_t)(int32_t)fy0 | ((uint32_t)(int32_t)fy1 << 16);
+    } while (0);
+    return bb;
+}
+
+__device__ __forceinline__ void count_splat(uint2 bb, uint32_t op8, float area, int bx_lo, int bx_hi, uint32_t& vis, uint32_t& tiles,
+                                            uint32_t& otiles, uint32_t& omass)
+{
+    if ((bb.x & 0xffffu) <= (bb.x >> 16)) {
+        vis++;
+        const int tx0 = max((int)(bb.x & 0xffffu) / TILE, bx_lo * BIN_TILES), tx1 = min((int)(bb.x >> 16) / TILE, bx_hi * BIN_TILES - 1);
+        const uint32_t nt = (uint32_t)((tx1 - tx0 + 1) * ((int)(bb.y >> 16) / TILE - (int)(bb.y & 0xffffu) / TILE + 1));
+        tiles += nt;
+        otiles += (op8 * min(nt, 4096u)) >> 4;
+        omass += (op8 * (uint32_t)area) >> 8;
+    }
+}
+
+template <int SUBS>
+__device__ __forceinline__ void project_ride_blocks(const RideArgs& ra, uint32_t rider)
+{
+    __shared__ uint32_t s_vis[SUBS][4], s_til[SUBS][4], s_oti[SUBS][4], s_oma[SUBS][4];
+    const CamParams& cam = ra.cam;
+    const uint32_t sub = threadIdx.x / PROJ_THREADS, t = threadIdx.x % PROJ_THREADS;
+    const uint32_t k = rider * SUBS + sub;
+    const bool mine = k < ra.count;
+    const uint32_t block = ra.first + k;
+    uint32_t vis = 0, tiles = 0, otiles = 0, omass = 0;
+    const int bx_lo = cam.band_px0 / BIN_PX, bx_hi = (cam.band_px1 + BIN_PX - 1) / BIN_PX;
+    const uint32_t i = block * PROJ_THREADS + t;
+    if (mine && i < ra.n) {
+        const float x = ra.sc.px[i], y = ra.sc.py[i], z = ra.sc.pz[i];
+        uint32_t op8 = 0;
+        float area = 0.0f;
+        const uint2 bb = project_splat(ra.sc, cam, i, x, y, z, ra.rec, op8, area);
+        ra.rect[i] = pack_bin_rect(bb.x, bb.y, bx_lo, bx_hi);
+        count_splat(bb, op8, area, bx_lo, bx_hi, vis, tiles, otiles, omass);
+    }
+#pragma unroll
+    for (int off = 32; off > 0; off >>= 1) {
+        vis += __shfl_xor(vis, off);
+        tiles += __shfl_xor(tiles, off);
+        otiles += __shfl_xor(otiles, off);
+        omass += __shfl_xor(omass, off);
+    }
+    const int wave = (int)(t >> 6);
+    if ((t & 63) == 0) { s_vis[sub][wave] = vis; s_til[sub][wave] = tiles; s_oti[sub][wave] = otiles; s_oma[sub][wave] = omass; }
+    __syncthreads();
+    if (t == 0 && mine) {
+        int32_t* slot = ra.slots + (size_t)(block & (FRAME_SLOTS - 1)) * FRAME_SLOT_WORDS;
+        atomicAdd(reinterpret_cast<uint32_t*>(&slot[2]), s_vis[sub][0] + s_vis[sub][1] + s_vis[sub][2] + s_vis[sub][3]);
+        atomicAdd(reinterpret_cast<uint32_t*>(&slot[3]), s_til[sub][0] + s_til[sub][1] + s_til[sub][2] + s_til[sub][3]);
+        atomicAdd(reinterpret_cast<uint32_t*>(&slot[4]), s_oti[sub][0] + s_oti[sub][1] + s_oti[sub][2] + s_oti[sub][3]);
+        atomicAdd(reinterpret_cast<uint32_t*>(&slot[5]), s_oma[sub][0] + s_oma[sub][1] + s_oma[sub][2] + s_oma[sub][3]);
+    }
+}
+inline uint32_t ride_workgroups(uint32_t count, uint32_t threads) { const uint32_t subs = threads / PROJ_THREADS; return (count + subs - 1) / subs; }
+
+}
diff --git a/gsplat.js_amd/csrc/k_sort.hip b/gsplat.js_amd/csrc/k_sort.hip
--- a/gsplat.js_amd/csrc/k_sort.hip
+++ b/gsplat.js_amd/csrc/k_sort.hip
@@ -1,4 +1,5 @@
 #include "gsr_internal.h"
+#include "k_project_body.h"
 
 #include <algorithm>
 #include <cstring>
@@ -119,13 +120,27 @@
     }
 }
 
+__device__ __forceinline__ const RideArgs& riders_of(const RideArgs& ra) { return ra; }
+__device__ __forceinline__ uint32_t host_grid_of(const RideArgs& ra) { return ra.host_grid; }
+__device__ __forceinline__ uint32_t host_grid_of() { return gridDim.x; }
+#define GSR_RIDERS_OR_HOST(THREADS)                                                                                    \
+    if constexpr (sizeof...(RIDE) != 0) {                                                                              \
+        const RideArgs& riders = riders_of(ra...);                                                                     \
+        if (blockIdx.x >= riders.host_grid) {                                                     \
+            project_ride_blocks<(THREADS) / (int)PROJ_THREADS>(riders, blockIdx.x - riders.host_grid);                 \
+            return;                                                                                                    \
+        }                                                                                                              \
+    }
+
+template <class... RIDE>
 __global__ __launch_bounds__(SORT_THREADS) void k_quantise_hist(const int32_t* __restrict__ depth,
                                                                 const int32_t* __restrict__ slots,
                                                                 int32_t* __restrict__ minmax_out, uint32_t n,
                                                                 uint32_t keys_per_block, const uint32_t* __restrict__ live,
                                                                 uint32_t* __restrict__ keys,
-                                                                uint32_t* __restrict__ block_hist, int hist_shift, int hist_bins)
-{
+                                                                uint32_t* __restrict__ block_hist, int hist_shift, int hist_bins, RIDE... ra)
+{
+    GSR_RIDERS_OR_HOST(SORT_THREADS)
     __shared__ uint32_t h_lo[RADIX_HI_BINS];
     __shared__ int32_t s_mm[2][SORT_THREADS / WAVE];
     for (int d = threadIdx.x; d < hist_bins; d += SORT_THREADS) h_lo[d] = 0;
@@ -198,10 +213,11 @@
 constexpr int CS_KEEP = 16;
 constexpr int CS_KEEP_LONG = 40;
 
-template <int KEEP>
+template <int KEEP, class... RIDE>
 __global__ __launch_bounds__(CS_THREADS) void k_column_scan(uint32_t* __restrict__ table, uint32_t* __restrict__ total,
-                                                            int ncols, uint32_t nrows, const uint32_t* __restrict__ live, uint32_t live_unit)
-{
+                                                            int ncols, uint32_t nrows, const uint32_t* __restrict__ live, uint32_t live_unit, RIDE... ra)
+{
+    GSR_RIDERS_OR_HOST(CS_THREADS)
     if (live) nrows = min(nrows, (*live + live_unit - 1u) / live_unit);
     __shared__ uint32_t s_sum[CS_SLOTS][CS_COLS];
     const int c = threadIdx.x & (CS_COLS - 1);
@@ -260,7 +276,6 @@
         if (slot == 0) total[col] = tot;
     }
 }
-
 void launch_column_scan(uint32_t* table, uint32_t* total, int ncols, uint32_t nrows, hipStream_t s, const uint32_t* live, uint32_t live_unit)
 {
     const dim3 grid((ncols + CS_COLS - 1) / CS_COLS), block(CS_THREADS);
@@ -281,7 +296,7 @@
     return (size_t)(waves * (1 << bits) + 2 * (1 << bits) + 3 * ((1 << bits) / WAVE) + 2 * keys_per_block) * sizeof(uint32_t);
 }
 
-template <int BITS, int SHIFT, bool FIRST, bool PAY = false, int WAVES = SCAT_WAVES>
+template <int BITS, int SHIFT, bool FIRST, bool PAY = false, int WAVES = SCAT_WAVES, class... RIDE>
 __global__ __launch_bounds__(WAVES * WAVE) void k_scatter(const uint32_t* __restrict__ keys_in,
                                                           const uint32_t* __restrict__ idx_in, uint32_t n_in,
                                                           uint32_t* __restrict__ count,
@@ -289,9 +304,10 @@
                                                           const uint32_t* __restrict__ total,
                                                           uint32_t* __restrict__ keys_out, uint32_t* __restrict__ idx_out,
                                                           uint32_t* __restrict__ max_bucket,
-                                                          const uint32_t* __restrict__ pay_in = nullptr, uint32_t* __restrict__ pay_out = nullptr,
-                                                          uint4* __restrict__ chunk_tab = nullptr)
-{
+                                                          const uint32_t* __restrict__ pay_in, uint32_t* __restrict__ pay_out,
+                                                          uint4* __restrict__ chunk_tab, RIDE... ra)
+{
+    GSR_RIDERS_OR_HOST(WAVES * WAVE)
     constexpr int BINS = 1 << BITS;
     constexpr int THREADS = WAVES * WAVE, MAX_STEPS = scat_max_steps(WAVES);
     static_assert(BINS <= THREADS, "one digit per thread");
@@ -305,7 +321,7 @@
     uint32_t* lkey = wsum + 3 * (BINS / WAVE);
     uint32_t* lidx = lkey + keys_per_block;
     const int lane = threadIdx.x & 63, wave = threadIdx.x >> 6;
-    const uint32_t blk = xcd_group_remap(blockIdx.x, gridDim.x);
+    const uint32_t blk = xcd_group_remap(blockIdx.x, host_grid_of(ra...));
     if ((unsigned long long)blk * keys_per_block >= n && blockIdx.x != 0) return;
     KSTAMP(0);
     uint32_t tot = 0, wg_base = 0;
@@ -449,12 +465,13 @@
 
 inline uint32_t local_sort_grid(uint32_t n) { return (n + LOCAL_CHUNK - 1) / LOCAL_CHUNK + RADIX_HI_BINS / 2 + 1; }
 
-template <int WAVES>
+template <int WAVES, class... RIDE>
 __global__ __launch_bounds__(WAVES * WAVE) void k_local_sort(const uint32_t* __restrict__ keys, const uint32_t* __restrict__ idx,
                                                               const uint4* __restrict__ chunk_tab,
                                                               uint32_t* __restrict__ depth_index,
-                                                              const uint32_t* __restrict__ pay_in, uint32_t* __restrict__ pay_out)
-{
+                                                              const uint32_t* __restrict__ pay_in, uint32_t* __restrict__ pay_out, RIDE... ra)
+{
+    GSR_RIDERS_OR_HOST(WAVES * WAVE)
     constexpr int BINS = RADIX_LO_BINS;
     constexpr int LOCAL_THREADS = WAVES * WAVE, LOCAL_WAVES = WAVES, LOCAL_STEPS = (int)LOCAL_CHUNK / LOCAL_THREADS;
     static_assert(BINS <= LOCAL_THREADS && LOCAL_STEPS * LOCAL_THREADS == (int)LOCAL_CHUNK, "one digit per thread, whole steps");
@@ -549,6 +566,8 @@
 constexpr uint32_t BUCKET_ORDER_MAX_N = 3u << 20;
 constexpr uint32_t LOCAL_BUCKET_LIMIT = 48u << 10;
 constexpr uint32_t CHUNK_TAB_SPARE = 2;
+constexpr bool RIDE_BY_DEFAULT = false;
+constexpr uint32_t RIDE_SHARES[RIDE_HOSTS] = {5, 7, 9, 12};
 
 inline uint32_t keys_per_block_of(uint32_t rows, const SortKnobs& k) { return k.sort_kpb ? k.sort_kpb : rows <= KPB_SMALL_MAX_ROWS ? KPB_SMALL : KPB_LARGE; }
 inline uint32_t ceil_div(uint32_t a, uint32_t b) { return (uint32_t)(((uint64_t)a + b - 1u) / b); }
@@ -564,10 +583,11 @@
     return z;
 }
 
-SortPlan plan_sort(uint32_t n, uint32_t rows, uint32_t front_waves, bool render, bool cull, uint32_t largest_bucket, const SortKnobs& k)
+SortPlan plan_sort(uint32_t n, uint32_t rows, uint32_t front_waves, bool render, bool cull, uint32_t largest_bucket, const SortKnobs& k, RidePlan* ride)
 {
     SortPlan p;
     memset(&p, 0, sizeof p);
+    if (ride) memset(ride, 0, sizeof *ride);
     p.keys_per_block = keys_per_block_of(rows, k);
     if (!n) return p;
     const bool bucket = k.sort_order >= 0 ? k.sort_order == 1 : (n <= BUCKET_ORDER_MAX_N && largest_bucket <= LOCAL_BUCKET_LIMIT);
@@ -581,6 +601,24 @@
     if (bucket) {
         p.lds_first = (uint32_t)scatter_lds_bytes(RADIX_HI_BITS, p.keys_per_block, (int)p.waves);
         p.local_grid = local_sort_grid(n);
+        const bool can_ride = render && !p.band && !p.carry;
+        if (ride && can_ride && (k.project_ride >= 0 ? k.project_ride == 1 : RIDE_BY_DEFAULT)) {
+            uint32_t share[RIDE_HOSTS];
+            for (int h = 0; h < RIDE_HOSTS; h++) share[h] = (k.ride_split[0] | k.ride_split[1] | k.ride_split[2] | k.ride_split[3]) ? k.ride_split[h] : RIDE_SHARES[h];
+            if (p.blocks > (uint32_t)CS_SLOTS * CS_KEEP) share[1] = 0;
+            uint64_t all = 0, run = 0;
+            for (int h = 0; h < RIDE_HOSTS; h++) all += share[h];
+            if (!all) share[3] = 1, all = 1;
+            uint32_t first = 0;
+            for (int h = 0; h < RIDE_HOSTS; h++) {
+                run += share[h];
+                const uint32_t end = (uint32_t)((uint64_t)p.proj_blocks * run / all);
+                ride->slice[h].first = first;
+                ride->slice[h].count = end - first;
+                first = end;
+            }
+            ride->on = 1u;
+        }
     } else {
         p.lds_first = (uint32_t)scatter_lds_bytes(RADIX_LO_BITS, p.keys_per_block, (int)p.waves);
         p.lds_last = (uint32_t)scatter_lds_bytes(RADIX_HI_BITS, p.keys_per_block, (int)p.waves);
@@ -594,6 +632,16 @@
     *out = plan_sort(n, rows, front_waves, render != 0, cull != 0, largest_bucket,
                      SortKnobs{sort_order, sort_kpb, rect_carry ? 1u : 0u, rect_carry_bucket ? 1u : 0u});
     return (int)sizeof(SortPlan);
+}
+extern "C" int gsr_debug_sort_plan_ride(unsigned int n, unsigned int rows, unsigned int front_waves, int render, int cull, unsigned int largest_bucket,
+                                         int sort_order, unsigned int sort_kpb, int rect_carry, int rect_carry_bucket, int project_ride,
+                                         const unsigned int* split, SortPlan* out, RidePlan* ride_out)
+{
+    SortKnobs k{sort_order, sort_kpb, rect_carry ? 1u : 0u, rect_carry_bucket ? 1u : 0u};
+    k.project_ride = project_ride;
+    for (int h = 0; split && h < RIDE_HOSTS; h++) k.ride_split[h] = split[h];
+    *out = plan_sort(n, rows, front_waves, render != 0, cull != 0, largest_bucket, k, ride_out);
+    return (int)sizeof(RidePlan);
 }
 extern "C" int gsr_debug_sort_sizes(unsigned int rows, unsigned int sort_kpb, unsigned long long* out)
 {
@@ -619,6 +667,12 @@
 struct LocalSortKernel { LocalSortFn fn; uint32_t waves; };
 static const LocalSortKernel LOCAL_SORT_KERNELS[] = {{k_local_sort<SCAT_WAVES>, FRONT_WAVES_WIDE}, {k_local_sort<FRONT_WAVES_NARROW>, FRONT_WAVES_NARROW}};
 
+struct ScatterRideKernel { const void* fn; uint32_t waves; };
+static const ScatterRideKernel SCATTER_RIDE_KERNELS[] = {{(const void*)k_scatter<RADIX_HI_BITS, RADIX_LO_BITS, true, false, SCAT_WAVES, RideArgs>, FRONT_WAVES_WIDE},
+                                                         {(const void*)k_scatter<RADIX_HI_BITS, RADIX_LO_BITS, true, false, FRONT_WAVES_NARROW, RideArgs>, FRONT_WAVES_NARROW}};
+static const ScatterRideKernel LOCAL_SORT_RIDE_KERNELS[] = {{(const void*)k_local_sort<SCAT_WAVES, RideArgs>, FRONT_WAVES_WIDE},
+                                                            {(const void*)k_local_sort<FRONT_WAVES_NARROW, RideArgs>, FRONT_WAVES_NARROW}};
+
 static const ScatterKernel& scatter_kernel(int bits, bool first, bool pay, uint32_t waves)
 {
     for (const ScatterKernel& k : SCATTER_KERNELS)
@@ -636,6 +690,9 @@
         for (const ScatterKernel& k : SCATTER_KERNELS)
             (void)hipFuncSetAttribute((const void*)k.fn, hipFuncAttributeMaxDynamicSharedMemorySize,
                                       (int)scatter_lds_bytes(k.bits, k.waves * WAVE * scat_max_steps((int)k.waves), (int)k.waves));
+        for (const ScatterRideKernel& k : SCATTER_RIDE_KERNELS)
+            (void)hipFuncSetAttribute((const void*)k.fn, hipFuncAttributeMaxDynamicSharedMemorySize,
+                                      (int)scatter_lds_bytes(RADIX_HI_BITS, k.waves * WAVE * scat_max_steps((int)k.waves), (int)k.waves));
         (void)hipGetLastError();
     });
 }
@@ -661,7 +718,7 @@
     const int bits = bucket ? RADIX_HI_BITS : RADIX_LO_BITS;
     uint32_t* total = bucket ? total_hi : total_lo;
     uint4* tab = bucket ? reinterpret_cast<uint4*>(b.chunk_tab) : nullptr;
-    hipLaunchKernelGGL(k_quantise_hist, grid, block, 0, s, depth_in, b.slots, b.minmax, n, p.keys_per_block, live, b.keys, b.block_hist,
+    hipLaunchKernelGGL(k_quantise_hist<>, grid, block, 0, s, depth_in, b.slots, b.minmax, n, p.keys_per_block, live, b.keys, b.block_hist,
                        bucket ? RADIX_LO_BITS : 0, 1 << bits);
     launch_column_scan(b.block_hist, total, 1 << bits, p.blocks, s, live, p.keys_per_block);
     const ScatterFn first = scatter_kernel(bits, true, p.carry, p.waves).fn;
@@ -682,4 +739,82 @@
                        (uint32_t*)nullptr, b.depth_index, b.max_bucket, p.carry ? (const uint32_t*)b.rect_tmp : nullptr, b.rects_out, (uint4*)nullptr);
 }
 
-}
+void bind_ride_chain(RideChain& r, const SortBuffers& b, uint32_t n, const SceneSoA& sc, int32_t* depth, Record* rec, uint32_t* rect, int32_t* slots,
+                     uint32_t* overflow)
+{
+    const SortPlan& p = b.plan;
+    uint32_t* total_hi = b.digit_total + RADIX_LO_BINS;
+    uint4* tab = reinterpret_cast<uint4*>(b.chunk_tab);
+    const CamParams cam = r.ra[0].cam;
+    r.key = {sc, n, cam.vp2, cam.vp6, cam.vp10, depth, slots, overflow};
+    r.quant = {b.depth, b.slots, b.minmax, n, p.keys_per_block, nullptr, b.keys, b.block_hist, RADIX_LO_BITS, RADIX_HI_BINS};
+    r.scan = {b.block_hist, total_hi, RADIX_HI_BINS, p.blocks, nullptr, p.keys_per_block};
+    r.scatter = {b.keys, nullptr, n, b.count, p.keys_per_block, b.block_hist, total_hi, b.keys_tmp, b.idx_tmp, b.max_bucket, nullptr, nullptr, tab};
+    r.local = {b.keys_tmp, b.idx_tmp, tab, b.depth_index, b.rect_tmp, b.rects_out};
+    const bool wide = p.waves == FRONT_WAVES_WIDE;
+    const uint32_t rows = p.blocks;
+    const void* scan_plain = rows <= (uint32_t)CS_SLOTS * CS_KEEP ? (const void*)k_column_scan<CS_KEEP>
+                             : rows <= (uint32_t)CS_SLOTS * CS_KEEP_LONG ? (const void*)k_column_scan<CS_KEEP_LONG> : (const void*)k_column_scan<0>;
+    const void* scan_ride = (const void*)k_column_scan<CS_KEEP, RideArgs>;
+    struct Host { const void* plain; const void* ride; uint32_t grid, threads, lds; };
+    const Host host[RIDE_HOSTS] = {
+        {(const void*)k_quantise_hist<>, (const void*)k_quantise_hist<RideArgs>, p.blocks, (uint32_t)SORT_THREADS, 0u},
+        {scan_plain, scan_ride, (uint32_t)((RADIX_HI_BINS + CS_COLS - 1) / CS_COLS), (uint32_t)CS_THREADS, 0u},
+        {(const void*)scatter_kernel(RADIX_HI_BITS, true, false, p.waves).fn, SCATTER_RIDE_KERNELS[wide ? 0 : 1].fn, p.blocks, p.waves * WAVE, p.lds_first},
+        {(const void*)local_sort_kernel(p.waves), LOCAL_SORT_RIDE_KERNELS[wide ? 0 : 1].fn, p.local_grid, p.waves * WAVE, 0u},
+    };
+    RideLaunch& k = r.launch[0];
+    k = RideLaunch{depth_key_frame_kernel(), depth_key_grid(n), dim3(PROJ_THREADS), 0u, true, {}};
+    {
+        void* q[] = {&r.key.sc, &r.key.n, &r.key.vp2, &r.key.vp6, &r.key.vp10, &r.key.depth, &r.key.slots, &r.key.overflow};
+        for (size_t a = 0; a < sizeof q / sizeof q[0]; a++) k.ptrs[a] = q[a];
+    }
+    for (int h = 0; h < RIDE_HOSTS; h++) {
+        const RideSlice sl = b.ride.slice[h];
+        r.ra[h] = RideArgs{sc, n, host[h].grid, sl.first, sl.count, cam, rec, rect, slots};
+        RideLaunch& l = r.launch[1 + h];
+        l = RideLaunch{sl.count ? host[h].ride : host[h].plain, dim3(host[h].grid + ride_workgroups(sl.count, host[h].threads)), dim3(host[h].threads),
+                       host[h].lds, sl.count != 0, {}};
+    }
+    {
+        RideChain::Quant& a = r.quant;
+        void* q[] = {&a.depth, &a.slots, &a.minmax, &a.n, &a.keys_per_block, &a.live, &a.keys, &a.block_hist, &a.hist_shift, &a.hist_bins, &r.ra[0]};
+        for (size_t i = 0; i < sizeof q / sizeof q[0]; i++) r.launch[1].ptrs[i] = q[i];
+    }
+    {
+        RideChain::Scan& a = r.scan;
+        void* q[] = {&a.table, &a.total, &a.ncols, &a.nrows, &a.live, &a.live_unit, &r.ra[1]};
+        for (size_t i = 0; i < sizeof q / sizeof q[0]; i++) r.launch[2].ptrs[i] = q[i];
+    }
+    {
+        RideChain::Scatter& a = r.scatter;
+        void* q[] = {&a.keys_in, &a.idx_in, &a.n_in, &a.count, &a.keys_per_block, &a.base, &a.total, &a.keys_out, &a.idx_out, &a.max_bucket, &a.pay_in,
+                     &a.pay_out, &a.chunk_tab, &r.ra[2]};
+        static_assert(sizeof q <= sizeof r.launch[3].ptrs, "one pointer per kernel argument");
+        for (size_t i = 0; i < sizeof q / sizeof q[0]; i++) r.launch[3].ptrs[i] = q[i];
+    }
+    {
+        RideChain::Local& a = r.local;
+        void* q[] = {&a.keys, &a.idx, &a.chunk_tab, &a.depth_index, &a.pay_in, &a.pay_out, &r.ra[3]};
+        for (size_t i = 0; i < sizeof q / sizeof q[0]; i++) r.launch[4].ptrs[i] = q[i];
+    }
+}
+
+void set_ride_camera(RideChain& r, const CamParams& cam)
+{
+    r.key.vp2 = cam.vp2; r.key.vp6 = cam.vp6; r.key.vp10 = cam.vp10;
+    for (RideArgs& a : r.ra) a.cam = cam;
+}
+
+static void launch_ride(const RideLaunch& l, hipStream_t s)
+{
+    (void)hipLaunchKernel(l.fn, l.grid, l.block, const_cast<void**>(l.ptrs), l.lds, s);
+}
+void launch_ride_key(const RideChain& r, hipStream_t s) { launch_ride(r.launch[0], s); }
+void launch_ride_sort(const RideChain& r, hipStream_t s)
+{
+    raise_scatter_lds();
+    for (int h = 0; h < RIDE_HOSTS; h++) launch_ride(r.launch[1 + h], s);
+}
+
+}
```

Result: slower. 5647 (-2.9%).
